# aicip/Cross-Scale-MAE

Measured on AMD Instinct MI355X. Metric: pretrain images/sec ViT-B/16 224^2 two-scale, higher is better.
Workload: dtype bf16; 1 GPU; MAE_ViT_MsLdCeCd ViT-B/16, 224^2 two-scale crops, mask 0.75, AdamW, full optimizer step; loss=mse, batch_per_gpu=128, global_batch=128, parallelism=dp1, headline_config=True

## Files before the change

### cross-scale-mae_amd/csmae_hip/__init__.py

```python
from __future__ import annotations

import ctypes
import os
from ctypes import c_float, c_int, c_longlong, c_void_p

import torch

F32, BF16 = 0, 1
ABI_VERSION = 7
EPI_NONE, EPI_GELU, EPI_RESID, EPI_DGELU, EPI_ATOMIC, EPI_SPLIT = 0, 1, 2, 3, 4, 5
EPI_GELU_Q8, EPI_DGELU_Q8 = 6, 7
ROUTE_F32, ROUTE_KSLAB = 7, 8
ATTN_ROUTE_RESIDENT, ATTN_ROUTE_STREAM, ATTN_ROUTE_ANY, ATTN_ROUTE_F32 = 0, 1, 2, 3
ATTN_STREAM_OWN, ATTN_STREAM_TILE = 128, 64
LOSS_KINDS = {"mse": 0, "l2": 1, "mae": 2, "l1": 3, "bce": 4, "none": 5}
SSIM_KINDS = {"ssim": ("none", 1, 1.0), "ms_ssim": ("none", 5, 1.0), "mse_ssim": ("mse", 1, 0.1), "mse_ms_ssim": ("mse", 5, 0.1)}

_ADDED_WITHIN_ABI = ("csmae_attn_route", "csmae_attn_stream_mode", "csmae_probe_pool_fwd", "csmae_bn1d_fwd", "csmae_head_linear_fwd",
                     "csmae_head_linear_bwd", "csmae_softmax_ce", "csmae_lars_step", "csmae_probe_pool_bwd", "csmae_head_linear_dx", "csmae_soft_ce",
                     "csmae_mixup_target", "csmae_mixup_cutmix", "csmae_pos_embed_grad", "csmae_eval_u8", "csmae_l2_normalize", "csmae_knn_select",
                     "csmae_knn_vote", "csmae_recon_eval", "csmae_recon_eval_workspace_floats", "csmae_recon_panel", "csmae_augment_u16",
                     "csmae_eval_u16")
_HERE = os.path.dirname(os.path.abspath(__file__))
LIB_PATH = os.environ.get("CSMAE_LIB_PATH") or os.path.join(_HERE, "libcsmae_hip.so")

I, L, P, F = c_int, c_longlong, c_void_p, c_float
_SIGNATURES = {
    "csmae_gemm": [I, I, I, L, L, L, P, L, P, L, P, L, I, P, I, P, L, P, L, I, P],
    "csmae_gemm_ks": [I, L, L, L, P, L, P, L, P, L, P, L, I, P, I, P, L, P, L, P],
    "csmae_weights_kslab": [I, P, I, P, P, P],
    "csmae_gemm_ln_supported": [L, L, L],
    "csmae_gemm_ln_fwd": [L, L, L, P, L, P, L, P, P, L, P, L, P, P, F, P, L, P, P, P],
    "csmae_gemm_ln_bwd": [L, L, L, P, L, P, L, P, L, P, P, P, P, L, P, L, P, L, P],
    "csmae_gemm_k2_mode": [I, I],
    "csmae_gemm_dw_mode": [I],
    "csmae_gemm_dw": [I, L, L, L, P, L, P, L, P, P, P, L, P],
    "csmae_gemm_dw_group": [I, I, L, P, P, P, P, P, P, P, P, I, P, L, P],
    "csmae_gemm_dw_group_fp8": [I, L, P, P, P, P, P, P, P, P, P, P, I, P, L, P],
    "csmae_fp8_amax": [I, L, I, P, L, P, P],
    "csmae_fp8_quantize": [I, I, I, L, I, P, L, P, L, P, P, P, P],
    "csmae_fp8_weights": [I, P, P, P, P, P, P, P],
    "csmae_gemm_fp8": [I, L, L, L, P, L, P, L, P, L, I, P, I, P, L, P, L, P, P, P, L, I, P, P, P, P],
    "csmae_gemm_force_tile": [I],
    "csmae_gemm_route": [I, I, I, L, L, L, L, L, L, I, I],
    "csmae_gemm_ks_route": [I, L, L, L, P, L, P, L, L, P, L, I],
    "csmae_attn_fwd": [I, L, I, I, I, P, P, P, P],
    "csmae_attn_bwd": [I, L, I, I, I, P, P, P, P, P, P],
    "csmae_attn_resident": [I, I, I],
    "csmae_attn_route": [I, I, I],
    "csmae_attn_stream_mode": [I],
    "csmae_attn_fwd_q": [I, L, I, I, I, P, P, P, P, I, P, P, P, P],
    "csmae_attn_bwd_q": [I, L, I, I, I, P, P, P, P, P, P, I, P, P, P, P],
    "csmae_layernorm_fwd": [I, I, L, I, P, P, P, F, P, P, P, P, P, I, P, P, P, P],
    "csmae_layernorm_bwd": [I, I, I, L, I, P, P, P, P, P, P, P, P, P, P, P, L, P, I, P, P, P, P],
    "csmae_ln_param_reduce": [I, L, I, P, L, L, P, P, P],
    "csmae_ln_param_reduce_rows": [I, I, I, P, L, P, P, P],
    "csmae_bnrelu_fwd": [I, I, I, I, P, P, P, F, F, P, P, P, P, P, P, I, P],
    "csmae_bnrelu_bwd": [I, I, I, I, P, P, P, P, P, P, P, P, P, P],
    "csmae_crop_resize": [L, I, P, P, P, P],
    "csmae_mask_sort": [L, I, I, P, P, P, P, P, P],
    "csmae_patch_gather": [I, L, I, I, I, I, I, P, P, P, P, L, P],
    "csmae_embed_assemble": [I, L, I, I, P, P, P, P, P, P],
    "csmae_embed_assemble_bwd": [I, I, L, I, I, P, P, P, P],
    "csmae_unshuffle_fwd": [I, L, I, I, I, P, P, P, P, P, P],
    "csmae_unshuffle_bwd": [I, I, L, I, I, I, P, P, P, P, P],
    "csmae_rows_gather": [I, L, I, P, L, L, L, P, P],
    "csmae_rows_scatter_add": [I, L, I, P, F, L, L, L, P, P],
    "csmae_rows_scatter_add2": [I, L, I, P, F, L, P, F, L, L, L, P, P],
    "csmae_spec_fixup": [P, P, L, P, L, P, L, P, P, P, P, I, P],
    "csmae_rows_gather_idx": [L, I, I, I, P, P, L, P, P],
    "csmae_target_minmax": [I, L, I, I, I, I, P, P, P, P, P],
    "csmae_recon_loss_fwd": [I, I, I, L, I, I, I, I, P, P, P, L, P, P, P, P],
    "csmae_recon_loss_bwd": [I, I, I, I, L, I, I, I, I, P, P, P, L, P, P, P, P, F, P, P, L, P],
    "csmae_ssim_workspace_floats": [L, I, I, I, I, P],
    "csmae_ssim_fwd": [I, I, I, L, I, I, I, I, P, P, P, L, P, P, P, P],
    "csmae_ssim_apply": [I, I, F, F, P, P, P],
    "csmae_ssim_bwd": [I, L, I, I, I, I, P, L, P, P, F, P, P, P],
    "csmae_pair_loss_fwd": [I, L, I, P, L, L, L, P, L, L, L, P, P],
    "csmae_pair_loss_bwd": [I, I, L, I, P, L, L, L, P, L, L, L, P, F, P, P, P, P],
    "csmae_ntxent_fwd": [I, I, I, I, P, F, F, P, P, P, P, P, P],
    "csmae_ntxent_bwd": [I, I, P, P, P, P, F, F, P, P, P],
    "csmae_latent_grad_finish": [I, L, I, I, P, P, F, P, P],
    "csmae_loss_finalize": [L, I, P, P, F, P, F, P, F, P, I, P, P],
    "csmae_augment_u8": [L, I, I, I, I, P, P, P, P, P, P],
    "csmae_eval_u8": [L, I, I, I, I, P, P, P, P, P, P],
    "csmae_augment_u16": [L, I, I, I, I, I, P, P, P, P, P, P, P],
    "csmae_eval_u16": [L, I, I, I, I, I, P, P, P, P, P, P, P],
    "csmae_next_launch_event": [P],
    "csmae_flush_launch_event": [P],
    "csmae_adamw": [L, P, P, P, P, P, P, P, F, F, F, F, F, F, P, P, P, P, P],
    "csmae_adamw_fp8": [L, P, F, P, P, P, P, F, F, F, F, F, F, P, P, P, P, P, P, P, P],
# ... 91 lines not shown
```

### cross-scale-mae_amd/csmae_hip/engine.py

```python
from __future__ import annotations

import contextlib
import math
import os
import weakref
from typing import Dict, Optional

import torch

from . import BF16, EPI_ATOMIC, EPI_DGELU, EPI_GELU, EPI_NONE, EPI_RESID, F32, SSIM_KINDS, debug_opt, ops
from . import trace

_FROZEN = ("encoder_pos_embed", "decoder_pos_embed")
_GEN_GONE = ("csmae_hip: backward of a forward whose activations are gone — the model ran another forward (training, eval "
             "or viz) in between; the engine keeps ONE activation workspace, so call loss.backward() before the next "
             "model(...) (accumulate gradients across backward calls, not across forwards)")
_GEN_TWICE = ("csmae_hip: backward called twice for the same forward (retain_graph is not supported: the reverse pass "
              "consumes the workspace)")


def _round_up(x, m):
    return (x + m - 1) // m * m


class FlatParams:

    def __init__(self, module: torch.nn.Module, device):
        self.names, self.slots = [], {}
        off = 0
        params = list(module.named_parameters())
        for name, p in params:
            n = p.numel()
            self.slots[name] = (off, n, tuple(p.shape))
            self.names.append(name)
            off += _round_up(n, 8)
        self.total = off
        self.p = torch.zeros(off, device=device, dtype=torch.float32)
        self.g = torch.zeros(off + 8, device=device, dtype=torch.float32)
        self.gate = self.g[off:off + 1]
        self.w_lp: Optional[torch.Tensor] = None
        self.lp_stamp = None
        self.raw_writes = 0
        self.params = dict(params)
        with torch.no_grad():
            for name, p in params:
                o, n, shape = self.slots[name]
                view = self.p[o:o + n].view(shape)
                view.copy_(p.data.to(device))
                p.data = view
        self.grad_views = {name: self.g[o:o + n].view(shape) for name, (o, n, shape) in self.slots.items()}
        self._by_id = {id(p): name for name, p in params}
        FlatParams._registry.append(weakref.ref(self))

    _registry = []

    @classmethod
    def owner_of(cls, p):
        alive = []
        found = None
        for ref in cls._registry:
            f = ref()
            if f is None:
                continue
            alive.append(ref)
            name = f._by_id.get(id(p))
            if name is not None and p.is_cuda and p.data_ptr() == f.p.data_ptr() + f.slots[name][0] * 4:
                found = f
        cls._registry[:] = alive
        return found

    def slot_of(self, p):
        return self.slots[self._by_id[id(p)]]

    def version_stamp(self) -> int:
        return sum(p._version for p in self.params.values())
# ... 121 lines not shown
                u8 = dict(device=dev, dtype=torch.uint8)
                self.t4_8 = [E(big8, **u8) for _ in range(2)]
                self.t3_8 = [E(max(Me * 3 * D, Md * 3 * Dd), **u8) for _ in range(2)]
                self.dres_e_8 = [E(Me, D, **u8) for _ in range(5)]
                self.dres_d_8 = [E(Md, Dd, **u8) for _ in range(5)]
            self.fp8_hist = False
            self.fp8_complete = False
        self.dw_ws = E(64 * 1024 * 1024, **f32)


class Engine:
    def __init__(self, module: torch.nn.Module, flat: FlatParams, cfg: dict, act_dtype=torch.bfloat16):
        self.module, self.cfg, self.device = module, cfg, flat.p.device
        self.fp8 = act_dtype == "fp8"
        self._fp8_site = 0
        self.fp8_dw = self.fp8 and not debug_opt("fp8_bf16_dw")
        self._fp8_blk = {}
        self._fp8_kept = {}
        self._fp8_cur = None
        self._fp8_fuse_lnb = not debug_opt("fp8_no_fuse_lnb")
        self._fp8_fuse_attn = not debug_opt("fp8_no_fuse_attn")
        self._fp8_fuse = not debug_opt("fp8_no_fuse")
        if self.fp8:
            act_dtype = torch.bfloat16
        if self.device.type != "cuda":
            raise RuntimeError("csmae_hip.Engine needs an MI355X (device 'cuda'): there is no CPU or eager fallback on the product path")
        self.act_dtype = act_dtype
        self.T = BF16 if act_dtype == torch.bfloat16 else F32
        self.res_dtype = torch.float32 if (self.T == F32 or os.environ.get("CSMAE_RESID_FP32")) else torch.bfloat16
        self.gp_q8 = self.T == BF16
        v = cfg["variant"]
        self.views = 1 if v == "Baseline" else 2
        self.has_pred = v in ("MsLdCd", "MsLdLeCd", "MsLdCeCd")
        self.has_ce = v == "MsLdCeCd"
        self.has_le = v in ("MsLdLe", "MsLdLeCd")
        self.Pp = _round_up(cfg["P"], 8) if self.T == BF16 else cfg["P"]
        self.flat = flat
        if self.T == BF16:
            if flat.w_lp is None:
                flat.w_lp = torch.zeros(flat.total, device=self.device, dtype=torch.bfloat16)
            if self.Pp != cfg["P"]:
                self.w_pe_pad = torch.zeros(cfg["D"], self.Pp, device=self.device, dtype=torch.bfloat16)
                self.w_pred_pad = torch.zeros(self.Pp, cfg["Dd"], device=self.device, dtype=torch.bfloat16)
        self.ws: Optional[Workspace] = None
        self._saved = None
        self.gen = 0
        self._gen_done = -1
        self.side, self.main, self.aux = None, None, None
        self._fwd_streams = []
        self._so = {}
        self._events, self._ev_i, self._side_reads, self._tog = [], 0, {}, 0
        self._side_seq, self._side_waited = 0, 0
        self._dw_cache = {}
        for key in ("bwd_main_cus", "main_cus"):
            v = debug_opt(key)
            if v is not None and not (len(v.split(":")) == 2 and all(q.isdigit() for q in v.split(":")) and int(v.split(":")[0]) < int(v.split(":")[1])):
                raise ValueError(f"CSMAE_DEBUG {key}={v!r}: expected lo:hi (mask bits of the compute units)")
        if not str(debug_opt("dw_cus", "0")).isdigit():
            raise ValueError(f"CSMAE_DEBUG dw_cus={debug_opt('dw_cus')!r}: expected the number of CUs per XCD")
        self.ln_fuse = self.T == BF16 and not self.fp8 and self.res_dtype == torch.bfloat16 and not debug_opt("no_lnfuse")
        self.ln_fuse_fwd = self.ln_fuse and not debug_opt("no_lnfuse_fwd")
        self.ln_fuse_bwd = self.ln_fuse and not debug_opt("no_lnfuse_bwd")
        self._ln_fuse_mask = int(debug_opt("lnfuse_mask", "15"))
        self.use_ks = not debug_opt("no_kslab")
        self._dw_slots = int(debug_opt("dw_slots", "160"))
        se = os.environ.get("CSMAE_DW_SLOTS_ED", "" if debug_opt("dw_slots") else "160,128")
        self._dw_slots_ed = tuple(int(v) for v in se.split(",")) if se else None
        self._dw_mode = debug_opt("dw_group", "half")
        self._dw_rot = self._dw_mode != "half0"
        if self._dw_mode == "half0":
            self._dw_mode = "half"
        if self._dw_mode not in ("block", "block_enc", "block_dec", "half", "none"):
            raise ValueError(f"CSMAE_DEBUG dw_group={self._dw_mode!r}: block, block_enc, block_dec, half or none")
        sl = flat.slots
        goff = lambda names: torch.tensor([[sl[n + ".weight"][0], sl[n + ".bias"][0]] for n in names], dtype=torch.long, device=self.device)
        self._goff_e = goff([f"encoder.{i}.norm{k}" for i in range(cfg["Ne"]) for k in (1, 2)])
        self._goff_d = goff([f"decoder.{i}.norm{k}" for i in range(cfg["Nd"]) for k in (1, 2)] + ["decoder_norm"])

    def W(self, name):
        if self.T == BF16:
            return self.flat.lp(name)
        t = self.flat.P(name)
        return t.view(t.shape[0], -1) if t.dim() > 1 else t

    def _refresh_lp(self, lazy_pads=False):
        if self.T != BF16:
            return
        if not self.fp8:
            self.flat.fp8_active = False
        stamp = self.flat.version_stamp()
        if stamp != self.flat.lp_stamp:
            self._opt_gate()
            ops.cast_bf16(self.flat.p, self.flat.w_lp)
            self.flat.lp_stamp = stamp
        if self.Pp != self.cfg["P"] and not lazy_pads:
            self._opt_gate()
            self._refresh_pads(True, True)
        self._refresh_ks()

    def _refresh_pads(self, pe, pred):
        P = self.cfg["P"]
        if pe:
            self.w_pe_pad[:, :P].copy_(self.flat.P("patch_embed.proj.weight").view(self.cfg["D"], P))
        if pred:
            self.w_pred_pad[:P].copy_(self.flat.P("decoder_pred.weight"))

# ... 122 lines not shown
                return ops.gemm_ks(a, f.w_ks[o:o + cnt], self.W(name), out, bias=bias, epilogue=epilogue, aux=aux, resid=resid, st=st)
            return ops.gemm(a, self.W(name), out, trans_b=trans_b, bias=bias, epilogue=epilogue, aux=aux, resid=resid, st=st)
        f, ws = self.flat, self.ws
        M, K = a.shape
        o, cnt, shape = f.slots[name]
        b8 = f.w8t[o:o + cnt].view(shape[1], shape[0]) if trans_b else f.w8[o:o + cnt].view(shape)
        fmt = ops.FP8_E5M2 if trans_b else ops.FP8_E4M3
        prev, cur = ws.fp8_amax[1], ws.fp8_amax[0]
        if a8 is not None:
            k = site
        else:
            k = site if site is not None else self._fp8_alloc()
            a8 = ws.a8[lane][: M * K].view(M, K)
            if ws.fp8_hist:
                ops.fp8_quantize(a, a8, prev[k], ws.fp8_dq[k:k + 1], fmt=fmt, amax_next=cur[k], st=st)
            else:
                ops.fp8_quantize(a, a8, cur[k], ws.fp8_dq[k:k + 1], fmt=fmt, st=st)
        emit = self._emit_to(emit_site, emit_dst, fmt) if emit_dst is not None else self._emit(emit_site, ws.q_b[lane], out.shape[0], out.shape[1], fmt)
        wi = f.w8_idx[name]
        return ops.gemm_fp8(a8, b8, out, ws.fp8_dq[k:k + 1], f.w8_dq[wi:wi + 1], a_fmt=fmt, bias=bias, epilogue=epilogue, aux=aux, resid=resid,
                            emit=emit, skip_out=skip_out and emit is not None, st=st)

    @staticmethod
    def _splitk(m_out, n_out, k_red, tile, ktile):
        tiles = math.ceil(m_out / tile) * math.ceil(n_out / tile)
        kt = math.ceil(k_red / ktile)
        want = max(1, 768 // tiles)
        return max(1, min(want, kt // 4 if kt >= 8 else 1))

    def _dw(self, dy, x, name):
        self._dw_group([(dy, x, name)])

    def _dw_group(self, items, slots=None, ready=None, items8=None):
        if items8 is not None:
            key = tuple((n, dy.data_ptr(), x.data_ptr(), qy.data_ptr(), qx.data_ptr()) for dy, qy, x, qx, n in items8)
            grp = self._dw_cache.get(key)
            if grp is None:
                prods = []
                for dy, qy, x, qx, name in items8:
                    gw = self.flat.G(name + ".weight")
                    gw2 = gw.view(gw.shape[0], -1)
                    prods.append((dy[:, : gw2.shape[0]], qy, x[:, : gw2.shape[1]], qx, gw2, self.flat.G(name + ".bias")))
                grp = self._dw_cache[key] = ops.DwGroup8(prods, self.ws.dw_ws)
        else:
            key = tuple((n, dy.data_ptr(), x.data_ptr()) for dy, x, n in items)
            grp = self._dw_cache.get(key)
        if grp is None:
            prods = []
            for dy, x, name in items:
                gw = self.flat.G(name + ".weight")
                gw2 = gw.view(gw.shape[0], -1)
                prods.append((dy[:, : gw2.shape[0]], x[:, : gw2.shape[1]], gw2, self.flat.G(name + ".bias")))
            grp = self._dw_cache[key] = ops.DwGroup(prods, self.ws.dw_ws)
        if ops._timer is not None or os.environ.get("CSMAE_DW_MAIN"):
            grp.launch(256, st=self.st)
            return
        side = self.side
        if ready is not None:
            ev = ready
        else:
            ev = self._event()
            ev.record(self.main)
        side.wait_event(ev)
        grp.launch(slots or self._dw_slots, st=side.cuda_stream)
        done = self._event()
        done.record(side)
        self._side_seq += 1
        for dy, _, _ in items:
            self._side_reads[dy.data_ptr()] = (self._side_seq, done)

    def _guard_write(self, *bufs):
        last = None
        for b in bufs:
            e = self._side_reads.pop(b.data_ptr(), None)
            if e is not None and (last is None or e[0] > last[0]):
                last = e
        if last is not None:
            if self._side_waited < last[0]:
                self.main.wait_event(last[1])
                self._side_waited = last[0]

    def _event(self):
        if self._ev_i == len(self._events):
            e = torch.cuda.Event()
            e.record()
            self._events.append(e)
        self._ev_i += 1
        return self._events[self._ev_i - 1]

    def _new_side(self):
        n = int(debug_opt("dw_cus", "0"))
        if n <= 0:
            return torch.cuda.Stream()
        self._side_masked = True
        return ops.cu_masked_stream(0, 8 * n)

    def _join_side(self):
        self.main.wait_stream(self.side)
        self._side_reads.clear()
        self._side_waited = self._side_seq

    def _block_fwd(self, S, i, pre, M, Dm, H, B2, T, b0=0, nb=None, st=None):
        P = self.flat.P
        st = self.st if st is None else st
        nb = B2 if nb is None else nb
        r = slice(b0 * T, (b0 + nb) * T)
        x_in, x_mid, x_out = S["x"][i][r], S["xm"][i][r], S["x"][i + 1][r]
        stt = [a[r] for a in S["st"][i]]
        lse = S["lse"][i][b0 * H * T: (b0 + nb) * H * T]
        qkv, o, h, pre_a = S["qkv"][i][r], S["o"][i][r], S["h"][i][r], S["pre"][i][r]
        y1, y2 = S["y1"][i][r], S["y2"][i][r]
        ws_q_a = self.ws.q_a if self.fp8 else None
        ln = int(b0 > 0)
        Mr = y1.shape[0]
        k1 = ko = k2 = kh = None
        if getattr(self.flat, "opt_pending", None) is not None:
            self._opt_gate((pre + "attn.qkv.weight", pre + "mlp.fc2.weight"), None if st is None else (self._so.get(st) or torch.cuda.ExternalStream(st)))
        if self.fp8:
            sites = self._fp8_blk.get((id(S), i))
            if sites is None:
                sites = self._fp8_blk[(id(S), i)] = tuple(self._fp8_alloc() for _ in range(4))
            k1, ko, k2, kh = sites
# ... 413 lines not shown
            self.ws = Workspace(self, N, keep)
        ws, P = self.ws, self.flat.P
        self.st = st = ops.stream()
        L, D = c["L"], c["D"]
        self.gen += 1
        if training:
            self._saved = dict(stream=True, N=N, keep=keep, gen=self.gen)
        self._opt_gate()
        self._refresh_lp()
        self._ks_wait()
        self._fp8_begin()
        ws.noise.copy_(noise)
        ops.mask_sort(ws.noise, keep, ws.ids_restore, ws.mask, ws.ids_keep, st=st)
        ops.patch_gather(imgs, None, ws.ids_keep, ws.a_pe, N, c["C"], c["S"], c["p"], keep, st=st)
        ops.gemm(ws.a_pe, self._w_pe(), ws.tok, bias=P("patch_embed.proj.bias"), st=st)
        ops.embed_assemble(ws.tok, P("encoder_pos_embed").view(L + 1, D), P("cls_token").view(D), ws.ids_keep, ws.enc["x"][0], N, keep, st=st)
        for i in range(c["Ne"]):
            self._block_fwd(ws.enc, i, f"encoder.{i}.", ws.Me, D, c["He"], N, ws.Te)
        return ws

    def stream_grad(self):
        return self.ws.dres_e if self.res_dtype == torch.float32 else self.ws.dres_e_lp[0]

    def stream_backward_ready(self, gen: Optional[int] = None):
        sv = self._saved
        if sv is None or not sv.get("stream"):
            if gen is not None and gen != self.gen:
                raise RuntimeError(_GEN_GONE)
            raise RuntimeError("backward_stream() called without a preceding encode_stream(training=True)")
        if (gen is not None and gen != sv["gen"]) or sv["gen"] != self.gen:
            raise RuntimeError(_GEN_GONE)
        if sv["gen"] == self._gen_done:
            raise RuntimeError(_GEN_TWICE)

    def backward_stream(self, dres: torch.Tensor, accumulate: bool, gen: Optional[int] = None, loss: Optional[torch.Tensor] = None):
        if self.fp8:
            raise NotImplementedError("backward_stream: the stand-alone encoder's backward is not implemented for fp8 engines")
        if getattr(self.module, "_dp", None) is not None:
            raise NotImplementedError("backward_stream: data-parallel gradient hooks are not implemented for the stand-alone encoder's backward")
        assert self.views == 1
        self.stream_backward_ready(gen)
        c, ws, sv = self.cfg, self.ws, self._saved
        N, keep, D = sv["N"], sv["keep"], c["D"]
        if keep != c["L"]:
            raise ValueError("backward_stream: the position-embedding gradient needs every patch in its place (mask_ratio 0)")
        self._gen_done = sv["gen"]
        self.st = st = ops.stream()
        self._opt_gate()
        self.main = torch.cuda.current_stream()
        if self.side is None:
            self.side = self._new_side()
        self._ev_i, self._tog = 0, 0
        self._side_reads.clear()
        with trace.range_("csmae.backward.encoder"):
            if not accumulate:
                self.flat.g[: self.flat.total].zero_()
            if loss is not None:
                ops.gate_accumulate(loss, self.flat.gate, accumulate, st=st)
            buf = self.stream_grad()
            if dres.dtype != buf.dtype or dres.numel() != buf.numel():
                raise ValueError(f"backward_stream: dres must be {tuple(buf.shape)} elements of {buf.dtype}, got {tuple(dres.shape)} of {dres.dtype}")
            if dres.data_ptr() != buf.data_ptr():
                buf.copy_(dres.reshape(buf.shape))
            if self.res_dtype == torch.float32:
                ops.latent_grad_finish(ws.dres_e, None, 1.0, ws.dres_e_lp[0], ws.B2, ws.Te, st=st)
            first = self._encoder_bwd()
            if self.flat.params["encoder_pos_embed"].requires_grad:
                ops.pos_embed_grad(first.view(N, ws.Te, D), self.flat.G("encoder_pos_embed").view(ws.Te, D), accumulate=True, st=st)
        for name, p in self.flat.params.items():
            if p.requires_grad:
                p.grad = self.flat.grad_views[name]
            elif not name.startswith("decoder"):
                self.flat.grad_views[name].zero_()

    def decode(self, latent: torch.Tensor, ids_restore: torch.Tensor):
        assert self.views == 1
        c = self.cfg
        N, Te, D = latent.shape
        keep, L, Dd = Te - 1, c["L"], c["Dd"]
        if self.ws is None or self.ws.N != N or self.ws.keep != keep:
            self.ws = None
            self.ws = Workspace(self, N, keep)
        ws, P = self.ws, self.flat.P
        self.st = st = ops.stream()
        self._opt_gate()
        self._refresh_lp()
        self._ks_wait()
        self._fp8_begin()
        lat = latent.reshape(N * Te, D).to(torch.float32).contiguous()
        if self.T == BF16:
            lat_op = ws.lat_lp if ws.lat_lp is not None else ws.enc["x"][c["Ne"]]
            ops.cast_bf16(lat, lat_op, st=st)
        else:
            lat_op = lat
        ws.ids_restore.copy_(ids_restore)
        ops.gemm(lat_op, self.W("decoder_embed.weight"), ws.z, bias=P("decoder_embed.bias"), st=st)
        ops.unshuffle_fwd(ws.z, P("mask_token").view(Dd), P("decoder_pos_embed").view(L + 1, Dd), ws.ids_restore, ws.dec["x"][0], N, L, keep, st=st)
        for i in range(c["Nd"]):
            self._block_fwd(ws.dec, i, f"decoder.{i}.", ws.Md, Dd, c["Hd"], N, ws.Td)
        ops.layernorm_fwd(ws.dec["x"][c["Nd"]], P("decoder_norm.weight"), P("decoder_norm.bias"), ws.emb_lp, ws.dn_st[0], ws.dn_st[1], y32=ws.emb32, st=st)
        ops.gemm(ws.emb_lp, self._w_pred()[: c["P"]], ws.pred, bias=P("decoder_pred.bias"), st=st)
        pred = ws.pred
        if pred.dtype != torch.float32:
            pred = torch.empty(ws.pred.shape, device=self.device, dtype=torch.float32)
            ops.cast_f32(ws.pred, pred, st=st)
        return pred.view(N, ws.Td, c["P"])[:, 1:, :].clone(), ws.emb32.view(N, ws.Td, Dd).clone()
# ... 7 lines not shown
        if not rng:
            with trace.range_("csmae.backward"):
                return self._backward(gout, accumulate, gen)
        lo, hi = (int(v) for v in rng.split(":"))
        outer, inner = torch.cuda.current_stream(), ops.cu_masked_stream(lo, hi)
        inner.wait_stream(outer)
        with torch.cuda.stream(inner):
            self._backward(gout, accumulate, gen)
        outer.wait_stream(inner)

    def _encoder_bwd(self, dp=None):
        c, ws, st, G = self.cfg, self.ws, self.st, self.flat.G
        B2, Te, D, keep = ws.B2, ws.Te, c["D"], self._saved["keep"]
        lp_stream = self.res_dtype != torch.float32
        self._fp8_cur = None
        pe, flushed = ws.ln_part_e, c["Ne"]
        fe = lp_stream and self._ln_fused_bwd(ws.Me, D)
        ke_ = 0
        for i in reversed(range(c["Ne"])):
            ke_ = self._block_bwd(ws.enc, i, f"encoder.{i}.", ws.Me, D, c["He"], B2, Te, None if lp_stream else ws.dres_e, ws.dres_e_lp, ke_, (pe[2 * i], pe[2 * i + 1]),
                                  lps8=ws.dres_e_8 if (self.fp8 and self.fp8_dw and lp_stream) else None)
            if dp is not None and dp.wants(("enc", i)):
                self._ln_flush(pe, self._goff_e, 2 * i, 2 * flushed, ws.Me, D, fused=fe)
                flushed = i
                dp.grads_ready(self.flat, ("enc", i), also=self.side if not (ops._timer is not None or os.environ.get("CSMAE_DW_MAIN")) else None)
        self._ln_flush(pe, self._goff_e, 0, 2 * flushed, ws.Me, D, fused=fe)
        first = ws.dres_e_lp[ke_] if lp_stream else ws.dres_e
        ops.embed_assemble_bwd(first, ws.dtok_lp, G("cls_token").view(D), B2, keep, st=st)
        self._join_side()
        ops.DwGroup([(ws.dtok_lp, ws.a_pe[:, : c["P"]], G("patch_embed.proj.weight").view(D, c["P"]), G("patch_embed.proj.bias"))], ws.dw_ws).launch(256, st=st)
        return first

    def _backward(self, gout: torch.Tensor, accumulate: bool, gen: Optional[int] = None):
        c, ws, sv = self.cfg, self.ws, self._saved
        if sv is None:
            raise RuntimeError("backward() called without a preceding forward()")
        if sv.get("stream"):
            raise RuntimeError("backward() after encode_stream(): the stand-alone encoder's reverse pass is backward_stream()")
        if gen is not None and gen != sv["gen"]:
            raise RuntimeError(_GEN_GONE)
        if sv["gen"] == self._gen_done:
            raise RuntimeError(_GEN_TWICE)
        self._gen_done = sv["gen"]
        P, G = self.flat.P, self.flat.G
        self.st = st = ops.stream()
        self._opt_gate()
        N, keep = sv["N"], sv["keep"]
        B2, Te, Td, L, D, Dd = ws.B2, ws.Te, ws.Td, c["L"], c["D"], c["Dd"]
        self.main = torch.cuda.current_stream()
        if self.side is None:
            self.side = self._new_side()
        self._ev_i, self._tog = 0, 0
        self._side_reads.clear()
        zeroed = None
        if not accumulate:
            if ops._timer is not None or os.environ.get("CSMAE_DW_MAIN") or debug_opt("zero_main"):
                self.flat.g[: self.flat.total].zero_()
            else:
                self.side.wait_stream(self.main)
                with torch.cuda.stream(self.side):
                    self.flat.g[: self.flat.total].zero_()
                zeroed = self._event()
                zeroed.record(self.side)
        ops.gate_accumulate(ws.losses, self.flat.gate, accumulate, st=st)
        ws.gout.copy_(gout.reshape(1).to(torch.float32))
        head_start = self._event()
        head_start.record(self.main)
        kind, npx = c["loss"], c["norm_pix"]
        trace.push("csmae.backward.junction")
        extra = None
        ssim = SSIM_KINDS.get(kind)
        if ssim is not None:
            kind, extra = ssim[0], ws.ssim_extra
            ops.ssim_bwd(ssim[1], ws.pred, ws.mask, ws.gout, sv["rscale"] * ssim[2], ws.ssim_ws, extra, B2, N, c["C"], c["S"], c["p"], st=st)
        ops.recon_loss_bwd(kind, npx, sv["img0"], sv["img1"], ws.pred, sv["mm"], ws.mask, ws.losses, ws.gout, sv["rscale"], ws.dpred_lp,
                           B2, N, c["C"], c["S"], c["p"], extra=extra, st=st)
        timed = ops._timer is not None or bool(os.environ.get("CSMAE_DW_MAIN"))
        heads_serial = timed or not self.has_pred
        if heads_serial:
            self._dw(ws.dpred_lp, ws.emb_lp, "decoder_pred")
        ops.gemm(ws.dpred_lp, self._w_pred(), ws.demb, trans_b=True, st=st)
        if zeroed is not None:
            self.main.wait_event(zeroed)
        if self.has_pred:
            kcd = c["loss_cd"]
            bn = "predictor.1."
            if heads_serial:
                ops.pair_loss_bwd(kcd, N * L, Dd, ws.v, (N * L, 0, 0), ws.emb32, (L, Td, 1), ws.gout, self._pair_scale(kcd, N * L, Dd),
                                  da_lp=ws.dv, dt_acc=ws.demb, st=st)
                self._dw(ws.dv, ws.r, "predictor.3")
                ops.gemm(ws.dv, self.W("predictor.3.weight"), ws.dr, trans_b=True, st=st)
                ops.bnrelu_bwd(ws.u, ws.dr, P(bn + "weight"), P(bn + "bias"), ws.bn_st[0], ws.bn_st[1], ws.dr, G(bn + "weight"), G(bn + "bias"), N, L, st=st)
                self._dw(ws.dr, ws.pin, "predictor.0")
                ops.gemm(ws.dr, self.W("predictor.0.weight"), ws.dpin, trans_b=True, st=st)
                ops.rows_scatter_add(ws.dpin, ws.demb, L, Td, N * Td + 1, st=st)
            else:
                aux, ast = self.aux, self.aux.cuda_stream
                aux.wait_event(head_start)
                if sv.get("spec"):
                    if zeroed is not None:
                        aux.wait_event(zeroed)
                    ops.spec_fixup(ws.gout, (ws.dv, ws.dr, ws.dpin), ws.bn_tmp, G(bn + "weight"), G(bn + "bias"), st=ast)
                else:
                    ops.pair_loss_bwd(kcd, N * L, Dd, ws.v, (N * L, 0, 0), ws.emb32, (L, Td, 1), ws.gout, self._pair_scale(kcd, N * L, Dd),
                                      da_lp=ws.dv, st=ast)
                    ops.gemm(ws.dv, self.W("predictor.3.weight"), ws.dr, trans_b=True, st=ast)
                    if zeroed is not None:
                        aux.wait_event(zeroed)
                    ops.bnrelu_bwd(ws.u, ws.dr, P(bn + "weight"), P(bn + "bias"), ws.bn_st[0], ws.bn_st[1], ws.dr, G(bn + "weight"), G(bn + "bias"), N, L, st=ast)
                    ops.gemm(ws.dr, self.W("predictor.0.weight"), ws.dpin, trans_b=True, st=ast)
                self.main.wait_stream(aux)
                ops.rows_scatter_add2(ws.dv, -1.0, 1, ws.dpin, 1.0, N * Td + 1, ws.demb, L, Td, st=st)
                ej = self._event()
                ej.record(self.main)
# ... 1 lines not shown
                self._dw_group([(ws.dv, ws.r, "predictor.3"), (ws.dr, ws.pin, "predictor.0")], ready=ej)
        trace.pop()
        trace.push("csmae.backward.decoder")
        lp_stream = self.res_dtype != torch.float32
        pd, Nd2 = ws.ln_part_d, 2 * c["Nd"]
        self._fp8_cur = None
        if lp_stream:
            k0 = self._fp8_alloc()
            e0 = None
            if self.fp8 and self._fp8_fuse_lnb:
                e0 = self._emit_to(k0, ws.dres_d_8[0], 1) if self.fp8_dw else self._emit(k0, ws.q_a[1], ws.Md, Dd, 1)
            ops.layernorm_bwd(ws.demb, ws.dec["x"][c["Nd"]], ws.dn_st[0], ws.dn_st[1], P("decoder_norm.weight"), ws.dres_d_lp[0], None, None,
                              partial_ws=pd[Nd2], emit=e0, st=st)
            if k0 is not None:
                self._fp8_cur = (k0, e0[0] if e0 else None)
        else:
            ops.layernorm_bwd(ws.demb, ws.dec["x"][c["Nd"]], ws.dn_st[0], ws.dn_st[1], P("decoder_norm.weight"), ws.dres_d, None, None,
                              dx_lp=ws.dres_d_lp[0], partial_ws=pd[Nd2], st=st)
        kd_ = 0
        for i in reversed(range(c["Nd"])):
            kd_ = self._block_bwd(ws.dec, i, f"decoder.{i}.", ws.Md, Dd, c["Hd"], B2, Td, ws.dres_d, ws.dres_d_lp, kd_, (pd[2 * i], pd[2 * i + 1]),
                                  lps8=ws.dres_d_8 if (self.fp8 and self.fp8_dw and lp_stream) else None)
        if lp_stream and self._ln_fused_bwd(ws.Md, Dd):
            self._ln_flush(pd, self._goff_d, 0, Nd2, ws.Md, Dd, fused=True)
            self._ln_flush(pd, self._goff_d, Nd2, Nd2 + 1, ws.Md, Dd)
        else:
            self._ln_flush(pd, self._goff_d, 0, Nd2 + 1, ws.Md, Dd)
        ops.unshuffle_bwd(ws.dres_d_lp[kd_] if lp_stream else ws.dres_d, ws.ids_restore, ws.dz_lp, G("mask_token").view(Dd), B2, L, keep, st=st)
        lat_op = ws.enc["x"][c["Ne"]] if (lp_stream or self.T != BF16) else ws.lat_lp
        self._dw(ws.dz_lp, lat_op, "decoder_embed")
        ops.gemm(ws.dz_lp, self.W("decoder_embed.weight"), ws.dres_e, trans_b=True, st=st)
        dp = getattr(self.module, "_dp", None)
        if dp is not None:
            dp.grads_ready(self.flat, "tail", also=self.side if not (ops._timer is not None or os.environ.get("CSMAE_DW_MAIN")) else None)
        trace.pop()
        trace.push("csmae.backward.encoder")
        latent = ws.lat32 if ws.lat32 is not None else ws.enc["x"][c["Ne"]]
        if self.has_le:
            ke = c["loss_e"]
            ops.pair_loss_bwd(ke, N * Te, D, latent, (N * Te, 0, N * Te), latent, (N * Te, 0, 0), ws.gout, self._pair_scale(ke, N * Te, D),
                              da_acc=ws.dres_e, dt_acc=ws.dres_e, lp_dtype=self.T, st=st)
        dpool = None
        if self.has_ce:
            ops.ntxent_bwd(ws.zc, ws.inv_norm, ws.E, ws.neg, ws.gout, ws.dpool, N, st=st)
            dpool = ws.dpool
        ops.latent_grad_finish(ws.dres_e, dpool, 1.0 / keep, ws.dres_e_lp[0], B2, Te, st=st)
        self._encoder_bwd(dp)
        if dp is not None:
            dp.grads_ready(self.flat, "stem")
            dp.backward_done(self.flat)
        trace.pop()
        if self.fp8:
            ws.fp8_complete = True
        for name, p in self.flat.params.items():
            if p.requires_grad and not name.startswith("encoder_norm."):
                p.grad = self.flat.grad_views[name]
            elif not (name in _FROZEN or name.startswith("encoder_norm.")):
                self.flat.grad_views[name].zero_()
```

### cross-scale-mae_amd/csmae_hip/ops.py

```python
from __future__ import annotations

import ctypes

import torch

from . import BF16, EPI_ATOMIC, EPI_DGELU, EPI_GELU, EPI_NONE, EPI_RESID, F32, LOSS_KINDS, check, load
from . import EPI_DGELU_Q8 as _EPI_DGELU_Q8, EPI_GELU_Q8 as _EPI_GELU_Q8

_DT = {torch.float32: F32, torch.bfloat16: BF16}
_timer = None
_Q8 = {EPI_GELU: _EPI_GELU_Q8, EPI_DGELU: _EPI_DGELU_Q8}


class KernelTimer:

    def __init__(self):
        self.records, self._e0 = [], None

    def __enter__(self):
        global _timer
        _timer = self
        return self

    def __exit__(self, *a):
# ... 132 lines not shown
    return rc


def gemm_ks(a, bk, b_plain, out, *, bias=None, epilogue=EPI_NONE, aux=None, resid=None, st=None):
    M, K = a.shape
    N = b_plain.shape[0]
    assert b_plain.shape[1] == K and out.shape == (M, N) and a.stride(1) == 1 and out.stride(1) == 1 and b_plain.stride(1) == 1
    assert resid is None or resid.dtype == out.dtype
    assert bk.dtype == torch.bfloat16 and bk.is_contiguous() and bk.numel() >= N * K, "gemm_ks: the K-slab mirror is a flat bf16 tensor of N * K elements"
    epilogue = _epi(epilogue, aux)
    t = _begin()
    check(load().csmae_gemm_ks(dt(a), M, N, K, _p(a), a.stride(0), _p(bk), N, _p(b_plain), b_plain.stride(0), _p(out), out.stride(0), dt(out), _p(bias), epilogue,
                               _p(aux), aux.stride(0) if aux is not None else 0, _p(resid), resid.stride(0) if resid is not None else 0, _s(st)), "csmae_gemm_ks")
    if t:
        t.end(("gemm_bf16" if a.dtype == torch.bfloat16 else "gemm_f32") + "_NT", 2.0 * M * N * K)
    return out


def gemm_ln_supported(M, N, K):
    return load().csmae_gemm_ln_supported(M, N, K) == 1


def gemm_ln_fwd(a, bk, bias, resid, x_out, gamma, beta, y, mean, rstd, eps=1e-6, st=None):
    M, K = a.shape
    N = x_out.shape[1]
    assert a.dtype == resid.dtype == x_out.dtype == y.dtype == bk.dtype == torch.bfloat16 and bk.is_contiguous() and bk.numel() >= N * K
    assert resid.shape == x_out.shape == y.shape == (M, N) and a.stride(1) == resid.stride(1) == x_out.stride(1) == y.stride(1) == 1
    assert mean.dtype == rstd.dtype == torch.float32 and mean.numel() >= M and rstd.numel() >= M and gamma.numel() == beta.numel() == N
    t = _begin()
    check(load().csmae_gemm_ln_fwd(M, N, K, _p(a), a.stride(0), _p(bk), N, _p(bias), _p(resid), resid.stride(0), _p(x_out), x_out.stride(0), _p(gamma), _p(beta),
                                   eps, _p(y), y.stride(0), _p(mean), _p(rstd), _s(st)), "csmae_gemm_ln_fwd")
    if t:
        t.end("gemm_bf16_NT", 2.0 * M * N * K)


def gemm_ln_bwd(dy, w, x, mean, rstd, gamma, dres_in, dx_out, partial_ws=None, st=None):
    M, K = dy.shape
    N = w.shape[1]
    assert w.shape[0] == K and x.shape == dx_out.shape == (M, N) and (dres_in is None or dres_in.shape == (M, N))
    assert dy.dtype == w.dtype == x.dtype == dx_out.dtype == torch.bfloat16 and (dres_in is None or dres_in.dtype == torch.bfloat16)
    assert dy.stride(1) == w.stride(1) == x.stride(1) == dx_out.stride(1) == 1 and mean.dtype == rstd.dtype == torch.float32
    t = _begin()
    check(load().csmae_gemm_ln_bwd(M, N, K, _p(dy), dy.stride(0), _p(w), w.stride(0), _p(x), x.stride(0), _p(mean), _p(rstd), _p(gamma), _p(dres_in),
                                   dres_in.stride(0) if dres_in is not None else 0, _p(dx_out), dx_out.stride(0), _p(partial_ws),
                                   partial_ws.numel() if partial_ws is not None else 0, _s(st)), "csmae_gemm_ln_bwd")
    if t:
        t.end("gemm_bf16_NN", 2.0 * M * N * K)


def weights_kslab(desc, src, dst, max_blocks=64, st=None):
    check(load().csmae_weights_kslab(desc.shape[0], _p(desc), max_blocks, _p(src), _p(dst), _s(st)), "csmae_weights_kslab")


def gemm_dw(dy, x, dw, workspace, db=None, st=None):
    K, M = dy.shape
    N = x.shape[1]
    assert x.shape[0] == K and dw.shape == (M, N) and dw.is_contiguous() and dy.dtype == x.dtype
    t = _begin()
    check(load().csmae_gemm_dw(dt(dy), M, N, K, _p(dy), dy.stride(0), _p(x), x.stride(0), _p(dw), _p(db), _p(workspace), workspace.numel(), _s(st)), "csmae_gemm_dw")
    if t:
        t.end(("gemm_bf16" if dy.dtype == torch.bfloat16 else "gemm_f32") + "_TN", 2.0 * M * N * K)


FP8_E4M3, FP8_E5M2 = 0, 1


def fp8_quantize(src, dst, amax, dq, fmt=FP8_E4M3, transpose=False, amax_next=None, st=None):
    rows, cols = src.shape
    assert dst.dtype == torch.uint8 and dst.shape == ((cols, rows) if transpose else (rows, cols)) and src.stride(1) == 1 and dst.stride(1) == 1
    s = _s(st)
    if amax_next is None:
        check(load().csmae_fp8_amax(dt(src), rows, cols, _p(src), src.stride(0), _p(amax), s), "csmae_fp8_amax")
    check(load().csmae_fp8_quantize(dt(src), fmt, int(transpose), rows, cols, _p(src), src.stride(0), _p(dst), dst.stride(0), _p(amax), _p(dq),
                                    _p(amax_next), s), "csmae_fp8_quantize")


FP8_SLOTS = 64


def fp8_weights(desc, p, w8, w8t, amax, dq, st=None):
    check(load().csmae_fp8_weights(desc.shape[0], _p(desc), _p(p), _p(w8), _p(w8t), _p(amax), _p(dq), _s(st)), "csmae_fp8_weights")


def gemm_fp8(a8, b8, out, dq_a, dq_b, *, a_fmt=FP8_E4M3, bias=None, epilogue=EPI_NONE, aux=None, resid=None, emit=None, skip_out=False, st=None):
    assert not skip_out or emit is not None
    M, K = a8.shape
    N = b8.shape[0]
    assert a8.dtype == torch.uint8 and b8.dtype == torch.uint8 and b8.shape[1] == K and out.shape == (M, N)
    assert resid is None or resid.dtype == out.dtype
    epilogue = _epi(epilogue, aux)
    q_out, *q_rest = _emit_args(emit)
    t = _begin()
    check(load().csmae_gemm_fp8(a_fmt, M, N, K, _p(a8), a8.stride(0), _p(b8), b8.stride(0), None if skip_out else _p(out), out.stride(0), dt(out), _p(bias), epilogue,
                                _p(aux), aux.stride(0) if aux is not None else 0, _p(resid), resid.stride(0) if resid is not None else 0,
                                _p(dq_a), _p(dq_b), q_out, emit[0].stride(0) if emit else 0, *q_rest, _s(st)), "csmae_gemm_fp8")
    if t:
        t.end("gemm_fp8_NT", 2.0 * M * N * K)
    return out


def _dw_group_args(self, products, workspace, dy, x, dw, db):
    VP, LL = ctypes.c_void_p * len(products), ctypes.c_longlong * len(products)
    self.n, self.keep = len(products), (products, workspace)
    self.dY, self.X, self.dW, self.dB = (VP(*[_p(q[i]) for q in products]) for i in (dy, x, dw, db))
    self.ldy, self.ldx = LL(*[q[dy].stride(0) for q in products]), LL(*[q[x].stride(0) for q in products])
    self.M, self.N = LL(*[q[dw].shape[0] for q in products]), LL(*[q[dw].shape[1] for q in products])
    self.flops = sum(2.0 * q[dw].shape[0] * q[dw].shape[1] * self.K for q in products)
    self.ws, self.ws_n = _p(workspace), workspace.numel()


class DwGroup:

    def __init__(self, products, workspace):
        self.K = products[0][0].shape[0]
        self.dtype = dt(products[0][0])
        for dy, x, dw, db in products:
            assert dy.shape[0] == self.K and x.shape[0] == self.K and dw.is_contiguous() and dy.dtype == x.dtype and dy.stride(1) == 1 and x.stride(1) == 1
        _dw_group_args(self, products, workspace, 0, 1, 2, 3)

    def launch(self, slots=0, st=None):
        t = _begin()
        check(load().csmae_gemm_dw_group(self.dtype, self.n, self.K, self.dY, self.ldy, self.X, self.ldx, self.dW, self.dB, self.M, self.N, slots,
                                         self.ws, self.ws_n, _s(st)), "csmae_gemm_dw_group")
        if t:
            t.end(("gemm_bf16" if self.dtype == BF16 else "gemm_f32") + "_TN", self.flops)


class DwGroup8:

    def __init__(self, products, workspace):
        self.K = products[0][0].shape[0]
        for dy, dqy, x, dqx, dw, db in products:
            assert dy.dtype == x.dtype == torch.uint8 and dy.shape[0] == x.shape[0] == self.K and dy.stride(1) == x.stride(1) == 1 and dw.is_contiguous()
            assert dqy.dtype == dqx.dtype == torch.float32 and dqy.numel() >= 1 and dqx.numel() >= 1
        _dw_group_args(self, products, workspace, 0, 2, 4, 5)
        self.dqy, self.dqx = ((ctypes.c_void_p * self.n)(*[_p(q[i]) for q in products]) for i in (1, 3))

    def launch(self, slots=0, st=None):
        t = _begin()
        check(load().csmae_gemm_dw_group_fp8(self.n, self.K, self.dY, self.ldy, self.dqy, self.X, self.ldx, self.dqx, self.dW, self.dB, self.M, self.N, slots,
                                             self.ws, self.ws_n, _s(st)), "csmae_gemm_dw_group_fp8")
        if t:
            t.end("gemm_fp8_TN", self.flops)


def attn_resident(dtype_code, T, hd):
    return load().csmae_attn_resident(dtype_code, T, hd) == 1


def attn_route(dtype_code, T, hd):
    rc = load().csmae_attn_route(dtype_code, T, hd)
    if rc < 0:
        raise RuntimeError(f"csmae_attn_route: dtype {dtype_code}, T {T}, head_dim {hd} unsupported ({rc})")
    return rc


def attn_stream_mode(mode=-1):
    return load().csmae_attn_stream_mode(mode)


def attn_fwd(qkv, out, lse, B, T, H, hd, emit=None, st=None):
    if emit is None:
        check(load().csmae_attn_fwd(dt(qkv), B, T, H, hd, _p(qkv), _p(out), _p(lse), _s(st)), "csmae_attn_fwd")
    else:
        check(load().csmae_attn_fwd_q(dt(qkv), B, T, H, hd, _p(qkv), _p(out), _p(lse), *_emit_args(emit), _s(st)), "csmae_attn_fwd_q")


def attn_bwd(qkv, out, dout, lse, dqkv, B, T, H, hd, emit=None, skip_out=False, st=None):
    assert not skip_out or emit is not None
    if emit is None:
        check(load().csmae_attn_bwd(dt(qkv), B, T, H, hd, _p(qkv), _p(out), _p(dout), _p(lse), _p(dqkv), _s(st)), "csmae_attn_bwd")
    else:
        check(load().csmae_attn_bwd_q(dt(qkv), B, T, H, hd, _p(qkv), _p(out), _p(dout), _p(lse), None if skip_out else _p(dqkv), *_emit_args(emit), _s(st)),
              "csmae_attn_bwd_q")


def _emit_args(emit):
    if emit is None:
        return None, 0, None, None, None
    return _p(emit[0]), emit[1], _p(emit[2]), _p(emit[3]), _p(emit[4])


def layernorm_fwd(x, gamma, beta, y, mean, rstd, y32=None, eps=1e-6, emit=None, skip_out=False, st=None):
    M, D = x.shape
    assert not skip_out or emit is not None
    check(load().csmae_layernorm_fwd(dt(x), dt(y), M, D, _p(x), _p(gamma), _p(beta), eps, None if skip_out else _p(y), _p(y32), _p(mean), _p(rstd), *_emit_args(emit),
                                     _s(st)), "csmae_layernorm_fwd")


def layernorm_bwd(dy, x, mean, rstd, gamma, dx_out, dgamma, dbeta, dres_in=None, dx_lp=None, partial_ws=None, emit=None, st=None):
    M, D = x.shape
    assert dx_out.dtype == x.dtype and (dres_in is None or dres_in.dtype == x.dtype)
    lp = dt(dx_lp) if dx_lp is not None else dt(dy)
    check(load().csmae_layernorm_bwd(dt(dy), dt(x), lp, M, D, _p(dy), _p(x), _p(mean), _p(rstd), _p(gamma), _p(dres_in), _p(dx_out), _p(dx_lp), _p(dgamma), _p(dbeta),
# ... 412 lines not shown
```

### cross-scale-mae_amd/csrc/gemm.hip

```cpp
#include "gemm_common.h"

template <bool TA, bool TB, int BM, int BN, int WM, int WN, int GEMM_STAGES, bool DB, int MINW = 1>
__global__ __launch_bounds__((BM / WM) * (BN / WN) * 64, MINW) void gemm_bf16_kernel(GemmArgs p) {
  constexpr int NWN = BN / WN, NW = (BM / WM) * NWN, FM = WM / 16, FN = WN / 16;
  constexpr int A_BYTES = BM * GEMM_BK * 2, B_BYTES = BN * GEMM_BK * 2, STAGE = A_BYTES + B_BYTES;
  constexpr int PA = A_BYTES / 1024, PB = B_BYTES / 1024, PPW = (PA + PB) / NW;
  static_assert((PA + PB) % NW == 0, "DMA pieces must divide evenly over the waves");
  __shared__ __attribute__((aligned(16))) char smem[GEMM_STAGES * STAGE];
  const int lane = threadIdx.x & 63, w = __builtin_amdgcn_readfirstlane(threadIdx.x >> 6);
  const int t = lane & 15, g = lane >> 4;
  const int tiles = p.tiles_m * p.tiles_n;
  const int wg = xcd_remap(blockIdx.x, tiles * p.splitk);
  const int split = wg / tiles, tile = wg - split * tiles;
  const int tm = tile / p.tiles_n, tn = tile - tm * p.tiles_n;
  const int m0 = tm * BM, n0 = tn * BN;
  const int kt_begin = split * p.ktiles_per_split;
  const int kt_end = min(kt_begin + p.ktiles_per_split, p.ktiles);
  if (kt_begin >= kt_end) return;
  if (p.epi == EPI_SPLIT) p.C = reinterpret_cast<float*>(p.C) + (long long)split * p.split_stride;

  const i4_t rsA = make_rsrc(p.A, p.a_bytes), rsB = make_rsrc(p.B, p.b_bytes);
  const unsigned kstepA = TA ? (unsigned)(GEMM_BK * p.lda * 2) : (unsigned)(GEMM_BK * 2);
  const unsigned kstepB = TB ? (unsigned)(GEMM_BK * p.ldb * 2) : (unsigned)(GEMM_BK * 2);

// ... 119 lines not shown
      if (!(grp == 1 && kt == last)) __builtin_amdgcn_s_barrier();
      __builtin_amdgcn_sched_barrier(0);
    }
  } else {
    int issued = min(kt_begin + GEMM_STAGES - 2, last);
    for (int kt = kt_begin; kt <= issued; ++kt) stage(kt);
    s8_t fa0[FM] = {}, fb0[FN] = {};
    for (int kt = kt_begin; kt < kt_end; ++kt) {
      arrive(kt, issued);
      if (issued < last) { ++issued; if (!(dbg & 32)) stage(issued); }
      if (!(dbg & 128)) read_frags(kt, fa0, fb0);
      if (!(dbg & 64)) mma(fa0, fb0);
    }
  }
  if (do_cs && g == 0) {
#pragma unroll
    for (int i = 0; i < FM; ++i) {
      const int m = m0 + wm + i * 16 + t;
      if (m < p.M) p.colsum[(long long)split * p.M + m] = accb[i][0];
    }
  }
  if ((p.force_cfg & 16) && acc[0][0][0] != 123456.0f) return;
  if (p.epi == EPI_ATOMIC) {
#pragma unroll
    for (int i = 0; i < FM; ++i)
#pragma unroll
      for (int j = 0; j < FN; ++j)
        epi_dispatch(p, m0 + wm + i * 16 + t, n0 + wn + j * 16 + 4 * g, acc[i][j]);
    return;
  }
  constexpr int ESTR = WN + 4, LPR = WN / 4, RPP = 64 / LPR;
  constexpr int EROWS = (NW * 32 * ESTR * 4 <= GEMM_STAGES * STAGE) ? 32 : 16;
  static_assert(NW * EROWS * ESTR * 4 <= GEMM_STAGES * STAGE, "epilogue strip must fit the staging ring");
  if (!DB) __syncthreads();
  void* Cptr = p.C;
  float* ew = reinterpret_cast<float*>(smem) + w * (EROWS * ESTR);
#define EPI_CALL(TC_, E_) epilogue_rows<TC_, E_, FM, FN, WM, EROWS, ESTR, LPR, RPP>(p, Cptr, acc, ew, m0 + wm, n0 + wn, lane, t, g)
  if (p.c_dtype == CSMAE_BF16) {
    if (p.epi == EPI_GELU) EPI_CALL(bf16_t, EPI_GELU); else if (p.epi == EPI_DGELU) EPI_CALL(bf16_t, EPI_DGELU);
    else if (p.epi == EPI_RESID) EPI_CALL(bf16_t, EPI_RESID); else EPI_CALL(bf16_t, EPI_NONE);
  } else {
    if (p.epi == EPI_GELU) EPI_CALL(float, EPI_GELU); else if (p.epi == EPI_DGELU) EPI_CALL(float, EPI_DGELU);
    else if (p.epi == EPI_RESID) EPI_CALL(float, EPI_RESID); else EPI_CALL(float, EPI_NONE);
  }
#undef EPI_CALL
}

#ifdef GEMM_TIMING
extern "C" int csmae_debug_gemm_ts(unsigned long long* out) { return (int)hipMemcpyFromSymbol(out, HIP_SYMBOL(g_gemm_ts), sizeof(g_gemm_ts)); }
#endif
#ifndef GEMM_ABL
#define GEMM_ABL 0
#endif
struct DwFold { float* slab; float* cs_slab; int nsplit; int slot; int nslots; };
#define K64_LDS_BYTES (5 * 256 * 64 * 2)

template <bool TA, bool TB, int BM, bool GROUP, int CSV = 0>
__device__ __forceinline__ void k64_tile(char* smem, const GemmArgs& p, const int tm, const int tn, const int split, const int kt_begin, const int kt_end, const DwFold fold) {
  static_assert(BM == 256 || (BM == 192 && !TA), "192-row tiles exist for K-contiguous A only");
  constexpr int BN = 256, WM = BM / 2, WN = 64, NWN = BN / WN, NW = 8, FM = WM / 16, FN = WN / 16;
  constexpr int UNIT = 256 * 64 * 2, NUNIT = 5, PPU = UNIT / 1024 / NW;
  constexpr int PPA = BM * 64 * 2 / 1024 / NW;
  static_assert(NUNIT * UNIT == K64_LDS_BYTES, "LDS of the pipelined kernels");
  const int lane = threadIdx.x & 63, w = __builtin_amdgcn_readfirstlane(threadIdx.x >> 6);
  const int t = lane & 15, g = lane >> 4;
  const int m0 = tm * BM, n0 = tn * BN;
  void* Cptr = (!GROUP && p.epi == EPI_SPLIT) ? static_cast<void*>(reinterpret_cast<float*>(p.C) + (long long)split * p.split_stride) : p.C;

  GTS(0);
  const i4_t rsA = make_rsrc(p.A, p.a_bytes), rsB = make_rsrc(p.B, p.b_bytes);
  const unsigned kstepA = TA ? (unsigned)(64 * p.lda * 2) : 128u;
  const unsigned kstepB = TB ? (unsigned)(64 * p.ldb * 2) : 128u;

  const int l3 = lane >> 3, l5 = lane >> 5, s16 = lane & 31;
  const int kc = ((lane & 7) ^ l3) * 8;
  auto tr_ch = [&](int qodd) { const int key = l5 | (qodd << 1) | ((w & 1) << 2); return (((s16 >> 1) ^ key) << 1) | (s16 & 1); };
  unsigned avo[2], bvo[2];
  if (!TA) avo[0] = avo[1] = (unsigned)(((long long)(m0 + w * (PPA * 8) + l3) * p.lda + kc) * 2);
  else {
    avo[0] = (unsigned)(((long long)(w * 8 + l5) * p.lda + m0 + tr_ch(0) * 8) * 2);
    avo[1] = (unsigned)(((long long)(w * 8 + l5) * p.lda + m0 + tr_ch(1) * 8) * 2);
  }
  if (!TB) bvo[0] = bvo[1] = (unsigned)(((long long)(n0 + w * 32 + l3) * p.ldb + kc) * 2);
  else {
    bvo[0] = (unsigned)(((long long)(w * 8 + l5) * p.ldb + n0 + tr_ch(0) * 8) * 2);
    bvo[1] = (unsigned)(((long long)(w * 8 + l5) * p.ldb + n0 + tr_ch(1) * 8) * 2);
  }
  const unsigned aqs = (unsigned)((TA ? 2 : 8) * p.lda * 2), bqs = (unsigned)((TB ? 2 : 8) * p.ldb * 2);
  const int dbg = p.force_cfg;
  const unsigned ldsA = (unsigned)(size_t)LDS_PTR(char, smem) + (unsigned)(w * PPA) * 1024u, ldsB = (unsigned)(size_t)LDS_PTR(char, smem) + (unsigned)(w * PPU) * 1024u;
  auto dma_a = [&](int slot, int j, int q) {
    if (GEMM_ABL & 2) return;
    lds_dma16u(rsA, avo[q & 1] + ((unsigned)j * kstepA + (unsigned)q * aqs), ldsA + (unsigned)(slot * UNIT + q * 1024));
  };
  auto dma_b = [&](int slot, int j, int q) {
    if (GEMM_ABL & 2) return;
    lds_dma16u(rsB, bvo[q & 1] + ((unsigned)j * kstepB + (unsigned)q * bqs), ldsB + (unsigned)(slot * UNIT + q * 1024));
  };

  f4_t acc[FM][FN];
#pragma unroll
  for (int i = 0; i < FM; ++i)
#pragma unroll
    for (int j = 0; j < FN; ++j) acc[i][j] = f4_t{0.f, 0.f, 0.f, 0.f};
  const int wm = (w / NWN) * WM, wn = (w % NWN) * WN;
  const int ra0 = !TA ? (wm + t) * 128 + ((g ^ (t & 7)) << 4)
                      : ((((wm >> 4) ^ ((t >> 2) | ((g & 1) << 2))) << 5) + (t & 3) * 8 + (8 * g + (t >> 2)) * (BM * 2));
// ... 113 lines not shown
    if (MODE <= 1) asm volatile("s_waitcnt vmcnt(%0)" ::"n"(PPA) : "memory");
    else if (MODE == 2) asm volatile("s_waitcnt vmcnt(0)" ::: "memory");
    asm volatile("s_waitcnt lgkmcnt(0)" ::: "memory");
    __builtin_amdgcn_s_barrier();
    __builtin_amdgcn_sched_barrier(0);
    if (more) { read_a(sl2, 0, std::integral_constant<int, 0>{}, fa[0]); read_a(sl2, 0, std::integral_constant<int, 1>{}, fa[1]); read_b(sl3, 0, fb0); }
    static_for<FM - 2>([&](auto ic) {
      constexpr int i = decltype(ic)::value + 2, r = i - 2, NR = FM - 2;
      mma_row(i, fa[i], fb1);
      if (more) read_a(sl2, 0, std::integral_constant<int, i>{}, fa[i]);
      if (MODE <= 1) {
#pragma unroll
        for (int pc = r * PPU / NR; pc < (r + 1) * PPU / NR; ++pc) dma_b(sl, jabs + 2, pc);
      }
      __builtin_amdgcn_sched_barrier(0);
    });
  };
  int j = 0, sl = 0;
  if (nsteps >= 3) { step(kt_begin, 0, std::integral_constant<int, 1>{}); j = 1; sl = 2; }
  for (; j < nsteps - 2; ++j, sl = nxt(sl, 2)) step(kt_begin + j, sl, std::integral_constant<int, 0>{});
  if (nsteps >= 2) { step(kt_begin + j, sl, std::integral_constant<int, 2>{}); ++j; sl = nxt(sl, 2); }
  step(kt_begin + j, sl, std::integral_constant<int, 3>{});
  GTS(2);
  if (TA && TB && do_cs) {
#pragma unroll
    for (int e = 0; e < 2; ++e) {
      float v = cs[e];
      v += __shfl_xor(v, 16); v += __shfl_xor(v, 32);
      cs[e] = v;
      const int m = m0 + wm + (2 * wq + e) * 16 + t;
      if (!GROUP && g == 0 && m < p.M) p.colsum[(long long)split * p.M + m] = v;
    }
  }
  if ((dbg & 16) && acc[0][0][0] != 123456.0f) return;
  if (GROUP) {
    constexpr int ESTR = WN + 4, LPR = WN / 4, RPP = 64 / LPR, EROWS = 32;
    float* ew = reinterpret_cast<float*>(smem) + w * (EROWS * ESTR);
    if (fold.nsplit > 1) {
      if (do_cs && g == 0) {
        float* csm = fold.cs_slab + ((long long)split * fold.nslots + fold.slot) * 256;
        csm[wm + (2 * wq) * 16 + t] = cs[0];
        csm[wm + (2 * wq + 1) * 16 + t] = cs[1];
      }
      GemmArgs q = p;
      q.M = 256; q.N = 256; q.ldc = 256; q.bias = nullptr;
      float* mine = fold.slab + ((long long)split * fold.nslots + fold.slot) * (256 * 256);
      epilogue_rows<float, EPI_NONE, FM, FN, WM, EROWS, ESTR, LPR, RPP>(q, mine, acc, ew, wm, wn, lane, t, g);
      return;
    }
    if (do_cs && g == 0) {
#pragma unroll
      for (int e = 0; e < 2; ++e) {
        const int m = m0 + wm + (2 * wq + e) * 16 + t;
        if (m < p.M) p.colsum[m] += cs[e];
      }
    }
    epilogue_rows<float, EPI_RESID, FM, FN, WM, EROWS, ESTR, LPR, RPP>(p, Cptr, acc, ew, m0 + wm, n0 + wn, lane, t, g);
    return;
  }
  if (p.epi == EPI_ATOMIC) {
#pragma unroll
    for (int i = 0; i < FM; ++i)
#pragma unroll
      for (int jj = 0; jj < FN; ++jj)
        epi_dispatch(p, m0 + wm + i * 16 + t, n0 + wn + jj * 16 + 4 * g, acc[i][jj]);
    return;
  }
  constexpr int ESTR = WN + 4, LPR = WN / 4, RPP = 64 / LPR, EROWS = 32;
  constexpr int STRIP = NW * EROWS * ESTR * 4;
  static_assert(STRIP <= NUNIT * UNIT, "epilogue strip must fit the staging ring");
  float* ew = reinterpret_cast<float*>(smem) + w * (EROWS * ESTR);
#define EPI_CALL(TC_, E_) epilogue_rows<TC_, E_, FM, FN, WM, EROWS, ESTR, LPR, RPP>(p, Cptr, acc, ew, m0 + wm, n0 + wn, lane, t, g)
#define EPI_CALL8(E_) epilogue_rows_bf16x8<E_, FM, FN, WM, EROWS, ESTR>(p, Cptr, acc, ew, m0 + wm, n0 + wn, lane, t, g)
  const bool wide = (p.ldc % 8 == 0) && (p.epi == EPI_NONE || (p.epi == EPI_RESID ? (p.ldr % 8 == 0 && (uintptr_t)p.resid % 16 == 0)
                                                                                   : (p.ldaux % 8 == 0 && (uintptr_t)p.aux % 16 == 0)));
  if (p.c_dtype == CSMAE_BF16) {
#define EPI_CALL8B(E_) epilogue_rows_bf16x8b<E_, FM, FN, WM, EROWS, ESTR>(p, acc, ew, m0 + wm, n0 + wn, lane, t, g)
    if (wide && p.epi == EPI_NONE && p.q_out == nullptr)
      epilogue_rows_bf16_plain<FM, FN, WM>(p, Cptr, acc, reinterpret_cast<char*>(ew), m0 + wm, n0 + wn, lane, t, g);
    else if (wide && (p.a_fmt & 256)) { if (p.epi == EPI_GELU) EPI_CALL8B(EPI_GELU); else if (p.epi == EPI_DGELU) EPI_CALL8B(EPI_DGELU); else EPI_CALL8B(EPI_RESID); }
    else if (wide) { if (p.epi == EPI_GELU) EPI_CALL8(EPI_GELU); else if (p.epi == EPI_DGELU) EPI_CALL8(EPI_DGELU); else if (p.epi == EPI_RESID) EPI_CALL8(EPI_RESID); else EPI_CALL8(EPI_NONE); }
    else if (p.epi == EPI_RESID) EPI_CALL(bf16_t, EPI_RESID);
    else if (p.epi == EPI_GELU) EPI_CALL(bf16_t, EPI_GELU); else if (p.epi == EPI_DGELU) EPI_CALL(bf16_t, EPI_DGELU);
    else EPI_CALL(bf16_t, EPI_NONE);
#undef EPI_CALL8B
  } else {
    if (p.epi == EPI_GELU) EPI_CALL(float, EPI_GELU); else if (p.epi == EPI_DGELU) EPI_CALL(float, EPI_DGELU);
    else if (p.epi == EPI_RESID) EPI_CALL(float, EPI_RESID); else EPI_CALL(float, EPI_NONE);
  }
#undef EPI_CALL
#undef EPI_CALL8
  GTS(3);
}

template <bool TA, bool TB, int BM = 256>
__global__ __launch_bounds__(512, 1) void gemm_bf16_k64_kernel(GemmArgs p) {
  const int tiles = p.tiles_m * p.tiles_n;
  const int wg = xcd_remap(blockIdx.x, tiles * p.splitk);
  const int split = wg / tiles, tile = wg - split * tiles;
  const int tm = tile / p.tiles_n, tn = tile - tm * p.tiles_n;
  const int kt_begin = split * p.ktiles_per_split;
  const int kt_end = min(kt_begin + p.ktiles_per_split, p.ktiles);
  if (kt_begin >= kt_end) return;
  __shared__ __attribute__((aligned(16))) char smem[K64_LDS_BYTES];
  k64_tile<TA, TB, BM, false>(smem, p, tm, tn, split, kt_begin, kt_end, DwFold{});
}
__global__ __launch_bounds__(512, 1) void gemm_dw_group_kernel(DwGroupArgs ga) {
  const int wg = xcd_remap(blockIdx.x, ga.total_tiles * ga.nsplit);
  const int split = wg / ga.total_tiles, tile_id = wg - split * ga.total_tiles;
  DwDesc d = ga.d[0];
#pragma unroll
  for (int i = 1; i < DW_GROUP_MAX; ++i) if (i < ga.n && tile_id >= ga.d[i].tile0) d = ga.d[i];
  const int tile = tile_id - d.tile0;
  const int tm = tile / d.tiles_n, tn = tile - tm * d.tiles_n;
  const int kt_begin = split * ga.ktiles_per_split;
  const int kt_end = min(kt_begin + ga.ktiles_per_split, ga.ktiles);
  GemmArgs p;
  p.A = d.dY; p.B = d.X; p.C = d.dW; p.bias = nullptr; p.aux = nullptr; p.resid = d.dW;
  p.lda = d.ldy; p.ldb = d.ldx; p.ldc = d.N; p.ldaux = 0; p.ldr = d.N;
  p.M = d.M; p.N = d.N; p.K = ga.K;
  p.c_dtype = CSMAE_F32; p.epi = EPI_RESID; p.splitk = ga.nsplit; p.tiles_m = 0; p.tiles_n = d.tiles_n; p.ktiles = ga.ktiles; p.ktiles_per_split = ga.ktiles_per_split;
  p.a_bytes = (unsigned)((long long)ga.K * d.ldy * 2); p.b_bytes = (unsigned)((long long)ga.K * d.ldx * 2);
  p.force_cfg = ga.force_cfg; p.split_stride = 0; p.colsum = d.db; p.dq_a = p.dq_b = nullptr; p.a_fmt = 0; p.aux_q8 = 0; p.q_out = nullptr;
  __shared__ __attribute__((aligned(16))) char smem[K64_LDS_BYTES];
  const DwFold fold{ga.slab, ga.cs_slab, ga.nsplit, tile_id, ga.total_tiles};
  if (d.db != nullptr && tn == 0) k64_tile<true, true, 256, true, 2>(smem, p, tm, tn, split, kt_begin, kt_end, fold);
  else k64_tile<true, true, 256, true, 1>(smem, p, tm, tn, split, kt_begin, kt_end, fold);
}
__global__ __launch_bounds__(256) void dw_group_reduce_kernel(DwGroupArgs ga) {
  const int tile_id = blockIdx.x / DWR_PARTS, quarter = blockIdx.x % DWR_PARTS;
  DwDesc d = ga.d[0];
#pragma unroll
  for (int i = 1; i < DW_GROUP_MAX; ++i) if (i < ga.n && tile_id >= ga.d[i].tile0) d = ga.d[i];
  const int tile = tile_id - d.tile0;
  const int tm = tile / d.tiles_n, tn = tile - tm * d.tiles_n;
  const int m0 = tm * 256, n0 = tn * 256;
  const int c4 = threadIdx.x & 63, r0 = threadIdx.x >> 6;
  const long long sstride = (long long)ga.total_tiles * 256 * 256;
  const float* base = ga.slab + (long long)tile_id * 256 * 256;
  const int n = n0 + c4 * 4;
  constexpr int RPB = 256 / DWR_PARTS;
#pragma unroll
  for (int r = quarter * RPB + r0; r < quarter * RPB + RPB; r += 4) {
    const int m = m0 + r;
    if (m >= d.M || n >= d.N) continue;
    float* dst = d.dW + (long long)m * d.N + n;
    f4_t a = *reinterpret_cast<f4_t*>(dst);
    for (int sl = 0; sl < ga.nsplit; ++sl) a += *reinterpret_cast<const f4_t*>(base + sl * sstride + r * 256 + c4 * 4);
    *reinterpret_cast<f4_t*>(dst) = a;
  }
  if (quarter == 0 && tn == 0 && d.db != nullptr) {
    const int m = m0 + threadIdx.x;
    if (m < d.M) {
      float a = d.db[m];
      for (int sl = 0; sl < ga.nsplit; ++sl) a += ga.cs_slab[((long long)sl * ga.total_tiles + tile_id) * 256 + threadIdx.x];
      d.db[m] = a;
    }
  }
}

typedef int i8v_t __attribute__((ext_vector_type(8)));
template <int AFMT>
__global__ __launch_bounds__(512, 1) void gemm_fp8_kernel(GemmArgs p) {
  constexpr int BM = 256, BN = 256, WM = 128, WN = 64, NWN = 4, NW = 8, FM = 8, FN = 4, IMG = 256 * 128, STAGE = 2 * IMG;
  __shared__ __attribute__((aligned(16))) char smem[2 * STAGE];
  const int lane = threadIdx.x & 63, w = __builtin_amdgcn_readfirstlane(threadIdx.x >> 6);
  const int t = lane & 15, g = lane >> 4;
  const int tiles = p.tiles_m * p.tiles_n;
  const int tile = xcd_remap(blockIdx.x, tiles);
  const int tm = tile / p.tiles_n, tn = tile - tm * p.tiles_n;
  const int m0 = tm * BM, n0 = tn * BN;
  const i4_t rsA = make_rsrc(p.A, p.a_bytes), rsB = make_rsrc(p.B, p.b_bytes);
  const int l3 = lane >> 3, kc = ((lane & 7) ^ l3) * 16;
  const int arow = m0 + w * 32 + l3, brow = n0 + w * 32 + l3;
  const unsigned avo = (unsigned)((long long)arow * p.lda + kc), bvo = (unsigned)((long long)brow * p.ldb + kc);
  auto stage = [&](int kt, int buf) {
    char* base = smem + buf * STAGE;
    const bool kok = kt * 128 + kc < p.K;
#pragma unroll
    for (int q = 0; q < 4; ++q) {
      const unsigned oa = (kok && arow + q * 8 < p.M) ? avo + (unsigned)(kt * 128) + (unsigned)(q * 8 * p.lda) : OOB_OFF;
      lds_dma16(rsA, oa, base + (w * 4 + q) * 1024);
    }
#pragma unroll
    for (int q = 0; q < 4; ++q) {
      const unsigned ob = (kok && brow + q * 8 < p.N) ? bvo + (unsigned)(kt * 128) + (unsigned)(q * 8 * p.ldb) : OOB_OFF;
      lds_dma16(rsB, ob, base + IMG + (w * 4 + q) * 1024);
    }
  };
  f4_t acc[FM][FN];
#pragma unroll
  for (int i = 0; i < FM; ++i)
#pragma unroll
    for (int j = 0; j < FN; ++j) acc[i][j] = f4_t{0.f, 0.f, 0.f, 0.f};
  const int wm = (w / NWN) * WM, wn = (w % NWN) * WN;
  const int ra0 = (wm + t) * 128, rb0 = (wn + t) * 128, sw = t & 7;
  const int c0 = ((2 * g) ^ sw) << 4, c1 = ((2 * g + 1) ^ sw) << 4;
  auto frag = [&](const char* img, int roff) {
    const u4_t lo = *reinterpret_cast<const u4_t*>(img + roff + c0), hi = *reinterpret_cast<const u4_t*>(img + roff + c1);
    return i8v_t{(int)lo[0], (int)lo[1], (int)lo[2], (int)lo[3], (int)hi[0], (int)hi[1], (int)hi[2], (int)hi[3]};
  };
  const int nk = p.ktiles;
  stage(0, 0);
  for (int kt = 0; kt < nk; ++kt) {
    const int buf = kt & 1;
    asm volatile("s_waitcnt vmcnt(0)" ::: "memory");
    __syncthreads();
// ... 360 lines not shown
    p.splitk = cdiv(p.ktiles, p.ktiles_per_split);
    dim3 grid(p.tiles_m * p.tiles_n * p.splitk);
#define LAUNCH_CFG(TA_, TB_)                                                                                              \
    if (cfg == 1) hipLaunchKernelGGL((gemm_bf16_kernel<TA_, TB_, 256, 128, 64, 64, 3, false, 4>), grid, dim3(512), 0, st, p);     \
    else if (cfg == 2) hipLaunchKernelGGL((gemm_bf16_kernel<TA_, TB_, 256, 256, 128, 64, 4, false>), grid, dim3(512), 0, st, p);  \
    else if (cfg == 3) hipLaunchKernelGGL((gemm_bf16_kernel<TA_, TB_, 256, 256, 128, 64, 4, true>), grid, dim3(512), 0, st, p);   \
    else hipLaunchKernelGGL((gemm_bf16_kernel<TA_, TB_, 128, 128, 64, 64, 4, false>), grid, dim3(256), 0, st, p);
    if (cfg == 6) gemm_k2_launch_nn(p, st);
    else if (cfg == 5 && !transB) CSMAE_LAUNCH((gemm_bf16_k64_kernel<false, false, 192>), grid, dim3(512), 0, st, p);
    else if (cfg == 5) CSMAE_LAUNCH((gemm_bf16_k64_kernel<false, true, 192>), grid, dim3(512), 0, st, p);
    else if (cfg == 4 && transA) CSMAE_LAUNCH((gemm_bf16_k64_kernel<true, true>), grid, dim3(512), 0, st, p);
    else if (cfg == 4 && !transB) CSMAE_LAUNCH((gemm_bf16_k64_kernel<false, false>), grid, dim3(512), 0, st, p);
    else if (cfg == 4) CSMAE_LAUNCH((gemm_bf16_k64_kernel<false, true>), grid, dim3(512), 0, st, p);
    else if (!transA && !transB) { LAUNCH_CFG(false, false) }
    else if (!transA && transB) { LAUNCH_CFG(false, true) }
    else if (transA && transB) { LAUNCH_CFG(true, true) }
    else { LAUNCH_CFG(true, false) }
#undef LAUNCH_CFG
  } else if (dtype == CSMAE_F32) {
    p.a_bytes = p.b_bytes = 0;
    p.tiles_m = cdiv(M, 64); p.tiles_n = cdiv(N, 64); p.ktiles = cdiv(K, 16);
    p.ktiles_per_split = cdiv(p.ktiles, splitk);
    p.splitk = cdiv(p.ktiles, p.ktiles_per_split);
    dim3 grid(p.tiles_m * p.tiles_n * p.splitk), block(256);
    if (!transA && !transB) hipLaunchKernelGGL((gemm_f32_kernel<false, false>), grid, block, 0, st, p);
    else if (!transA && transB) hipLaunchKernelGGL((gemm_f32_kernel<false, true>), grid, block, 0, st, p);
    else if (transA && transB) hipLaunchKernelGGL((gemm_f32_kernel<true, true>), grid, block, 0, st, p);
    else hipLaunchKernelGGL((gemm_f32_kernel<true, false>), grid, block, 0, st, p);
  } else {
    csmae_set_error("csmae_gemm: unsupported dtype %d", dtype);
    return CSMAE_ERR_UNSUPPORTED;
  }
  return csmae_check_launch("csmae_gemm");
}
extern "C" int csmae_gemm(int dtype, int transA, int transB, long long M, long long N, long long K,
                          const void* A, long long lda, const void* B, long long ldb,
                          void* C, long long ldc, int c_dtype, const float* bias, int epilogue,
                          void* aux, long long ldaux, const void* resid, long long ldr,
                          int splitk, void* stream) {
  return gemm_core(dtype, transA, transB, M, N, K, A, lda, B, ldb, C, ldc, c_dtype, bias, epilogue, aux, ldaux, resid, ldr, splitk, stream);
}

int gemm_core_route(int dtype, int transA, int transB, long long M, long long N, long long K, long long lda, long long ldb, int epilogue, int splitk) {
  if (dtype != CSMAE_F32 && dtype != CSMAE_BF16) return CSMAE_ERR_UNSUPPORTED;
  return gemm_route(dtype, transA, transB, M, N, K, lda, ldb, epilogue == EPI_GELU_Q8 ? EPI_GELU : (epilogue == EPI_DGELU_Q8 ? EPI_DGELU : epilogue), splitk);
}
extern "C" int csmae_gemm_route(int dtype, int transA, int transB, long long M, long long N, long long K, long long lda, long long ldb, long long ldc,
                                int epilogue, int splitk) {
  (void)ldc;
  return gemm_core_route(dtype, transA, transB, M, N, K, lda, ldb, epilogue, splitk);
}

__global__ __launch_bounds__(256) void dw_reduce_kernel(long long n4, int S, long long slab4, const f4_t* __restrict__ ws, f4_t* __restrict__ dw,
                                                        const float* __restrict__ wsb, float* __restrict__ db, int M) {
  for (long long i = (long long)blockIdx.x * blockDim.x + threadIdx.x; i < n4; i += (long long)gridDim.x * blockDim.x) {
    f4_t a = dw[i];
    for (int s = 0; s < S; ++s) a += ws[s * slab4 + i];
    dw[i] = a;
  }
  if (db && blockIdx.x == 0)
    for (int m = threadIdx.x; m < M; m += blockDim.x) {
      float a = db[m];
      for (int s = 0; s < S; ++s) a += wsb[(long long)s * M + m];
      db[m] = a;
    }
}
extern "C" int csmae_gemm_dw(int dtype, long long M, long long N, long long K, const void* dY, long long ldy, const void* X, long long ldx,
                             float* dW, float* db, float* workspace, long long ws_elems, void* stream);
extern "C" int csmae_gemm_dw_group(int dtype, int count, long long K, const void* const* dY, const long long* ldy, const void* const* X,
                                   const long long* ldx, float* const* dW, float* const* db, const long long* M, const long long* N, int slots,
                                   float* workspace, long long ws_elems, void* stream) {
  CSMAE_REQUIRE(count > 0 && count <= DW_GROUP_MAX && K > 0 && dY && X && dW && M && N && ldy && ldx && workspace, "csmae_gemm_dw_group: bad arguments (1..%d products)", DW_GROUP_MAX);
  bool fused = dtype == CSMAE_BF16 && g_force_cfg < 0;
  for (int i = 0; i < count && fused; ++i) fused = M[i] >= 256 && N[i] >= 256 && N[i] % 4 == 0 && ldy[i] % 8 == 0 && ldx[i] % 8 == 0 && ldy[i] >= (M[i] + 7) / 8 * 8 && ldx[i] >= (N[i] + 7) / 8 * 8 &&
                                                   K * ldy[i] * 2 < 0xFFFFFFF0ll && K * ldx[i] * 2 < 0xFFFFFFF0ll && ((((uintptr_t)dY[i] | (uintptr_t)X[i] | (uintptr_t)dW[i]) & 15) == 0);
  if (!fused) {
    for (int i = 0; i < count; ++i) {
      int rc = csmae_gemm_dw(dtype, M[i], N[i], K, dY[i], ldy[i], X[i], ldx[i], dW[i], db ? db[i] : nullptr, workspace, ws_elems, stream);
      if (rc) return rc;
    }
    return CSMAE_OK;
  }
  DwGroupArgs ga;
  if (g_k2_dw) {
    for (int i = 0; i < count; ++i) {
      DwDesc& d = ga.d[i];
      d.dY = dY[i]; d.X = X[i]; d.dW = dW[i]; d.db = db ? db[i] : nullptr; d.M = (int)M[i]; d.N = (int)N[i]; d.ldy = ldy[i]; d.ldx = ldx[i];
    }
    ga.n = count; ga.K = (int)K; ga.force_cfg = 0; ga.ktiles = cdiv(K, 64);
    return gemm_k2_launch_dw(ga, count, slots <= 0 ? 128 : slots, workspace, ws_elems, (hipStream_t)stream);
  }
  int tiles = 0;
  for (int i = 0; i < count; ++i) {
    DwDesc& d = ga.d[i];
    d.dY = dY[i]; d.X = X[i]; d.dW = dW[i]; d.db = db ? db[i] : nullptr; d.M = (int)M[i]; d.N = (int)N[i]; d.ldy = ldy[i]; d.ldx = ldx[i];
    d.tiles_n = cdiv(N[i], 256); d.tile0 = tiles;
    tiles += cdiv(M[i], 256) * d.tiles_n;
  }
  for (int i = count; i < DW_GROUP_MAX; ++i) ga.d[i] = ga.d[0];
  ga.n = count; ga.K = (int)K; ga.total_tiles = tiles; ga.force_cfg = 0;
  ga.ktiles = cdiv(K, 64);
  if (slots <= 0) slots = 128;
  long long S = slots / tiles;
  if (S > ga.ktiles / 8) S = ga.ktiles / 8;
  const long long per_slice = (long long)tiles * (256 * 256 + 256);
  if (S > ws_elems / per_slice) S = ws_elems / per_slice;
  if (S < 1) S = 1;
  ga.ktiles_per_split = cdiv(ga.ktiles, S);
  ga.nsplit = cdiv(ga.ktiles, ga.ktiles_per_split);
  ga.slab = workspace; ga.cs_slab = workspace + (long long)ga.nsplit * tiles * 256 * 256;
  CSMAE_REQUIRE(ga.nsplit == 1 || ws_elems >= ga.nsplit * per_slice, "csmae_gemm_dw_group: workspace too small");
  hipLaunchKernelGGL(gemm_dw_group_kernel, dim3(tiles * ga.nsplit), dim3(512), 0, (hipStream_t)stream, ga);
  if (ga.nsplit > 1) hipLaunchKernelGGL(dw_group_reduce_kernel, dim3(tiles * DWR_PARTS), dim3(256), 0, (hipStream_t)stream, ga);
  return csmae_check_launch("csmae_gemm_dw_group");
}
extern "C" int csmae_gemm_dw(int dtype, long long M, long long N, long long K, const void* dY, long long ldy, const void* X, long long ldx,
                             float* dW, float* db, float* workspace, long long ws_elems, void* stream) {
  CSMAE_REQUIRE(M > 0 && N > 0 && K > 0 && N % 4 == 0 && workspace && ws_elems >= M * N + M, "csmae_gemm_dw: bad arguments / workspace too small");
  const int tile = dtype == CSMAE_BF16 ? ((M >= 256 && N >= 256) ? 256 : 128) : 64;
  const bool k64 = dtype == CSMAE_BF16 && tile == 256 && (g_force_cfg < 0 || (g_force_cfg & 7) == 4);
  const int kt = dtype == CSMAE_BF16 ? (k64 ? 64 : GEMM_BK) : 16;
  const long long tiles = (long long)cdiv(M, tile) * cdiv(N, tile), ktiles = cdiv(K, kt);
  static const int slots256 = csmae_debug_opt("dw_slots") ? atoi(csmae_debug_opt("dw_slots")) : 160;
  const long long slots = dtype == CSMAE_BF16 ? (tile == 256 ? slots256 : 512) : 2048;
  long long S = slots / tiles;
  if (S > ktiles / (k64 ? 4 : 6)) S = ktiles / (k64 ? 4 : 6);
  if (S > ws_elems / (M * N + M)) S = ws_elems / (M * N + M);
  if (S < 1) S = 1;
  const int kps = cdiv(ktiles, S);
  S = cdiv(ktiles, kps);
  float* wsb = workspace + S * M * N;
  const bool fused_bias = db && dtype == CSMAE_BF16;
  int rc = csmae_gemm(dtype, 1, 1, M, N, K, dY, ldy, X, ldx, workspace, N, CSMAE_F32, nullptr, EPI_SPLIT, fused_bias ? wsb : nullptr, 0, nullptr, 0, (int)S, stream);
  if (rc) return rc;
  const long long n4 = M * N / 4;
  hipLaunchKernelGGL(dw_reduce_kernel, dim3((unsigned)fmin((double)cdiv(n4, 256), 2048.0)), dim3(256), 0, (hipStream_t)stream, n4, (int)S, n4,
                     reinterpret_cast<const f4_t*>(workspace), reinterpret_cast<f4_t*>(dW), wsb, fused_bias ? db : nullptr, (int)M);
  if (db && !fused_bias) return csmae_colsum_launch(dtype, K, (int)M, dY, ldy, db, stream);
  return csmae_check_launch("csmae_gemm_dw");
}
```

### cross-scale-mae_amd/csrc/gemm_common.h

```cpp
#pragma once
#include "common.h"
#include <type_traits>
#include <cstdlib>
#include <utility>

template <typename F, int... I>
__device__ __forceinline__ void static_for_impl(F&& f, std::integer_sequence<int, I...>) { (f(std::integral_constant<int, I>{}), ...); }
template <int N, typename F>
__device__ __forceinline__ void static_for(F&& f) { static_for_impl(f, std::make_integer_sequence<int, N>{}); }

constexpr int EPI_NONE = CSMAE_EPI_NONE;
constexpr int EPI_GELU = CSMAE_EPI_GELU;
constexpr int EPI_RESID = CSMAE_EPI_RESID;
constexpr int EPI_DGELU = CSMAE_EPI_DGELU;
constexpr int EPI_ATOMIC = CSMAE_EPI_ATOMIC;
constexpr int EPI_SPLIT = CSMAE_EPI_SPLIT;
constexpr int EPI_GELU_Q8 = CSMAE_EPI_GELU_Q8, EPI_DGELU_Q8 = CSMAE_EPI_DGELU_Q8;

struct GemmArgs {
  const void* A; const void* B; void* C; const float* bias; void* aux; const void* resid;
  long long lda, ldb, ldc, ldaux, ldr;
  int M, N, K;
  int c_dtype, epi, splitk, tiles_m, tiles_n, ktiles, ktiles_per_split;
  unsigned a_bytes, b_bytes;
// ... 370 lines not shown
  }
}

template <int FM, int FN, int WM>
__device__ __forceinline__ void epilogue_rows_bf16_plain(const GemmArgs& p, void* Cptr, f4_t (&acc)[FM][FN], char* ew, int mbase, int nbase, int lane, int t, int g) {
  constexpr int WN = FN * 16, ROWB = WN * 2 + 8, EROWS = (WM % 64 == 0) ? 64 : 32, NPART = WM / EROWS, LPR = WN / 8, RPP = 64 / LPR, NPASS = EROWS / RPP;
  static_assert(WM % EROWS == 0 && EROWS * ROWB <= 32 * (WN + 4) * 4, "the bf16 strip reuses the fp32 strip's bytes");
  f4_t bj[FN];
#pragma unroll
  for (int j = 0; j < FN; ++j) {
    const int n = nbase + j * 16 + 4 * g;
    bj[j] = (p.bias && n < p.N) ? *reinterpret_cast<const f4_t*>(p.bias + n) : f4_t{0.f, 0.f, 0.f, 0.f};
  }
  const int col = (lane % LPR) * 8, rsub = lane / LPR;
  const int gn = nbase + col;
  const bool ok0 = gn < p.N, ok1 = gn + 4 < p.N;
  bf16_t* C = reinterpret_cast<bf16_t*>(Cptr);
#pragma unroll
  for (int part = 0; part < NPART; ++part) {
#pragma unroll
    for (int ii = 0; ii < EROWS / 16; ++ii)
#pragma unroll
      for (int j = 0; j < FN; ++j) {
        f4_t v = acc[part * (EROWS / 16) + ii][j];
        v += bj[j];
        *reinterpret_cast<uint2*>(ew + (ii * 16 + t) * ROWB + (j * 16 + 4 * g) * 2) = make_uint2(pack2bf(v[0], v[1]), pack2bf(v[2], v[3]));
      }
#pragma unroll
    for (int ps = 0; ps < NPASS; ++ps) {
      const int r = ps * RPP + rsub, gm = mbase + part * EROWS + r;
      const uint4 v = *reinterpret_cast<const uint4*>(ew + r * ROWB + col * 2);
      if (gm < p.M) {
        if (ok1) *reinterpret_cast<uint4*>(C + (long long)gm * p.ldc + gn) = v;
        else if (ok0) *reinterpret_cast<uint2*>(C + (long long)gm * p.ldc + gn) = make_uint2(v.x, v.y);
      }
    }
  }
}

#ifdef GEMM_TIMING
static __device__ unsigned long long g_gemm_ts[8];
#ifndef GTS_BLOCK
#define GTS_BLOCK 300
#endif
#define GTS(i) do { if (blockIdx.x == GTS_BLOCK && threadIdx.x == 0) g_gemm_ts[i] = __builtin_readcyclecounter(); } while (0)
#else
#define GTS(i)
#endif
#define DW_GROUP_MAX 8
struct DwDesc { const void* dY; const void* X; float* dW; float* db; int M, N; long long ldy, ldx; int tiles_n, tile0; };
struct DwGroupArgs {
  DwDesc d[DW_GROUP_MAX];
  int n, K, ktiles, ktiles_per_split, nsplit, total_tiles, force_cfg;
  float* slab; float* cs_slab;
};
#define DWR_PARTS 16
int gemm_k2_launch_dw(DwGroupArgs& ga, int count, int slots, float* workspace, long long ws_elems, hipStream_t st);
int gemm_force_cfg();
bool gemm_k2_nn_wanted(int epilogue, long long K, long long N, long long M);
bool gemm_k2_nt_wanted(int epilogue, long long K, long long N, long long M);
int gemm_k2_launch_nn(const GemmArgs& p, hipStream_t st);
int gemm_core_route(int dtype, int transA, int transB, long long M, long long N, long long K, long long lda, long long ldb, int epilogue, int splitk);
int gemm_core(int dtype, int transA, int transB, long long M, long long N, long long K, const void* A, long long lda, const void* B, long long ldb,
              void* C, long long ldc, int c_dtype, const float* bias, int epilogue, void* aux, long long ldaux, const void* resid, long long ldr,
              int splitk, void* stream);
```

### cross-scale-mae_amd/csrc/gemm_fp8_dw.hip

```cpp
#include "gemm_common.h"

typedef int i8v_t __attribute__((ext_vector_type(8)));
struct Dw8Desc { const void* dY; const void* X; float* dW; float* db; const float* dq_y; const float* dq_x; int M, N; long long ldy, ldx; int tiles_n, tile0; };
struct Dw8GroupArgs {
  Dw8Desc d[DW_GROUP_MAX];
  int n, K, ktiles, ktiles_per_split, nsplit, total_tiles;
  float* slab; float* cs_slab;
};

__device__ __forceinline__ void fp8_dw_tile(char* smem, const Dw8Desc& d, const int K, const int tm, const int tn, const int split, const int kt_begin, const int kt_end,
                                            float* slab, const int nsplit, const int slot, const int nslots) {
  constexpr int WM = 128, WN = 64, NWN = 4, NW = 8, FM = 8, FN = 4, UNIT = 128 * 256, NUNIT = 5, PP = UNIT / 1024 / NW;
  const int lane = threadIdx.x & 63, w = __builtin_amdgcn_readfirstlane(threadIdx.x >> 6);
  const int t = lane & 15, g = lane >> 4;
  const int m0 = tm * 256, n0 = tn * 256;
  const i4_t rsA = make_rsrc(d.dY, (unsigned)((long long)K * d.ldy)), rsB = make_rsrc(d.X, (unsigned)((long long)K * d.ldx));
  unsigned avo[2], bvo[2];
  {
    const int kr = lane >> 4, p = lane & 15;
#pragma unroll
    for (int qo = 0; qo < 2; ++qo) {
      const int key = ((4 * qo + kr) & 7) | (((w >> 1) & 1) << 3);
      avo[qo] = (unsigned)((long long)(16 * w + kr) * d.ldy + m0 + ((p ^ key) << 4));
      bvo[qo] = (unsigned)((long long)(16 * w + kr) * d.ldx + n0 + ((p ^ key) << 4));
    }
  }
  const unsigned aqs = (unsigned)(4 * d.ldy), bqs = (unsigned)(4 * d.ldx), ajs = (unsigned)(128 * d.ldy), bjs = (unsigned)(128 * d.ldx);
  const unsigned lds0 = (unsigned)(size_t)LDS_PTR(char, smem);
  const unsigned ldsW = lds0 + (unsigned)(w * PP) * 1024u;
  auto dma_a = [&](int slot_, int j, int q) { lds_dma16u(rsA, avo[q & 1] + ((unsigned)j * ajs + (unsigned)q * aqs), ldsW + (unsigned)(slot_ * UNIT + q * 1024)); };
  auto dma_b = [&](int slot_, int j, int q) { lds_dma16u(rsB, bvo[q & 1] + ((unsigned)j * bjs + (unsigned)q * bqs), ldsW + (unsigned)(slot_ * UNIT + q * 1024)); };
  f4_t acc[FM][FN];
#pragma unroll
  for (int i = 0; i < FM; ++i)
#pragma unroll
    for (int j = 0; j < FN; ++j) acc[i][j] = f4_t{0.f, 0.f, 0.f, 0.f};
  const int wm = (w / NWN) * WM, wn = (w % NWN) * WN;
  const int kx = (t >> 1) | ((g & 1) << 3);
  const int ra0 = (32 * g + (t >> 1)) * 256 + ((((wm >> 4)) ^ kx) << 4) + (t & 1) * 8;
  const int rb0 = (32 * g + (t >> 1)) * 256 + ((((wn >> 4)) ^ kx) << 4) + (t & 1) * 8;
  uint2 fa[FM][4], fb[FN][4];
#pragma unroll
  for (int i = 0; i < FM; ++i)
#pragma unroll
    for (int r = 0; r < 4; ++r) fa[i][r] = make_uint2(0u, 0u);
#pragma unroll
  for (int j = 0; j < FN; ++j)
#pragma unroll
    for (int r = 0; r < 4; ++r) fb[j][r] = make_uint2(0u, 0u);
  auto read_frag = [&](int slot_, int base, int i, uint2 (&f)[4]) {
    const unsigned a = lds0 + (unsigned)(slot_ * UNIT) + (unsigned)(base ^ (i << 4));
    asm volatile("ds_read_b64_tr_b8 %0, %1" : "+v"(f[0]) : "v"(a));
    asm volatile("ds_read_b64_tr_b8 %0, %1 offset:2048" : "+v"(f[1]) : "v"(a));
    asm volatile("ds_read_b64_tr_b8 %0, %1 offset:4096" : "+v"(f[2]) : "v"(a));
    asm volatile("ds_read_b64_tr_b8 %0, %1 offset:6144" : "+v"(f[3]) : "v"(a));
  };
  auto read_a = [&](int slot_, auto ic) { constexpr int i = decltype(ic)::value; read_frag(slot_, ra0, i, fa[i]); };
  auto read_b = [&](int slot_, auto jc) { constexpr int j = decltype(jc)::value; read_frag(slot_, rb0, j, fb[j]); };
  auto join8 = [](const uint2 (&f)[4]) { return i8v_t{(int)f[0].x, (int)f[0].y, (int)f[1].x, (int)f[1].y, (int)f[2].x, (int)f[2].y, (int)f[3].x, (int)f[3].y}; };
  const int nsteps = kt_end - kt_begin, U = 2 * nsteps;
  const int issued0 = min(NUNIT - 1, U - 1);
#pragma unroll
  for (int u = 0; u < NUNIT; ++u)
    if (u <= issued0) {
// ... 10 lines not shown
#define FP8_MMA(i, j) acc[i][j] = __builtin_amdgcn_mfma_scale_f32_16x16x128_f8f6f4(join8(fb[j]), join8(fa[i]), acc[i][j], 0, 1, 0, 0x7f7f7f7f, 0, 0x7f7f7f7f)
  auto step = [&](int j, int sl, auto mode_tag) {
    constexpr int MODE = decltype(mode_tag)::value;
    constexpr bool more = MODE < 3;
    if (MODE <= 1) asm volatile("s_waitcnt vmcnt(%0)" ::"n"(PP) : "memory"); else asm volatile("s_waitcnt vmcnt(0)" ::: "memory");
    asm volatile("s_waitcnt lgkmcnt(0)" ::: "memory");
    __builtin_amdgcn_s_barrier();
    __builtin_amdgcn_sched_barrier(0);
    const int sb_cur = nxt(sl, 1), sa = nxt(sl, 2), sb = nxt(sl, 3);
    static_for<FM - 2>([&](auto ic) {
      constexpr int i = decltype(ic)::value;
#pragma unroll
      for (int jj = 0; jj < FN; ++jj) FP8_MMA(i, jj);
      if (more) read_a(sa, ic);
      if (i < PP) { if (MODE <= 1) dma_b(sl, kt_begin + j + 2, i); }
      else if (MODE == 0) dma_a(sb_cur, kt_begin + j + 3, i - PP);
      __builtin_amdgcn_sched_barrier(0);
    });
    static_for<FN>([&](auto jc) {
      constexpr int jj = decltype(jc)::value;
      FP8_MMA(FM - 2, jj); FP8_MMA(FM - 1, jj);
      if (more) read_b(sb, jc);
      if (MODE == 0 && jj + (FM - 2 - PP) < PP) dma_a(sb_cur, kt_begin + j + 3, jj + (FM - 2 - PP));
      __builtin_amdgcn_sched_barrier(0);
    });
    if (more) { read_a(sa, std::integral_constant<int, FM - 2>{}); read_a(sa, std::integral_constant<int, FM - 1>{}); }
    __builtin_amdgcn_sched_barrier(0);
  };
  int j = 0, sl = 0;
  for (; j < nsteps - 3; ++j, sl = nxt(sl, 2)) step(j, sl, std::integral_constant<int, 0>{});
  if (nsteps >= 3) { step(j, sl, std::integral_constant<int, 1>{}); ++j; sl = nxt(sl, 2); }
  if (nsteps >= 2) { step(j, sl, std::integral_constant<int, 2>{}); ++j; sl = nxt(sl, 2); }
  step(j, sl, std::integral_constant<int, 3>{});
#undef FP8_MMA
  const float alpha = (d.dq_y ? d.dq_y[0] : 1.f) * (d.dq_x ? d.dq_x[0] : 1.f);
#pragma unroll
  for (int i = 0; i < FM; ++i)
#pragma unroll
    for (int jj = 0; jj < FN; ++jj) acc[i][jj] *= alpha;
  constexpr int ESTR = WN + 4, LPR = WN / 4, RPP = 64 / LPR, EROWS = 32;
  float* ew = reinterpret_cast<float*>(smem) + w * (EROWS * ESTR);
  GemmArgs p;
  p.A = nullptr; p.B = nullptr; p.C = d.dW; p.bias = nullptr; p.aux = nullptr; p.resid = d.dW; p.lda = p.ldb = 0; p.ldc = d.N; p.ldaux = 0; p.ldr = d.N;
  p.M = d.M; p.N = d.N; p.K = K; p.c_dtype = CSMAE_F32; p.epi = EPI_RESID; p.splitk = nsplit; p.tiles_m = 0; p.tiles_n = d.tiles_n; p.ktiles = 0; p.ktiles_per_split = 0;
  p.a_bytes = p.b_bytes = 0; p.force_cfg = 0; p.split_stride = 0; p.colsum = d.db; p.dq_a = p.dq_b = nullptr; p.a_fmt = 0; p.aux_q8 = 0; p.q_out = nullptr;
  __syncthreads();
  if (nsplit > 1) {
    GemmArgs q = p;
    q.M = 256; q.N = 256; q.ldc = 256;
    float* mine = slab + ((long long)split * nslots + slot) * (256 * 256);
    epilogue_rows<float, EPI_NONE, FM, FN, WM, EROWS, ESTR, LPR, RPP>(q, mine, acc, ew, wm, wn, lane, t, g);
    return;
  }
  epilogue_rows<float, EPI_RESID, FM, FN, WM, EROWS, ESTR, LPR, RPP>(p, d.dW, acc, ew, m0 + wm, n0 + wn, lane, t, g);
}

__global__ __launch_bounds__(512, 1) void gemm_fp8_dw_group_kernel(Dw8GroupArgs ga) {
  const int wg = xcd_remap(blockIdx.x, ga.total_tiles * ga.nsplit);
  const int split = wg / ga.total_tiles, tile_id = wg - split * ga.total_tiles;
  Dw8Desc d = ga.d[0];
#pragma unroll
  for (int i = 1; i < DW_GROUP_MAX; ++i) if (i < ga.n && tile_id >= ga.d[i].tile0) d = ga.d[i];
  const int tile = tile_id - d.tile0;
  const int tm = tile / d.tiles_n, tn = tile - tm * d.tiles_n;
  const int kt_begin = split * ga.ktiles_per_split;
  const int kt_end = min(kt_begin + ga.ktiles_per_split, ga.ktiles);
  __shared__ __attribute__((aligned(16))) char smem[5 * 128 * 256];
fp8_dw_tile(smem, d, ga.K, tm, tn, split, kt_begin, kt_end, ga.slab, ga.nsplit, tile_id, ga.total_tiles);
}
__global__ __launch_bounds__(256) void fp8_dw_group_reduce_kernel(Dw8GroupArgs ga) {
  const int tile_id = blockIdx.x / DWR_PARTS, quarter = blockIdx.x % DWR_PARTS;
  Dw8Desc d = ga.d[0];
#pragma unroll
  for (int i = 1; i < DW_GROUP_MAX; ++i) if (i < ga.n && tile_id >= ga.d[i].tile0) d = ga.d[i];
  const int tile = tile_id - d.tile0;
  const int tm = tile / d.tiles_n, tn = tile - tm * d.tiles_n;
  const int m0 = tm * 256, n0 = tn * 256;
  const int c4 = threadIdx.x & 63, r0 = threadIdx.x >> 6;
  const long long sstride = (long long)ga.total_tiles * 256 * 256;
  const float* base = ga.slab + (long long)tile_id * 256 * 256;
  const int n = n0 + c4 * 4;
  constexpr int RPB = 256 / DWR_PARTS;
#pragma unroll 1
  for (int r = quarter * RPB + r0; r < quarter * RPB + RPB; r += 4) {
    const int m = m0 + r;
    if (m >= d.M || n >= d.N) continue;
    float* dst = d.dW + (long long)m * d.N + n;
    f4_t a = *reinterpret_cast<f4_t*>(dst);
    for (int sl = 0; sl < ga.nsplit; ++sl) a += *reinterpret_cast<const f4_t*>(base + sl * sstride + r * 256 + c4 * 4);
    *reinterpret_cast<f4_t*>(dst) = a;
  }
}

#define CS_RB 64
__global__ __launch_bounds__(256) void fp8_colsum_partial_kernel(Dw8GroupArgs ga, float* __restrict__ part , int pitch) {
  const Dw8Desc d = ga.d[blockIdx.z];
  if (d.db == nullptr || (int)blockIdx.x * 256 >= d.M) return;
  __shared__ float red[16][256 + 4];
  const int cg = threadIdx.x & 15, rl = threadIdx.x >> 4;
  const int col = blockIdx.x * 256 + cg * 16;
  const long long rows_per = ((long long)ga.K + CS_RB - 1) / CS_RB, r0 = (long long)blockIdx.y * rows_per, r1 = r0 + rows_per < ga.K ? r0 + rows_per : ga.K;
  float s[16];
#pragma unroll
  for (int e = 0; e < 16; ++e) s[e] = 0.f;
  if (col < d.ldy) {
    const unsigned char* src = reinterpret_cast<const unsigned char*>(d.dY) + col;
    auto add16 = [&](const uint4& v) {
      const unsigned wv[4] = {v.x, v.y, v.z, v.w};
#pragma unroll
      for (int q = 0; q < 4; ++q) {
        const auto lo = __builtin_amdgcn_cvt_pk_f32_bf8((int)wv[q], false), hi = __builtin_amdgcn_cvt_pk_f32_bf8((int)wv[q], true);
        s[4 * q] += lo[0]; s[4 * q + 1] += lo[1]; s[4 * q + 2] += hi[0]; s[4 * q + 3] += hi[1];
      }
    };
    long long r = r0 + rl;
    for (; r + 48 < r1; r += 64) {
      const uint4 v0 = *reinterpret_cast<const uint4*>(src + r * d.ldy), v1 = *reinterpret_cast<const uint4*>(src + (r + 16) * d.ldy);
      const uint4 v2 = *reinterpret_cast<const uint4*>(src + (r + 32) * d.ldy), v3 = *reinterpret_cast<const uint4*>(src + (r + 48) * d.ldy);
      add16(v0); add16(v1); add16(v2); add16(v3);
    }
    for (; r < r1; r += 16) add16(*reinterpret_cast<const uint4*>(src + r * d.ldy));
  }
#pragma unroll
  for (int e = 0; e < 16; ++e) red[rl][cg * 16 + e] = s[e];
  __syncthreads();
  float a = 0.f;
#pragma unroll
  for (int k = 0; k < 16; ++k) a += red[k][threadIdx.x];
  part[((long long)blockIdx.z * CS_RB + blockIdx.y) * pitch + blockIdx.x * 256 + threadIdx.x] = a;
}
__global__ __launch_bounds__(256) void fp8_colsum_fold_kernel(Dw8GroupArgs ga, const float* __restrict__ part, int pitch) {
  const Dw8Desc d = ga.d[blockIdx.z];
  const int m = blockIdx.x * 256 + threadIdx.x;
  if (d.db == nullptr || m >= d.M) return;
  const float* src = part + (long long)blockIdx.z * CS_RB * pitch + m;
  float a0 = 0.f, a1 = 0.f, a2 = 0.f, a3 = 0.f;
#pragma unroll 4
  for (int rb = 0; rb < CS_RB; rb += 4) {
    a0 += src[(long long)rb * pitch]; a1 += src[(long long)(rb + 1) * pitch]; a2 += src[(long long)(rb + 2) * pitch]; a3 += src[(long long)(rb + 3) * pitch];
  }
  d.db[m] += ((a0 + a1) + (a2 + a3)) * (d.dq_y ? d.dq_y[0] : 1.f);
}

extern "C" int csmae_gemm_dw_group_fp8(int count, long long K, const void* const* dY, const long long* ldy, const float* const* dq_y, const void* const* X,
                                       const long long* ldx, const float* const* dq_x, float* const* dW, float* const* db, const long long* M, const long long* N,
                                       int slots, float* workspace, long long ws_elems, void* stream) {
  CSMAE_REQUIRE(count > 0 && count <= DW_GROUP_MAX && K > 0 && dY && X && dW && M && N && ldy && ldx && dq_y && dq_x && workspace, "csmae_gemm_dw_group_fp8: bad arguments (1..%d products)", DW_GROUP_MAX);
  Dw8GroupArgs ga;
  int tiles = 0;
  for (int i = 0; i < count; ++i) {
    CSMAE_REQUIRE(M[i] >= 256 && N[i] >= 256 && N[i] % 4 == 0 && ldy[i] % 16 == 0 && ldx[i] % 16 == 0 && ldy[i] >= (M[i] + 15) / 16 * 16 && ldx[i] >= (N[i] + 15) / 16 * 16 &&
                  (K + 128) * ldy[i] < 0xFFFFFFF0ll && (K + 128) * ldx[i] < 0xFFFFFFF0ll && ((((uintptr_t)dY[i] | (uintptr_t)X[i] | (uintptr_t)dW[i]) & 15) == 0),
                  "csmae_gemm_dw_group_fp8: product %d: need M, N >= 256, N %% 4 == 0, rows of 16-byte multiples covering the rounded-up widths, 16-byte aligned operands", i);
    Dw8Desc& d = ga.d[i];
    d.dY = dY[i]; d.X = X[i]; d.dW = dW[i]; d.db = db ? db[i] : nullptr; d.dq_y = dq_y[i]; d.dq_x = dq_x[i]; d.M = (int)M[i]; d.N = (int)N[i]; d.ldy = ldy[i]; d.ldx = ldx[i];
    d.tiles_n = cdiv(N[i], 256); d.tile0 = tiles;
    tiles += cdiv(M[i], 256) * d.tiles_n;
  }
  for (int i = count; i < DW_GROUP_MAX; ++i) ga.d[i] = ga.d[0];
  ga.n = count; ga.K = (int)K; ga.total_tiles = tiles;
  ga.ktiles = cdiv(K, 128);
  if (slots <= 0) slots = 128;
  long long S = slots / tiles;
  if (S > ga.ktiles / 4) S = ga.ktiles / 4;
  const long long per_slice = (long long)tiles * (256 * 256);
  if (S > ws_elems / per_slice) S = ws_elems / per_slice;
  if (S < 1) S = 1;
  ga.ktiles_per_split = cdiv(ga.ktiles, S);
  ga.nsplit = cdiv(ga.ktiles, ga.ktiles_per_split);
  ga.slab = workspace; ga.cs_slab = nullptr;
  CSMAE_REQUIRE(ga.nsplit == 1 || ws_elems >= ga.nsplit * per_slice, "csmae_gemm_dw_group_fp8: workspace too small");
  hipLaunchKernelGGL(gemm_fp8_dw_group_kernel, dim3(tiles * ga.nsplit), dim3(512), 0, (hipStream_t)stream, ga);
  if (ga.nsplit > 1) hipLaunchKernelGGL(fp8_dw_group_reduce_kernel, dim3(tiles * DWR_PARTS), dim3(256), 0, (hipStream_t)stream, ga);
  if (db) {
    int maxM = 0; bool any = false;
    for (int i = 0; i < count; ++i) if (db[i]) { any = true; if (M[i] > maxM) maxM = (int)M[i]; }
    if (any) {
      const int pitch = cdiv(maxM, 256) * 256;
      float* part = workspace + (long long)ga.nsplit * per_slice;
      CSMAE_REQUIRE(ws_elems >= (long long)ga.nsplit * per_slice + (long long)count * CS_RB * pitch, "csmae_gemm_dw_group_fp8: workspace too small for the bias-gradient partial sums");
      hipLaunchKernelGGL(fp8_colsum_partial_kernel, dim3(pitch / 256, CS_RB, count), dim3(256), 0, (hipStream_t)stream, ga, part, pitch);
      hipLaunchKernelGGL(fp8_colsum_fold_kernel, dim3(pitch / 256, 1, count), dim3(256), 0, (hipStream_t)stream, ga, part, pitch);
    }
  }
  return csmae_check_launch("csmae_gemm_dw_group_fp8");
}
```

### cross-scale-mae_amd/csrc/gemm_k2.hip

```cpp
#include "gemm_common.h"
#ifdef GEMM_TIMING
extern "C" int csmae_debug_k2_ts(unsigned long long* out) { return (int)hipMemcpyFromSymbol(out, HIP_SYMBOL(g_gemm_ts), sizeof(g_gemm_ts)); }
#endif

#ifndef K2_ABL
#define K2_ABL 0
#endif
template <bool TB>
__device__ __forceinline__ void k2_tile(const GemmArgs& p, const int tm, const int tn) {
  constexpr int WM = 128, WN = 64, NW = 4, FM = 8, FN = 4;
  constexpr int ASLOT = 128 * 64 * 2, BSLOT = 64 * 32 * 2, BWAVE = 3 * BSLOT, BBASE = 2 * ASLOT;
  __shared__ __attribute__((aligned(16))) char smem[BBASE + NW * BWAVE];
  const int lane = threadIdx.x & 63, w = __builtin_amdgcn_readfirstlane(threadIdx.x >> 6);
  const int t = lane & 15, g = lane >> 4;
  const int m0 = tm * 128, n0 = tn * 256, wn = w * WN;
  GTS(0);
  const i4_t rsA = make_rsrc(p.A, p.a_bytes), rsB = make_rsrc(p.B, p.b_bytes);
  const int l3 = lane >> 3;
  const unsigned avo = (unsigned)(((long long)(m0 + w * 32 + l3) * p.lda + ((lane & 7) ^ l3) * 8) * 2);
  const unsigned aqs = (unsigned)(8 * p.lda * 2);
  unsigned bvo[2], bqs, bhs;
  if (!TB) {
    const int r = lane >> 2, c = (lane & 3) ^ ((r >> 1) & 3);
    bvo[0] = bvo[1] = (unsigned)(((long long)(n0 + wn + r) * 32 + c * 8) * 2);
// ... 202 lines not shown
}
extern "C" int csmae_gemm_ks(int dtype, long long M, long long N, long long K, const void* A, long long lda, const void* Bk, long long slab_rows,
                             const void* B_plain, long long ldb_plain, void* C, long long ldc, int c_dtype, const float* bias, int epilogue,
                             void* aux, long long ldaux, const void* resid, long long ldr, void* stream) {
  if (!ks_taken(dtype, M, N, K, A, lda, Bk, slab_rows, C, ldc, epilogue)) {
    CSMAE_REQUIRE(B_plain != nullptr, "csmae_gemm_ks: shape not taken by the K-slab kernel and no plain weight given (M=%lld N=%lld K=%lld)", M, N, K);
    return gemm_core(dtype, 0, 0, M, N, K, A, lda, B_plain, ldb_plain, C, ldc, c_dtype, bias, epilogue, aux, ldaux, resid, ldr, 1, stream);
  }
  const int q8 = (epilogue == EPI_GELU_Q8 || epilogue == EPI_DGELU_Q8);
  if (q8) epilogue = epilogue == EPI_GELU_Q8 ? EPI_GELU : EPI_DGELU;
  CSMAE_REQUIRE(!q8 || c_dtype == CSMAE_BF16, "csmae_gemm_ks: the 8-bit gelu' epilogues write bf16");
  CSMAE_REQUIRE(epilogue >= EPI_NONE && epilogue <= EPI_DGELU, "csmae_gemm_ks: bad epilogue %d", epilogue);
  CSMAE_REQUIRE(!(epilogue == EPI_GELU || epilogue == EPI_DGELU) || (aux && ldaux % 4 == 0), "csmae_gemm_ks: gelu epilogues need aux");
  CSMAE_REQUIRE(epilogue != EPI_RESID || (resid && ldr % 4 == 0), "csmae_gemm_ks: residual epilogue needs resid");
  GemmArgs p;
  p.force_cfg = 0; p.split_stride = 0; p.colsum = nullptr; p.dq_a = p.dq_b = nullptr; p.a_fmt = 0; p.aux_q8 = q8; p.q_out = nullptr;
  p.A = A; p.B = Bk; p.C = C; p.bias = (epilogue >= EPI_DGELU) ? nullptr : bias; p.aux = aux; p.resid = resid;
  p.lda = lda; p.ldb = slab_rows; p.ldc = ldc; p.ldaux = ldaux; p.ldr = ldr;
  p.M = (int)M; p.N = (int)N; p.K = (int)K; p.c_dtype = c_dtype; p.epi = epilogue; p.splitk = 1;
  p.a_bytes = (unsigned)(M * lda * 2); p.b_bytes = (unsigned)((K / 32) * slab_rows * 64);
  p.ktiles = (int)(K / 64); p.ktiles_per_split = p.ktiles;
  p.tiles_m = cdiv(M, 128); p.tiles_n = cdiv(N, 256);
  if (c_dtype == CSMAE_BF16 && N % 8 == 0 && ldc % 8 == 0 && (M + 256) * ldc * 2 < 0xFFFFFFF0ll && (epilogue != EPI_RESID || (M + 256) * ldr * 2 < 0xFFFFFFF0ll) &&
      ((epilogue != EPI_GELU && epilogue != EPI_DGELU) || (M + 256) * ldaux * 2 < 0xFFFFFFF0ll) && !csmae_debug_opt("epi_pointers"))
    p.a_fmt |= 256;
  p.split_stride = k2_stagger_sleeps(p.ktiles, p.epi);
  CSMAE_LAUNCH((gemm_bf16_k2_kernel<false>), dim3(p.tiles_m * p.tiles_n), dim3(256), 0, (hipStream_t)stream, p);
  return csmae_check_launch("csmae_gemm_ks");
}
__global__ __launch_bounds__(256) void weights_kslab_kernel(const long long* __restrict__ desc, const bf16_t* __restrict__ src, bf16_t* __restrict__ dst) {
  const long long off = desc[blockIdx.y * 3 + 0];
  const int N = (int)desc[blockIdx.y * 3 + 1], K = (int)desc[blockIdx.y * 3 + 2];
  const int kb2 = K / 64, nblk = (N + 31) / 32;
  __shared__ uint4 tile[32][9];
  for (int b = blockIdx.x; b < nblk * kb2; b += gridDim.x) {
    const int nb = b / kb2, k2 = b - nb * kb2;
    const int r = threadIdx.x >> 3, c = threadIdx.x & 7, n = nb * 32 + r;
    __syncthreads();
    if (n < N) tile[r][c] = *reinterpret_cast<const uint4*>(src + off + (long long)n * K + k2 * 64 + c * 8);
    __syncthreads();
    const int h = threadIdx.x >> 7, ro = (threadIdx.x >> 2) & 31, co = threadIdx.x & 3, no = nb * 32 + ro;
    if (no < N) *reinterpret_cast<uint4*>(dst + off + ((long long)(2 * k2 + h) * N + no) * 32 + co * 8) = tile[ro][h * 4 + co];
  }
}
extern "C" int csmae_weights_kslab(int count, const long long* desc, int max_blocks, const void* src_bf16, void* dst_bf16, void* stream) {
  CSMAE_REQUIRE(count > 0 && desc && src_bf16 && dst_bf16 && max_blocks > 0, "csmae_weights_kslab: bad arguments");
  hipLaunchKernelGGL(weights_kslab_kernel, dim3((unsigned)max_blocks, (unsigned)count), dim3(256), 0, (hipStream_t)stream, desc,
                     reinterpret_cast<const bf16_t*>(src_bf16), reinterpret_cast<bf16_t*>(dst_bf16));
  return csmae_check_launch("csmae_weights_kslab");
}


#ifdef CSMAE_K2_DW
struct DwFold2 { float* slab; float* cs_slab; int nsplit; int slot; int nslots; };
#define K2_LDS_BYTES (2 * 64 * 128 * 2 + 4 * 3 * 32 * 64 * 2)
template <bool CS>
__device__ __forceinline__ void k2_tile_tn(char* smem, const GemmArgs& p, const int tm, const int tn, const int split, const int kt_begin, const int kt_end, const DwFold2 fold) {
  constexpr int WM = 128, WN = 64, NW = 4, FM = 8, FN = 4;
  constexpr int ASLOT = 64 * 128 * 2, BSLOT = 32 * 64 * 2, BWAVE = 3 * BSLOT, BBASE = 2 * ASLOT;
  static_assert(BBASE + NW * BWAVE == K2_LDS_BYTES, "LDS layout");
  const int lane = threadIdx.x & 63, w = __builtin_amdgcn_readfirstlane(threadIdx.x >> 6);
  const int t = lane & 15, g = lane >> 4;
  const int m0 = tm * 128, n0 = tn * 256, wn = w * WN;
  GTS(0);
  const i4_t rsA = make_rsrc(p.A, p.a_bytes), rsB = make_rsrc(p.B, p.b_bytes);
  unsigned avo[2], bvo[2];
  {
    const int kr = lane >> 4, ch = lane & 15;
#pragma unroll
    for (int qq = 0; qq < 2; ++qq) {
      const int key = kr | (qq << 2);
      avo[qq] = (unsigned)(((long long)(w * 16 + kr) * p.lda + m0 + ((((ch >> 1) ^ key) << 1) | (ch & 1)) * 8) * 2);
    }
  }
  {
    const int kr = lane >> 3, ch = lane & 7;
#pragma unroll
    for (int qo = 0; qo < 2; ++qo) {
      const int key = ((kr >> 1) & 1) | (qo << 1);
      bvo[qo] = (unsigned)(((long long)kr * p.ldb + n0 + wn + ((((ch >> 1) ^ key) << 1) | (ch & 1)) * 8) * 2);
    }
  }
  const unsigned aqs = (unsigned)(4 * p.lda * 2), ajs = (unsigned)(64 * p.lda * 2), bqs = (unsigned)(8 * p.ldb * 2), bhs = (unsigned)(32 * p.ldb * 2);
  const unsigned lds0 = (unsigned)(size_t)LDS_PTR(char, smem);
  const unsigned ldsA = lds0 + (unsigned)(w * 4) * 1024u, ldsB = lds0 + (unsigned)(BBASE + w * BWAVE);
  auto dma_a = [&](int slot, int j, int q) {
    lds_dma16u(rsA, avo[q >> 1] + ((unsigned)j * ajs + (unsigned)q * aqs), ldsA + (unsigned)(slot * ASLOT + q * 1024));
  };
  auto dma_b = [&](int slot, int u, int q) {
    lds_dma16u(rsB, bvo[q & 1] + ((unsigned)u * bhs + (unsigned)q * bqs), ldsB + (unsigned)(slot * BSLOT + q * 1024));
  };
  f4_t acc[FM][FN];
#pragma unroll
  for (int i = 0; i < FM; ++i)
#pragma unroll
    for (int jj = 0; jj < FN; ++jj) acc[i][jj] = f4_t{0.f, 0.f, 0.f, 0.f};
  const int ra0 = (8 * g + (t >> 2)) * 256 + (((t >> 2) | ((g & 1) << 2)) << 5) + (t & 3) * 8;
  const int rb0 = (8 * g + (t >> 2)) * 128 + ((((t >> 3) & 1) | ((g & 1) << 1)) << 5) + (t & 3) * 8;
  s4_t alo[FM], ahi[FM], b0lo[FN], b0hi[FN], b1lo[FN], b1hi[FN];
#pragma unroll
  for (int i = 0; i < FM; ++i) { alo[i] = s4_t{0, 0, 0, 0}; ahi[i] = s4_t{0, 0, 0, 0}; }
  auto read_a2 = [&](int slot, int h, int i, s4_t& lo, s4_t& hi) {
    const unsigned addr = lds0 + (unsigned)(slot * ASLOT) + (unsigned)((ra0 ^ (i << 5)) + h * 8192);
    asm volatile("ds_read_b64_tr_b16 %0, %1" : "+v"(lo) : "v"(addr));
    asm volatile("ds_read_b64_tr_b16 %0, %1 offset:1024" : "+v"(hi) : "v"(addr));
  };
  auto read_a = [&](int slot, int h, auto ic) { constexpr int i = decltype(ic)::value; read_a2(slot, h, i, alo[i], ahi[i]); };
// ... 64 lines not shown
      else if (r < 8) read_a(sa, 1, std::integral_constant<int, r - 4>{});
      else if (r < 12) read_a(sa, 1, std::integral_constant<int, r - 4>{});
      if (r == 0) read_b(sb1, b1lo, b1hi);
      if (r == 8 && more) {
        asm volatile("s_waitcnt vmcnt(8)" ::: "memory");
        read_b(sb2, b0lo, b0hi);
      }
      if (r == 13) {
        if (MODE == 0) asm volatile("s_waitcnt vmcnt(8)" ::: "memory"); else if (MODE == 2) asm volatile("s_waitcnt vmcnt(4)" ::: "memory");
        asm volatile("s_waitcnt lgkmcnt(0)" ::: "memory");
        if (more) {
          __builtin_amdgcn_s_barrier();
          __builtin_amdgcn_sched_barrier(0);
          read_a(sa ^ 1, 0, std::integral_constant<int, 0>{}); read_a(sa ^ 1, 0, std::integral_constant<int, 1>{});
        }
      }
      if (r == 14 && more) read_a(sa ^ 1, 0, std::integral_constant<int, 2>{});
      if (r == 15 && more) read_a(sa ^ 1, 0, std::integral_constant<int, 3>{});
      if (more && r < 8 && (r & 1)) dma_b(sb, 2 * ja + 3, r >> 1);
      if (MODE == 0 && r >= 9 && r <= 12) dma_b(sb1, 2 * ja + 4, r - 9);
      if (MODE == 0 && r >= 14) { dma_a(sa, ja + 2, 2 * (r - 14)); dma_a(sa, ja + 2, 2 * (r - 14) + 1); }
      __builtin_amdgcn_sched_barrier(0);
    });
  };
  int j = 0, sa = 0, sb = 0;
  for (; j < nsteps - 2; ++j, sa ^= 1, sb = nx3(sb, 2)) step(j, sa, sb, std::integral_constant<int, 0>{});
  if (nsteps >= 2) { step(j, sa, sb, std::integral_constant<int, 2>{}); ++j; sa ^= 1; sb = nx3(sb, 2); }
  step(j, sa, sb, std::integral_constant<int, 3>{});
  GTS(2);
  asm volatile("s_waitcnt lgkmcnt(0)" ::: "memory");
  if (do_cs) {
#pragma unroll
    for (int e = 0; e < 2; ++e) { float v = cs[e]; v += __shfl_xor(v, 16); v += __shfl_xor(v, 32); cs[e] = v; }
  }
  constexpr int ESTR = WN + 4, LPR = WN / 4, RPP = 64 / LPR, EROWS = 32;
  float* ew = reinterpret_cast<float*>(smem + BBASE + w * BWAVE);
  if (fold.nsplit > 1) {
    if (do_cs && g == 0) {
      float* csm = fold.cs_slab + ((long long)split * fold.nslots + fold.slot) * 128;
      csm[(2 * w) * 16 + t] = cs[0];
      csm[(2 * w + 1) * 16 + t] = cs[1];
    }
    GemmArgs q = p;
    q.M = 128; q.N = 256; q.ldc = 256; q.bias = nullptr;
    float* mine = fold.slab + ((long long)split * fold.nslots + fold.slot) * (128 * 256);
    epilogue_rows<float, EPI_NONE, FM, FN, WM, EROWS, ESTR, LPR, RPP>(q, mine, acc, ew, 0, wn, lane, t, g);
    GTS(3);
    return;
  }
  if (do_cs && g == 0) {
#pragma unroll
    for (int e = 0; e < 2; ++e) {
      const int m = m0 + (2 * w + e) * 16 + t;
      if (m < p.M) p.colsum[m] += cs[e];
    }
  }
  epilogue_rows<float, EPI_RESID, FM, FN, WM, EROWS, ESTR, LPR, RPP>(p, p.C, acc, ew, m0, n0 + wn, lane, t, g);
  GTS(3);
}
__global__ __launch_bounds__(256, 2) void gemm_dw_group_k2_kernel(DwGroupArgs ga) {
  const int wg = xcd_remap(blockIdx.x, ga.total_tiles * ga.nsplit);
  const int split = wg / ga.total_tiles, tile_id = wg - split * ga.total_tiles;
  DwDesc d = ga.d[0];
#pragma unroll
  for (int i = 1; i < DW_GROUP_MAX; ++i) if (i < ga.n && tile_id >= ga.d[i].tile0) d = ga.d[i];
  const int tile = tile_id - d.tile0;
  const int tm = tile / d.tiles_n, tn = tile - tm * d.tiles_n;
  const int kt_begin = split * ga.ktiles_per_split;
  const int kt_end = min(kt_begin + ga.ktiles_per_split, ga.ktiles);
  GemmArgs p;
  p.A = d.dY; p.B = d.X; p.C = d.dW; p.bias = nullptr; p.aux = nullptr; p.resid = d.dW;
  p.lda = d.ldy; p.ldb = d.ldx; p.ldc = d.N; p.ldaux = 0; p.ldr = d.N;
  p.M = d.M; p.N = d.N; p.K = ga.K;
  p.c_dtype = CSMAE_F32; p.epi = EPI_RESID; p.splitk = ga.nsplit; p.tiles_m = 0; p.tiles_n = d.tiles_n; p.ktiles = ga.ktiles; p.ktiles_per_split = ga.ktiles_per_split;
  p.a_bytes = (unsigned)((long long)ga.K * d.ldy * 2); p.b_bytes = (unsigned)((long long)ga.K * d.ldx * 2);
  p.force_cfg = 0; p.split_stride = 0; p.colsum = d.db; p.dq_a = p.dq_b = nullptr; p.a_fmt = 0; p.aux_q8 = 0; p.q_out = nullptr;
  __shared__ __attribute__((aligned(16))) char smem[K2_LDS_BYTES];
  const DwFold2 fold{ga.slab, ga.cs_slab, ga.nsplit, tile_id, ga.total_tiles};
  if (d.db != nullptr && tn == 0) k2_tile_tn<true>(smem, p, tm, tn, split, kt_begin, kt_end, fold);
  else k2_tile_tn<false>(smem, p, tm, tn, split, kt_begin, kt_end, fold);
}
__global__ __launch_bounds__(256) void dw_group_reduce_k2_kernel(DwGroupArgs ga) {
  const int tile_id = blockIdx.x / DWR_PARTS, part = blockIdx.x % DWR_PARTS;
  DwDesc d = ga.d[0];
#pragma unroll
  for (int i = 1; i < DW_GROUP_MAX; ++i) if (i < ga.n && tile_id >= ga.d[i].tile0) d = ga.d[i];
  const int tile = tile_id - d.tile0;
  const int tm = tile / d.tiles_n, tn = tile - tm * d.tiles_n;
  const int m0 = tm * 128, n0 = tn * 256;
  const int c4 = threadIdx.x & 63, r0 = threadIdx.x >> 6;
  const long long sstride = (long long)ga.total_tiles * 128 * 256;
  const float* base = ga.slab + (long long)tile_id * 128 * 256;
  const int n = n0 + c4 * 4;
  constexpr int RPB = 128 / DWR_PARTS;
#pragma unroll
  for (int r = part * RPB + r0; r < part * RPB + RPB; r += 4) {
    const int m = m0 + r;
    if (m >= d.M || n >= d.N) continue;
    float* dst = d.dW + (long long)m * d.N + n;
    f4_t a = *reinterpret_cast<f4_t*>(dst);
    for (int sl = 0; sl < ga.nsplit; ++sl) a += *reinterpret_cast<const f4_t*>(base + sl * sstride + r * 256 + c4 * 4);
    *reinterpret_cast<f4_t*>(dst) = a;
  }
  if (part == 0 && tn == 0 && d.db != nullptr && threadIdx.x < 128) {
    const int m = m0 + threadIdx.x;
    if (m < d.M) {
      float a = d.db[m];
      for (int sl = 0; sl < ga.nsplit; ++sl) a += ga.cs_slab[((long long)sl * ga.total_tiles + tile_id) * 128 + threadIdx.x];
      d.db[m] = a;
    }
  }
}
int gemm_k2_launch_dw(DwGroupArgs& ga, int count, int slots, float* workspace, long long ws_elems, hipStream_t st) {
  int tiles = 0;
  for (int i = 0; i < count; ++i) {
    DwDesc& d = ga.d[i];
    d.tiles_n = cdiv(d.N, 256); d.tile0 = tiles;
    tiles += cdiv(d.M, 128) * d.tiles_n;
  }
  for (int i = count; i < DW_GROUP_MAX; ++i) ga.d[i] = ga.d[0];
  ga.total_tiles = tiles;
  long long S = (2LL * slots) / tiles;
  if (S > ga.ktiles / 8) S = ga.ktiles / 8;
  const long long per_slice = (long long)tiles * (128 * 256 + 128);
  if (S > ws_elems / per_slice) S = ws_elems / per_slice;
  if (S < 1) S = 1;
  ga.ktiles_per_split = cdiv(ga.ktiles, S);
  ga.nsplit = cdiv(ga.ktiles, ga.ktiles_per_split);
  ga.slab = workspace; ga.cs_slab = workspace + (long long)ga.nsplit * tiles * 128 * 256;
  if (ga.nsplit > 1 && ws_elems < ga.nsplit * per_slice) { csmae_set_error("csmae_gemm_dw_group: workspace too small"); return CSMAE_ERR_ARG; }
  hipLaunchKernelGGL(gemm_dw_group_k2_kernel, dim3(tiles * ga.nsplit), dim3(256), 0, st, ga);
  if (ga.nsplit > 1) hipLaunchKernelGGL(dw_group_reduce_k2_kernel, dim3(tiles * DWR_PARTS), dim3(256), 0, st, ga);
  return csmae_check_launch("csmae_gemm_dw_group");
}
#else
int gemm_k2_launch_dw(DwGroupArgs&, int, int, float*, long long, hipStream_t) {
  csmae_set_error("csmae_gemm_dw_group: the two-workgroups-per-CU weight-gradient kernel is not in this build (-DCSMAE_K2_DW)");
  return CSMAE_ERR_UNSUPPORTED;
}
#endif
bool gemm_k2_dw_built() {
#ifdef CSMAE_K2_DW
  return true;
#else
  return false;
#endif
}
```

### cross-scale-mae_amd/csrc/optim.hip

```cpp
#include "common.h"

__global__ __launch_bounds__(256) void adamw_kernel(const long long* __restrict__ tile_off, const int* __restrict__ tile_cnt,
                                                    const float* __restrict__ tile_wd, float* __restrict__ p, const float* __restrict__ g,
                                                    float* __restrict__ m, float* __restrict__ v, float lr, float b1, float b2, float eps,
                                                    float bc1, float bc2, bf16_t* __restrict__ p_lp, const float* __restrict__ gate,
                                                    const long long* __restrict__ tile_ks, bf16_t* __restrict__ p_ks) {
  if (gate != nullptr && !isfinite(gate[0])) return;
  const long long off = tile_off[blockIdx.x];
  const int cnt = tile_cnt[blockIdx.x];
  const float wd = tile_wd[blockIdx.x];
  const float step_size = lr / bc1, rbc2 = 1.f / sqrtf(bc2), decay = 1.f - lr * wd;
  long long wbase = 0; int ksN = 0, ksK = 0;
  if (tile_ks != nullptr && p_ks != nullptr) { wbase = tile_ks[blockIdx.x * 3]; ksN = (int)tile_ks[blockIdx.x * 3 + 1]; ksK = (int)tile_ks[blockIdx.x * 3 + 2]; }
  for (int i = threadIdx.x * 4; i < cnt; i += blockDim.x * 4) {
    if (i + 4 <= cnt && ((off + i) & 3) == 0) {
      f4_t pp = *reinterpret_cast<f4_t*>(p + off + i), gg = *reinterpret_cast<const f4_t*>(g + off + i);
      f4_t mm = *reinterpret_cast<f4_t*>(m + off + i), vv = *reinterpret_cast<f4_t*>(v + off + i);
#pragma unroll
      for (int k = 0; k < 4; ++k) {
        pp[k] *= decay;
        mm[k] = mm[k] + (1.f - b1) * (gg[k] - mm[k]);
        vv[k] = b2 * vv[k] + (1.f - b2) * gg[k] * gg[k];
        pp[k] -= step_size * (mm[k] / (sqrtf(vv[k]) * rbc2 + eps));
      }
      *reinterpret_cast<f4_t*>(p + off + i) = pp; *reinterpret_cast<f4_t*>(m + off + i) = mm; *reinterpret_cast<f4_t*>(v + off + i) = vv;
      if (p_lp) st4<bf16_t>(p_lp + off + i, pp);
      if (ksK) {
        const long long e = off + i - wbase;
        const int n = (int)(e / ksK), k = (int)(e - (long long)n * ksK);
        if ((k & 3) == 0 && k + 4 <= ksK) st4<bf16_t>(p_ks + wbase + ((long long)(k >> 5) * ksN + n) * 32 + (k & 31), pp);
        else {
#pragma unroll
          for (int q = 0; q < 4; ++q) {
            const long long eq = e + q;
            const int nq = (int)(eq / ksK), kq = (int)(eq - (long long)nq * ksK);
            p_ks[wbase + ((long long)(kq >> 5) * ksN + nq) * 32 + (kq & 31)] = f2bf(pp[q]);
          }
        }
      }
    } else {
      for (int k = i; k < cnt && k < i + 4; ++k) {
        float pp = p[off + k] * decay, gg = g[off + k];
        float mm = m[off + k] + (1.f - b1) * (gg - m[off + k]);
        float vv = b2 * v[off + k] + (1.f - b2) * gg * gg;
        pp -= step_size * (mm / (sqrtf(vv) * rbc2 + eps));
        p[off + k] = pp; m[off + k] = mm; v[off + k] = vv;
        if (p_lp) p_lp[off + k] = f2bf(pp);
        if (ksK) {
          const long long e = off + k - wbase;
          const int n = (int)(e / ksK), kk = (int)(e - (long long)n * ksK);
          p_ks[wbase + ((long long)(kk >> 5) * ksN + n) * 32 + (kk & 31)] = f2bf(pp);
        }
      }
    }
  }
}
extern "C" int csmae_adamw(long long ntiles, const long long* tile_off, const int* tile_cnt, const float* tile_wd, float* p, const float* g,
                           float* m, float* v, float lr, float beta1, float beta2, float eps, float bias_correction1, float bias_correction2,
                           void* p_lp, const float* gate, const long long* tile_ks, void* p_ks, void* stream) {
  CSMAE_REQUIRE(ntiles > 0 && tile_off && tile_cnt && tile_wd && p && g && m && v, "csmae_adamw: null argument");
  CSMAE_REQUIRE(bias_correction1 > 0.f && bias_correction2 > 0.f, "csmae_adamw: bias corrections must be positive (step >= 1)");
  hipLaunchKernelGGL(adamw_kernel, dim3((unsigned)ntiles), dim3(256), 0, (hipStream_t)stream, tile_off, tile_cnt, tile_wd, p, g, m, v, lr, beta1, beta2, eps,
                     bias_correction1, bias_correction2, (bf16_t*)p_lp, gate, tile_ks, (bf16_t*)p_ks);
  return csmae_check_launch("csmae_adamw");
}

__global__ __launch_bounds__(256) void adamw_f8_kernel(const long long* __restrict__ tile8, float wd, float* __restrict__ p, const float* __restrict__ g, float* __restrict__ m,
                                                       float* __restrict__ v, float lr, float b1, float b2, float eps, float bc1, float bc2, bf16_t* __restrict__ p_lp,
                                                       const float* __restrict__ gate, unsigned char* __restrict__ w8, unsigned char* __restrict__ w8t,
                                                       const float* __restrict__ amax_prev, float* __restrict__ amax_next, float* __restrict__ dq) {
  const long long* t = tile8 + (long long)blockIdx.x * 6;
  const long long wbase = t[0];
  const int N = (int)t[1], K = (int)t[2], n0 = (int)t[3], k0 = (int)t[4], wi = (int)t[5];
  const int lane = threadIdx.x & 63;
  const float am = wave_max(amax_prev[(long long)wi * 64 + lane]);
  if (gate != nullptr && !isfinite(gate[0])) {
    if (n0 == 0 && k0 == 0 && threadIdx.x == 0 && am > 0.f) atomicMax(reinterpret_cast<unsigned*>(amax_next) + (long long)wi * 64, __float_as_uint(am));
    return;
  }
  __shared__ unsigned q8[64][17];
  __shared__ float red[4];
  const float scale = am > 0.f ? 448.0f / am : 1.f;
  if (n0 == 0 && k0 == 0 && threadIdx.x == 0) dq[wi] = am > 0.f ? am / 448.0f : 1.f;
  const float step_size = lr / bc1, rbc2 = 1.f / sqrtf(bc2), decay = 1.f - lr * wd;
  const int c4 = (threadIdx.x & 15) * 4, r0 = threadIdx.x >> 4;
  float seen = 0.f;
#pragma unroll
  for (int pass = 0; pass < 4; ++pass) {
    const int r = pass * 16 + r0;
    const long long e = wbase + (long long)(n0 + r) * K + k0 + c4;
    f4_t pp = *reinterpret_cast<f4_t*>(p + e), gg = *reinterpret_cast<const f4_t*>(g + e);
    f4_t mm = *reinterpret_cast<f4_t*>(m + e), vv = *reinterpret_cast<f4_t*>(v + e);
#pragma unroll
    for (int k = 0; k < 4; ++k) {
      pp[k] *= decay;
      mm[k] = mm[k] + (1.f - b1) * (gg[k] - mm[k]);
      vv[k] = b2 * vv[k] + (1.f - b2) * gg[k] * gg[k];
      pp[k] -= step_size * (mm[k] / (sqrtf(vv[k]) * rbc2 + eps));
      const float a = fabsf(pp[k]);
      seen = fmaxf(seen, a == a ? a : INFINITY);
    }
    *reinterpret_cast<f4_t*>(p + e) = pp; *reinterpret_cast<f4_t*>(m + e) = mm; *reinterpret_cast<f4_t*>(v + e) = vv;
    if (p_lp) st4<bf16_t>(p_lp + e, pp);
    f4_t q = pp * scale;
#pragma unroll
    for (int k = 0; k < 4; ++k) q[k] = q[k] != q[k] ? q[k] : fminf(fmaxf(q[k], -448.0f), 448.0f);
    int w = 0;
    w = __builtin_amdgcn_cvt_pk_fp8_f32(q[0], q[1], w, false); w = __builtin_amdgcn_cvt_pk_fp8_f32(q[2], q[3], w, true);
    *reinterpret_cast<unsigned*>(w8 + e) = (unsigned)w;
    q8[r][c4 >> 2] = (unsigned)w;
  }
  __syncthreads();
  const unsigned char* qb = reinterpret_cast<const unsigned char*>(&q8[0][0]);
#pragma unroll
  for (int pass = 0; pass < 4; ++pass) {
    const int c = pass * 16 + r0, r4 = (threadIdx.x & 15) * 4;
    const unsigned b0 = qb[(r4 + 0) * 68 + c], b1_ = qb[(r4 + 1) * 68 + c], b2_ = qb[(r4 + 2) * 68 + c], b3 = qb[(r4 + 3) * 68 + c];
    *reinterpret_cast<unsigned*>(w8t + wbase + (long long)(k0 + c) * N + n0 + r4) = b0 | (b1_ << 8) | (b2_ << 16) | (b3 << 24);
  }
// ... 125 lines not shown
```

### include/csmae.h

```cpp
#ifndef CSMAE_H
#define CSMAE_H
#ifdef __cplusplus
extern "C" {
#endif

#define CSMAE_F32 0
#define CSMAE_BF16 1

enum csmae_status { CSMAE_OK = 0, CSMAE_ERR_ARG = -1, CSMAE_ERR_LAUNCH = -2, CSMAE_ERR_UNSUPPORTED = -3 };
enum csmae_epilogue { CSMAE_EPI_NONE = 0, CSMAE_EPI_GELU = 1, CSMAE_EPI_RESID = 2, CSMAE_EPI_DGELU = 3, CSMAE_EPI_ATOMIC = 4, CSMAE_EPI_SPLIT = 5,
                      CSMAE_EPI_GELU_Q8 = 6, CSMAE_EPI_DGELU_Q8 = 7  };
enum csmae_loss { CSMAE_LOSS_MSE = 0, CSMAE_LOSS_L2 = 1, CSMAE_LOSS_MAE = 2, CSMAE_LOSS_L1 = 3, CSMAE_LOSS_BCE = 4 };

const char* csmae_last_error(void);
int csmae_abi_version(void);
const char* csmae_source_hash(void);

int csmae_next_launch_event(void* hip_event);
int csmae_flush_launch_event(void* stream);

int csmae_gemm(int dtype, int transA, int transB, long long M, long long N, long long K,
               const void* A, long long lda, const void* B, long long ldb, void* C, long long ldc, int c_dtype,
               const float* bias, int epilogue, void* aux, long long ldaux, const void* resid , long long ldr,
               int splitk, void* stream);

int csmae_gemm_ks(int dtype, long long M, long long N, long long K, const void* A, long long lda, const void* Bk, long long slab_rows,
                  const void* B_plain, long long ldb_plain, void* C, long long ldc, int c_dtype, const float* bias, int epilogue,
                  void* aux, long long ldaux, const void* resid, long long ldr, void* stream);
int csmae_weights_kslab(int count, const long long* desc, int max_blocks, const void* src_bf16, void* dst_bf16, void* stream);
int csmae_gemm_ln_supported(long long M, long long N, long long K);
int csmae_gemm_ln_fwd(long long M, long long N, long long K, const void* A, long long lda, const void* Bk, long long slab_rows,
                      const float* bias, const void* resid, long long ldr, void* X, long long ldx, const float* gamma, const float* beta,
                      float eps, void* Y, long long ldy, float* mean, float* rstd, void* stream);
int csmae_gemm_ln_bwd(long long M, long long N, long long K, const void* dY, long long lda, const void* W, long long ldb,
                      const void* x, long long ldx, const float* mean, const float* rstd, const float* gamma, const void* dres_in, long long ldd,
                      void* dx_out, long long ldo, float* partial_ws, long long partial_elems, void* stream);
int csmae_gemm_k2_mode(int nn, int nt);
int csmae_gemm_dw_mode(int k2);

int csmae_gemm_dw(int dtype, long long M, long long N, long long K, const void* dY, long long ldy, const void* X, long long ldx,
                  float* dW, float* db, float* workspace, long long ws_elems, void* stream);
int csmae_gemm_dw_group(int dtype, int count, long long K, const void* const* dY, const long long* ldy, const void* const* X,
                        const long long* ldx, float* const* dW, float* const* db, const long long* M, const long long* N, int slots,
                        float* workspace, long long ws_elems, void* stream);
int csmae_gemm_dw_group_fp8(int count, long long K, const void* const* dY, const long long* ldy, const float* const* dq_y, const void* const* X,
                            const long long* ldx, const float* const* dq_x, float* const* dW, float* const* db, const long long* M, const long long* N,
                            int slots, float* workspace, long long ws_elems, void* stream);
int csmae_fp8_amax(int in_dtype, long long rows, int cols, const void* src, long long ld, float* amax, void* stream);
int csmae_fp8_quantize(int in_dtype, int fmt, int transpose, long long rows, int cols, const void* src, long long ld, void* dst,
                       long long ldd, const float* amax, float* dq, float* amax_next , void* stream);
int csmae_fp8_weights(int count, const long long* desc, const float* p, void* w8, void* w8t, float* amax, float* dq, void* stream);
int csmae_gemm_fp8(int a_fmt, long long M, long long N, long long K, const void* A, long long lda, const void* B, long long ldb,
                   void* C, long long ldc, int c_dtype, const float* bias, int epilogue, void* aux, long long ldaux,
                   const void* resid, long long ldr, const float* dq_a, const float* dq_b,
                   void* q_out ,
                   long long ldq, int q_fmt, const float* q_amax_prev , float* q_amax_next , float* q_dq, void* stream);
int csmae_gemm_force_tile(int cfg);
#define CSMAE_GEMM_ROUTE_F32 7
#define CSMAE_GEMM_ROUTE_KSLAB 8
int csmae_gemm_route(int dtype, int transA, int transB, long long M, long long N, long long K, long long lda, long long ldb, long long ldc,
                     int epilogue, int splitk);
int csmae_gemm_ks_route(int dtype, long long M, long long N, long long K, const void* A, long long lda, const void* Bk, long long slab_rows,
                        long long ldb_plain, const void* C, long long ldc, int epilogue);

int csmae_attn_fwd(int dtype, long long B, int T, int H, int hd, const void* qkv, void* out, float* lse, void* stream);
int csmae_attn_bwd(int dtype, long long B, int T, int H, int hd, const void* qkv, const void* out, const void* dout,
                   const float* lse, void* dqkv, void* stream);
#define CSMAE_ATTN_ROUTE_RESIDENT 0
#define CSMAE_ATTN_ROUTE_STREAM 1
#define CSMAE_ATTN_ROUTE_ANY 2
#define CSMAE_ATTN_ROUTE_F32 3
int csmae_attn_route(int dtype, int T, int hd);
int csmae_attn_stream_mode(int mode);
int csmae_attn_resident(int dtype, int T, int hd);
int csmae_attn_fwd_q(int dtype, long long B, int T, int H, int hd, const void* qkv, void* out, float* lse, void* q_out, int q_fmt,
                     const float* q_amax_prev, float* q_amax_next, float* q_dq, void* stream);
int csmae_attn_bwd_q(int dtype, long long B, int T, int H, int hd, const void* qkv, const void* out, const void* dout, const float* lse,
                     void* dqkv, void* q_out, int q_fmt, const float* q_amax_prev, float* q_amax_next, float* q_dq, void* stream);

int csmae_layernorm_fwd(int x_dtype, int out_dtype, long long M, int D, const void* x, const float* gamma, const float* beta, float eps,
                        void* y, float* y32, float* mean, float* rstd, void* q_out, int q_fmt, const float* q_amax_prev,
                        float* q_amax_next, float* q_dq, void* stream);
int csmae_layernorm_bwd(int dy_dtype, int x_dtype, int lp_dtype, long long M, int D, const void* dy, const void* x, const float* mean,
                        const float* rstd, const float* gamma, const void* dres_in, void* dx_out, void* dx_lp,
                        float* dgamma, float* dbeta, float* partial_ws, long long partial_elems, void* q_out, int q_fmt,
                        const float* q_amax_prev, float* q_amax_next, float* q_dq, void* stream);
int csmae_ln_param_reduce(int count, long long M, int D, const float* partials, long long stride, long long slice_elems,
                          float* gbase, const long long* goff, void* stream);
int csmae_ln_param_reduce_rows(int count, int rows, int D, const float* partials, long long stride, float* gbase, const long long* goff, void* stream);

int csmae_bnrelu_fwd(int dtype, int N, int L, int Hp, const void* u, const float* gamma, const float* beta, float eps,
                     float momentum, void* r, float* mean, float* rstd, float* running_mean, float* running_var,
                     long long* num_batches_tracked, int training, void* stream);
int csmae_bnrelu_bwd(int dtype, int N, int L, int Hp, const void* u, const void* dr, const float* gamma, const float* beta,
                     const float* mean, const float* rstd, void* du, float* dgamma, float* dbeta, void* stream);

int csmae_crop_resize(long long planes, int S, const float* src, float* dst, const int* box, void* stream);
int csmae_mask_sort(long long rows, int L, int keep, const float* noise, long long* ids_restore, float* mask, int* ids_keep,
                    int* ids_shuffle, void* stream);
int csmae_patch_gather(int dtype, long long rows, int keep, int N, int C, int S, int p, const float* img0, const float* img1,
// ... 7 lines not shown
                        float* dmask_token, void* stream);
int csmae_rows_gather(int dtype, long long rows, int D, const float* src, long long group, long long gstride, long long off,
                      void* dst, void* stream);
int csmae_rows_scatter_add(int dtype, long long rows, int D, const void* src, float scale, long long group, long long gstride,
                           long long off, float* dst, void* stream);
int csmae_rows_scatter_add2(int dtype, long long rows, int D, const void* a, float scale_a, long long off_a, const void* b, float scale_b, long long off_b,
                            long long group, long long gstride, float* dst, void* stream);
int csmae_spec_fixup(const float* g, void* b0, long long n0, void* b1, long long n1, void* b2, long long n2, const float* tmp_dgamma, const float* tmp_dbeta,
                     float* dgamma, float* dbeta, int L, void* stream);
int csmae_rows_gather_idx(long long N, int L, int keep, int D, const float* x, const int* ids, long long ids_ld, float* out, void* stream);

int csmae_target_minmax(int norm_pix, long long B2, int N, int C, int S, int p, const float* img0, const float* img1,
                        float* scratch, float* out, void* stream);
int csmae_recon_loss_fwd(int kind, int norm_pix, int pred_dtype, long long B2, int N, int C, int S, int p, const float* img0, const float* img1,
                         const void* pred, long long ldp, const float* minmax, const float* mask, float* rowloss, void* stream);
int csmae_recon_loss_bwd(int kind, int norm_pix, int out_dtype, int pred_dtype, long long B2, int N, int C, int S, int p, const float* img0,
                         const float* img1, const void* pred, long long ldp, const float* minmax, const float* mask,
                         const float* losses, const float* gout, float vscale, const float* extra, void* dpred, long long ldd,
                         void* stream);
int csmae_ssim_workspace_floats(long long B2, int C, int S, int p, int levels, long long* floats );
int csmae_ssim_fwd(int levels, int flags , int norm_pix,
                   long long B2, int N, int C, int S, int p, const float* img0, const float* img1, const float* pred, long long ldp,
                   const float* mask, float* ws, float* terms, void* stream);
int csmae_ssim_apply(int pure, int views, float weight, float recon_scale, const float* terms, float* losses, void* stream);
int csmae_ssim_bwd(int levels, long long B2, int N, int C, int S, int p, const float* pred, long long ldp, const float* mask,
                   const float* gout, float scale, float* ws, float* extra, void* stream);
int csmae_pair_loss_fwd(int kind, long long rows, int D, const float* a, long long a_group, long long a_gstride, long long a_off,
                        const float* t, long long t_group, long long t_gstride, long long t_off, float* partial, void* stream);
int csmae_pair_loss_bwd(int kind, int lp_dtype, long long rows, int D, const float* a, long long a_group, long long a_gstride,
                        long long a_off, const float* t, long long t_group, long long t_gstride, long long t_off,
                        const float* gout, float coef, void* da_lp, float* da_acc, float* dt_acc, void* stream);
int csmae_ntxent_fwd(int N, int Te, int keep, int D, const float* latent, float tau, float eps, float* z, float* inv_norm,
                     float* E, float* neg, float* rowloss, void* stream);
int csmae_ntxent_bwd(int N, int D, const float* z, const float* inv_norm, const float* E, const float* neg, float tau, float eps,
                     const float* gout, float* dpool, void* stream);
int csmae_latent_grad_finish(int lp_dtype, long long B2, int Te, int D, float* dlat, const float* dpool, float inv_keep,
                             void* dlat_lp, void* stream);
int csmae_loss_finalize(long long per_view, int views, const float* rowloss, const float* mask, float recon_scale,
                        const float* cd_partial, float cd_scale, const float* e_partial, float e_scale,
                        const float* ce_rowloss, int ce_rows, float* losses, void* stream);

int csmae_augment_u8(long long N, int C, int Hmax, int Wmax, int S, const unsigned char* src, const int* meta, const float* mean,
                     const float* inv_std, float* dst, void* stream);
int csmae_eval_u8(long long N, int C, int Hmax, int Wmax, int S, const unsigned char* src, const int* meta, const float* mean,
                  const float* inv_std, float* dst, void* stream);
int csmae_augment_u16(long long N, int Cin, int Cout, int Hmax, int Wmax, int S, const unsigned short* src, const int* meta,
                      const int* band, const float* mean, const float* inv_std, float* dst, void* stream);
int csmae_eval_u16(long long N, int Cin, int Cout, int Hmax, int Wmax, int S, const unsigned short* src, const int* meta,
                   const int* band, const float* mean, const float* inv_std, float* dst, void* stream);

int csmae_adamw(long long ntiles, const long long* tile_off, const int* tile_cnt, const float* tile_wd, float* p, const float* g,
                float* m, float* v, float lr, float beta1, float beta2, float eps, float bias_correction1, float bias_correction2,
                void* p_lp, const float* gate, const long long* tile_ks, void* p_ks, void* stream);
int csmae_adamw_fp8(long long ntiles, const long long* tile8, float weight_decay, float* p, const float* g, float* m, float* v, float lr, float beta1,
                    float beta2, float eps, float bias_correction1, float bias_correction2, void* p_lp, const float* gate, void* w8, void* w8t,
                    const float* amax_prev, float* amax_next, float* dq, void* stream);
int csmae_gate_accumulate(const float* loss, float* slot, int accumulate, void* stream);
int csmae_clip_grad_norm(long long n, float* g, float max_norm, float* scratch, float* out, void* stream);
int csmae_cast_f32_to_bf16(long long n, const float* src, void* dst, void* stream);
int csmae_cast_bf16_to_f32(long long n, const void* src, float* dst, void* stream);
int csmae_colsum(int dtype, long long M, int N, const void* x, long long ld, float* out, void* stream);

int csmae_probe_pool_fwd(int dtype, int global_pool, long long N, int T, int D, const void* x, const float* gamma, const float* beta, float eps,
                         float* feat, void* stream);
int csmae_bn1d_fwd(long long N, int D, const float* feat, float eps, float momentum, float* fbn, float* running_mean, float* running_var,
                   long long* num_batches_tracked, int training, void* stream);
int csmae_head_linear_fwd(long long N, int D, int K, const float* x, const float* w, const float* b, float* logits, void* stream);
int csmae_head_linear_bwd(long long N, int D, int K, const float* dlogits, const float* x, const float* gscale, float* dw, float* db, int accumulate,
                          void* stream);
int csmae_softmax_ce(long long N, int K, const float* logits, const long long* labels, const float* gout, float* scratch, float* loss, float* dlogits,
                     float* counts, int accumulate_counts, void* stream);
int csmae_lars_step(int ntensors, const long long* table, float lr, float weight_decay, float momentum, float trust, float* norms, const float* gate,
                    void* stream);

int csmae_probe_pool_bwd(int dtype, int global_pool, long long N, int T, int D, const void* x, const float* dfeat, const float* gamma, float eps,
                         void* dres, float* partial, float* dgamma, float* dbeta, int accumulate, void* stream);
int csmae_head_linear_dx(long long N, int D, int K, const float* dlogits, const float* w, const float* gscale, float* dx, void* stream);
int csmae_soft_ce(long long N, int K, const float* logits, const float* target, const float* gout, float* scratch, float* loss, float* dlogits,
                  void* stream);
int csmae_mixup_target(long long N, int K, const long long* labels, float lam, float smoothing, float* target, void* stream);
int csmae_mixup_cutmix(int cutmix, long long N, int C, int H, int W, const float* x, float* out, float lam, int yl, int yh, int xl, int xh,
                       void* stream);
int csmae_pos_embed_grad(int dtype, long long N, int T, int D, const void* dres, float* dpos, int accumulate, void* stream);

int csmae_l2_normalize(int in_dtype, int out_dtype, long long rows, int D, const void* src, long long ld, float eps, void* dst, void* stream);
int csmae_knn_select(long long Q, int Bc, int k, const float* sim, long long ld, long long base, float* val, int* idx, void* stream);
int csmae_knn_vote(long long Q, int k, int K, const float* val, const int* idx, const long long* bank_labels, float inv_T, float* votes, int* top5,
                   float* counts, const long long* query_labels, int accumulate_counts, void* stream);

int csmae_recon_eval_workspace_floats(long long N, int C, int S, long long* floats );
int csmae_recon_eval(int pred_dtype, long long N, int C, int S, int p, const float* img, const void* pred, long long ldp, long long img_stride,
                     const float* mean, const float* std, float* part, float* out, void* stream);

int csmae_recon_panel(int pred_dtype, long long N, int C, int S, int p, const float* img, const void* pred, long long ldp, long long img_stride,
                      const float* mask, const float* mean, const float* std, int band_r, int band_g, int band_b, int panel0, int panel1, int panel2,
                      int panel3, int panel4, int n_panels, int gap, unsigned char* out, void* stream);


int csmae_stream_create_cu_mask(int words, const unsigned* mask, void** out);
int csmae_stream_destroy(void* stream);

#ifdef __cplusplus
}
#endif
#endif
```

Baseline: 6041 images/s.

## Overwrite linear weight gradients in dW kernels instead of zero-then-accumulate

The full gradient buffer is no longer zeroed before backward. Only ranges outside the main linear layers (qkv, proj, fc1, fc2, decoder embed/pred, predictor) are cleared, using a new multi-range zero kernel. The first dW group write to those slots stores directly instead of doing a read-modify-write, which saves a memset and a read pass over most of the gradient memory. Bookkeeping tracks which slots are still fresh, raises an error on mixed groups, and zeroes any fresh slots left unwritten at the end.

```diff
diff --git a/cross-scale-mae_amd/csmae_hip/__init__.py b/cross-scale-mae_amd/csmae_hip/__init__.py
--- a/cross-scale-mae_amd/csmae_hip/__init__.py
+++ b/cross-scale-mae_amd/csmae_hip/__init__.py
@@ -20,7 +20,7 @@
                      "csmae_head_linear_bwd", "csmae_softmax_ce", "csmae_lars_step", "csmae_probe_pool_bwd", "csmae_head_linear_dx", "csmae_soft_ce",
                      "csmae_mixup_target", "csmae_mixup_cutmix", "csmae_pos_embed_grad", "csmae_eval_u8", "csmae_l2_normalize", "csmae_knn_select",
                      "csmae_knn_vote", "csmae_recon_eval", "csmae_recon_eval_workspace_floats", "csmae_recon_panel", "csmae_augment_u16",
-                     "csmae_eval_u16")
+                     "csmae_eval_u16", "csmae_gemm_dw_group_ow", "csmae_gemm_dw_group_fp8_ow", "csmae_zero_ranges")
 _HERE = os.path.dirname(os.path.abspath(__file__))
 LIB_PATH = os.environ.get("CSMAE_LIB_PATH") or os.path.join(_HERE, "libcsmae_hip.so")
 
@@ -37,6 +37,9 @@
     "csmae_gemm_dw": [I, L, L, L, P, L, P, L, P, P, P, L, P],
     "csmae_gemm_dw_group": [I, I, L, P, P, P, P, P, P, P, P, I, P, L, P],
     "csmae_gemm_dw_group_fp8": [I, L, P, P, P, P, P, P, P, P, P, P, I, P, L, P],
+    "csmae_gemm_dw_group_ow": [I, I, L, P, P, P, P, P, P, P, P, I, P, L, I, P],
+    "csmae_gemm_dw_group_fp8_ow": [I, L, P, P, P, P, P, P, P, P, P, P, I, P, L, I, P],
+    "csmae_zero_ranges": [I, P, L, P, P],
     "csmae_fp8_amax": [I, L, I, P, L, P, P],
     "csmae_fp8_quantize": [I, I, I, L, I, P, L, P, L, P, P, P, P],
     "csmae_fp8_weights": [I, P, P, P, P, P, P, P],
diff --git a/cross-scale-mae_amd/csmae_hip/engine.py b/cross-scale-mae_amd/csmae_hip/engine.py
--- a/cross-scale-mae_amd/csmae_hip/engine.py
+++ b/cross-scale-mae_amd/csmae_hip/engine.py
@@ -3,6 +3,7 @@
 import contextlib
 import math
 import os
+import re
 import weakref
 from typing import Dict, Optional
 
@@ -21,6 +22,21 @@
 
 def _round_up(x, m):
     return (x + m - 1) // m * m
+
+
+_OW_LINEAR = re.compile(r"^(?:(?:encoder|decoder)\.\d+\.(?:attn\.qkv|attn\.proj|mlp\.fc1|mlp\.fc2)|decoder_embed|decoder_pred|predictor\.[03])$")
+
+
+def clear_ranges(slots, total, skip):
+    holes = sorted((slots[n + sfx][0], slots[n + sfx][1]) for n in skip for sfx in (".weight", ".bias"))
+    out, at = [], 0
+    for off, cnt in holes:
+        if off > at:
+            out.append((at, off - at))
+        at = max(at, off + cnt)
+    if total > at:
+        out.append((at, total - at))
+    return out
 
 
 class FlatParams:
@@ -248,6 +264,10 @@
         self._events, self._ev_i, self._side_reads, self._tog = [], 0, {}, 0
         self._side_seq, self._side_waited = 0, 0
         self._dw_cache = {}
+        self._ow_names = frozenset() if debug_opt("dw_accum") else frozenset(
+            n[:-7] for n in flat.slots if n.endswith(".weight") and _OW_LINEAR.match(n[:-7]) and n[:-7] + ".bias" in flat.slots)
+        self._ow_live = None
+        self._clear_table = None
         for key in ("bwd_main_cus", "main_cus"):
             v = debug_opt(key)
             if v is not None and not (len(v.split(":")) == 2 and all(q.isdigit() for q in v.split(":")) and int(v.split(":")[0]) < int(v.split(":")[1])):
@@ -476,8 +496,16 @@
                 gw2 = gw.view(gw.shape[0], -1)
                 prods.append((dy[:, : gw2.shape[0]], x[:, : gw2.shape[1]], gw2, self.flat.G(name + ".bias")))
             grp = self._dw_cache[key] = ops.DwGroup(prods, self.ws.dw_ws)
+        ow = False
+        if self._ow_live is not None:
+            names = [it[-1] for it in (items8 if items8 is not None else items)]
+            fresh = [n for n in names if n in self._ow_live]
+            if fresh and len(fresh) != len(set(names)):
+                raise RuntimeError(f"_dw_group: {names} mixes gradient slots that were cleared or already written with slots that were not ({fresh})")
+            ow = bool(fresh)
+            self._ow_live.difference_update(fresh)
         if ops._timer is not None or os.environ.get("CSMAE_DW_MAIN"):
-            grp.launch(256, st=self.st)
+            grp.launch(256, st=self.st, overwrite=ow)
             return
         side = self.side
         if ready is not None:
@@ -486,12 +514,22 @@
             ev = self._event()
             ev.record(self.main)
         side.wait_event(ev)
-        grp.launch(slots or self._dw_slots, st=side.cuda_stream)
+        grp.launch(slots or self._dw_slots, st=side.cuda_stream, overwrite=ow)
         done = self._event()
         done.record(side)
         self._side_seq += 1
         for dy, _, _ in items:
             self._side_reads[dy.data_ptr()] = (self._side_seq, done)
+
+    def _clear_grads(self, st=None):
+        if not self._ow_names:
+            self.flat.g[: self.flat.total].zero_()
+            return
+        if self._clear_table is None:
+            rows = clear_ranges(self.flat.slots, self.flat.total, self._ow_names)
+            self._clear_table = (torch.tensor(rows, dtype=torch.int64, device=self.device).reshape(-1, 2), max((c for _, c in rows), default=0))
+        ops.zero_ranges(self._clear_table[0], self._clear_table[1], self.flat.g, st=torch.cuda.current_stream().cuda_stream if st is None else st)
+        self._ow_live = set(self._ow_names)
 
     def _guard_write(self, *bufs):
         last = None
@@ -1011,6 +1049,7 @@
             self.side = self._new_side()
         self._ev_i, self._tog = 0, 0
         self._side_reads.clear()
+        self._ow_live = None
         with trace.range_("csmae.backward.encoder"):
             if not accumulate:
                 self.flat.g[: self.flat.total].zero_()
@@ -1124,14 +1163,15 @@
             self.side = self._new_side()
         self._ev_i, self._tog = 0, 0
         self._side_reads.clear()
+        self._ow_live = None
         zeroed = None
         if not accumulate:
             if ops._timer is not None or os.environ.get("CSMAE_DW_MAIN") or debug_opt("zero_main"):
-                self.flat.g[: self.flat.total].zero_()
+                self._clear_grads()
             else:
                 self.side.wait_stream(self.main)
                 with torch.cuda.stream(self.side):
-                    self.flat.g[: self.flat.total].zero_()
+                    self._clear_grads()
                 zeroed = self._event()
                 zeroed.record(self.side)
         ops.gate_accumulate(ws.losses, self.flat.gate, accumulate, st=st)
@@ -1239,6 +1279,10 @@
         trace.pop()
         if self.fp8:
             ws.fp8_complete = True
+        for name in sorted(self._ow_live or ()):
+            G(name + ".weight").zero_()
+            G(name + ".bias").zero_()
+        self._ow_live = None
         for name, p in self.flat.params.items():
             if p.requires_grad and not name.startswith("encoder_norm."):
                 p.grad = self.flat.grad_views[name]
diff --git a/cross-scale-mae_amd/csmae_hip/ops.py b/cross-scale-mae_amd/csmae_hip/ops.py
--- a/cross-scale-mae_amd/csmae_hip/ops.py
+++ b/cross-scale-mae_amd/csmae_hip/ops.py
@@ -208,6 +208,11 @@
     check(load().csmae_weights_kslab(desc.shape[0], _p(desc), max_blocks, _p(src), _p(dst), _s(st)), "csmae_weights_kslab")
 
 
+def zero_ranges(table, max_count, buf, st=None):
+    assert table.dtype == torch.int64 and table.is_contiguous() and table.dim() == 2 and table.shape[1] == 2 and buf.dtype == torch.float32 and buf.is_contiguous()
+    check(load().csmae_zero_ranges(table.shape[0], _p(table), int(max_count), _p(buf), _s(st)), "csmae_zero_ranges")
+
+
 def gemm_dw(dy, x, dw, workspace, db=None, st=None):
     K, M = dy.shape
     N = x.shape[1]
@@ -274,10 +279,10 @@
             assert dy.shape[0] == self.K and x.shape[0] == self.K and dw.is_contiguous() and dy.dtype == x.dtype and dy.stride(1) == 1 and x.stride(1) == 1
         _dw_group_args(self, products, workspace, 0, 1, 2, 3)
 
-    def launch(self, slots=0, st=None):
+    def launch(self, slots=0, st=None, overwrite=False):
         t = _begin()
-        check(load().csmae_gemm_dw_group(self.dtype, self.n, self.K, self.dY, self.ldy, self.X, self.ldx, self.dW, self.dB, self.M, self.N, slots,
-                                         self.ws, self.ws_n, _s(st)), "csmae_gemm_dw_group")
+        check(load().csmae_gemm_dw_group_ow(self.dtype, self.n, self.K, self.dY, self.ldy, self.X, self.ldx, self.dW, self.dB, self.M, self.N, slots,
+                                            self.ws, self.ws_n, int(overwrite), _s(st)), "csmae_gemm_dw_group_ow")
         if t:
             t.end(("gemm_bf16" if self.dtype == BF16 else "gemm_f32") + "_TN", self.flops)
 
@@ -292,10 +297,10 @@
         _dw_group_args(self, products, workspace, 0, 2, 4, 5)
         self.dqy, self.dqx = ((ctypes.c_void_p * self.n)(*[_p(q[i]) for q in products]) for i in (1, 3))
 
-    def launch(self, slots=0, st=None):
+    def launch(self, slots=0, st=None, overwrite=False):
         t = _begin()
-        check(load().csmae_gemm_dw_group_fp8(self.n, self.K, self.dY, self.ldy, self.dqy, self.X, self.ldx, self.dqx, self.dW, self.dB, self.M, self.N, slots,
-                                             self.ws, self.ws_n, _s(st)), "csmae_gemm_dw_group_fp8")
+        check(load().csmae_gemm_dw_group_fp8_ow(self.n, self.K, self.dY, self.ldy, self.dqy, self.X, self.ldx, self.dqx, self.dW, self.dB, self.M, self.N, slots,
+                                                self.ws, self.ws_n, int(overwrite), _s(st)), "csmae_gemm_dw_group_fp8_ow")
         if t:
             t.end("gemm_fp8_TN", self.flops)
 
diff --git a/cross-scale-mae_amd/csrc/gemm.hip b/cross-scale-mae_amd/csrc/gemm.hip
--- a/cross-scale-mae_amd/csrc/gemm.hip
+++ b/cross-scale-mae_amd/csrc/gemm.hip
@@ -195,7 +195,7 @@
 #ifndef GEMM_ABL
 #define GEMM_ABL 0
 #endif
-struct DwFold { float* slab; float* cs_slab; int nsplit; int slot; int nslots; };
+struct DwFold { float* slab; float* cs_slab; int nsplit; int slot; int nslots; int overwrite; };
 #define K64_LDS_BYTES (5 * 256 * 64 * 2)
 
 template <bool TA, bool TB, int BM, bool GROUP, int CSV = 0>
@@ -415,8 +415,16 @@
 #pragma unroll
       for (int e = 0; e < 2; ++e) {
         const int m = m0 + wm + (2 * wq + e) * 16 + t;
-        if (m < p.M) p.colsum[m] += cs[e];
+        if (m < p.M) p.colsum[m] = (fold.overwrite ? 0.0f : p.colsum[m]) + cs[e];
       }
+    }
+    if (fold.overwrite) {
+#pragma unroll
+      for (int i = 0; i < FM; ++i)
+#pragma unroll
+        for (int jj = 0; jj < FN; ++jj) acc[i][jj] = f4_t{0.f, 0.f, 0.f, 0.f} + acc[i][jj];
+      epilogue_rows<float, EPI_NONE, FM, FN, WM, EROWS, ESTR, LPR, RPP>(p, Cptr, acc, ew, m0 + wm, n0 + wn, lane, t, g);
+      return;
     }
     epilogue_rows<float, EPI_RESID, FM, FN, WM, EROWS, ESTR, LPR, RPP>(p, Cptr, acc, ew, m0 + wm, n0 + wn, lane, t, g);
     return;
@@ -486,7 +494,7 @@
   p.a_bytes = (unsigned)((long long)ga.K * d.ldy * 2); p.b_bytes = (unsigned)((long long)ga.K * d.ldx * 2);
   p.force_cfg = ga.force_cfg; p.split_stride = 0; p.colsum = d.db; p.dq_a = p.dq_b = nullptr; p.a_fmt = 0; p.aux_q8 = 0; p.q_out = nullptr;
   __shared__ __attribute__((aligned(16))) char smem[K64_LDS_BYTES];
-  const DwFold fold{ga.slab, ga.cs_slab, ga.nsplit, tile_id, ga.total_tiles};
+  const DwFold fold{ga.slab, ga.cs_slab, ga.nsplit, tile_id, ga.total_tiles, ga.overwrite};
   if (d.db != nullptr && tn == 0) k64_tile<true, true, 256, true, 2>(smem, p, tm, tn, split, kt_begin, kt_end, fold);
   else k64_tile<true, true, 256, true, 1>(smem, p, tm, tn, split, kt_begin, kt_end, fold);
 }
@@ -502,20 +510,20 @@
   const long long sstride = (long long)ga.total_tiles * 256 * 256;
   const float* base = ga.slab + (long long)tile_id * 256 * 256;
   const int n = n0 + c4 * 4;
-  constexpr int RPB = 256 / DWR_PARTS;
-#pragma unroll
-  for (int r = quarter * RPB + r0; r < quarter * RPB + RPB; r += 4) {
-    const int m = m0 + r;
-    if (m >= d.M || n >= d.N) continue;
-    float* dst = d.dW + (long long)m * d.N + n;
-    f4_t a = *reinterpret_cast<f4_t*>(dst);
-    for (int sl = 0; sl < ga.nsplit; ++sl) a += *reinterpret_cast<const f4_t*>(base + sl * sstride + r * 256 + c4 * 4);
-    *reinterpret_cast<f4_t*>(dst) = a;
-  }
+  constexpr int RPB = 256 / DWR_PARTS, NR = RPB / 4;
+  const int r = quarter * RPB + r0;
+  float* dst[NR]; bool ok[NR];
+#pragma unroll
+  for (int i = 0; i < NR; ++i) {
+    const int m = m0 + r + 4 * i;
+    ok[i] = m < d.M && n < d.N;
+    dst[i] = d.dW + (long long)(ok[i] ? m : 0) * d.N + (ok[i] ? n : 0);
+  }
+  dw_fold_rows<NR>(base + r * 256 + c4 * 4, sstride, 4 * 256, ga.nsplit, dst, ok, ga.overwrite != 0);
   if (quarter == 0 && tn == 0 && d.db != nullptr) {
     const int m = m0 + threadIdx.x;
     if (m < d.M) {
-      float a = d.db[m];
+      float a = ga.overwrite ? 0.0f : d.db[m];
       for (int sl = 0; sl < ga.nsplit; ++sl) a += ga.cs_slab[((long long)sl * ga.total_tiles + tile_id) * 256 + threadIdx.x];
       d.db[m] = a;
     }
@@ -982,36 +990,43 @@
 }
 
 __global__ __launch_bounds__(256) void dw_reduce_kernel(long long n4, int S, long long slab4, const f4_t* __restrict__ ws, f4_t* __restrict__ dw,
-                                                        const float* __restrict__ wsb, float* __restrict__ db, int M) {
+                                                        const float* __restrict__ wsb, float* __restrict__ db, int M, int overwrite) {
   for (long long i = (long long)blockIdx.x * blockDim.x + threadIdx.x; i < n4; i += (long long)gridDim.x * blockDim.x) {
-    f4_t a = dw[i];
+    f4_t a = {0.f, 0.f, 0.f, 0.f};
+    if (!overwrite) a = dw[i];
     for (int s = 0; s < S; ++s) a += ws[s * slab4 + i];
     dw[i] = a;
   }
   if (db && blockIdx.x == 0)
     for (int m = threadIdx.x; m < M; m += blockDim.x) {
-      float a = db[m];
+      float a = overwrite ? 0.0f : db[m];
       for (int s = 0; s < S; ++s) a += wsb[(long long)s * M + m];
       db[m] = a;
     }
 }
-extern "C" int csmae_gemm_dw(int dtype, long long M, long long N, long long K, const void* dY, long long ldy, const void* X, long long ldx,
-                             float* dW, float* db, float* workspace, long long ws_elems, void* stream);
-extern "C" int csmae_gemm_dw_group(int dtype, int count, long long K, const void* const* dY, const long long* ldy, const void* const* X,
-                                   const long long* ldx, float* const* dW, float* const* db, const long long* M, const long long* N, int slots,
-                                   float* workspace, long long ws_elems, void* stream) {
+static int gemm_dw_one(int dtype, long long M, long long N, long long K, const void* dY, long long ldy, const void* X, long long ldx,
+                       float* dW, float* db, float* workspace, long long ws_elems, int overwrite, void* stream);
+static bool gemm_dw_one_ok(int dtype, long long M, long long N, long long K, long long ldy, const float* db, const float* workspace, long long ws_elems) {
+  return M > 0 && N > 0 && K > 0 && N % 4 == 0 && workspace && ws_elems >= M * N + M && (!db || dtype == CSMAE_BF16 || (M % 4 == 0 && ldy % 4 == 0));
+}
+static int gemm_dw_group_core(int dtype, int count, long long K, const void* const* dY, const long long* ldy, const void* const* X,
+                              const long long* ldx, float* const* dW, float* const* db, const long long* M, const long long* N, int slots,
+                              float* workspace, long long ws_elems, int overwrite, void* stream) {
   CSMAE_REQUIRE(count > 0 && count <= DW_GROUP_MAX && K > 0 && dY && X && dW && M && N && ldy && ldx && workspace, "csmae_gemm_dw_group: bad arguments (1..%d products)", DW_GROUP_MAX);
   bool fused = dtype == CSMAE_BF16 && g_force_cfg < 0;
   for (int i = 0; i < count && fused; ++i) fused = M[i] >= 256 && N[i] >= 256 && N[i] % 4 == 0 && ldy[i] % 8 == 0 && ldx[i] % 8 == 0 && ldy[i] >= (M[i] + 7) / 8 * 8 && ldx[i] >= (N[i] + 7) / 8 * 8 &&
                                                    K * ldy[i] * 2 < 0xFFFFFFF0ll && K * ldx[i] * 2 < 0xFFFFFFF0ll && ((((uintptr_t)dY[i] | (uintptr_t)X[i] | (uintptr_t)dW[i]) & 15) == 0);
   if (!fused) {
+    for (int i = 0; i < count; ++i)
+      CSMAE_REQUIRE(gemm_dw_one_ok(dtype, M[i], N[i], K, ldy[i], db ? db[i] : nullptr, workspace, ws_elems), "csmae_gemm_dw_group: product %d: bad arguments / workspace too small", i);
     for (int i = 0; i < count; ++i) {
-      int rc = csmae_gemm_dw(dtype, M[i], N[i], K, dY[i], ldy[i], X[i], ldx[i], dW[i], db ? db[i] : nullptr, workspace, ws_elems, stream);
+      int rc = gemm_dw_one(dtype, M[i], N[i], K, dY[i], ldy[i], X[i], ldx[i], dW[i], db ? db[i] : nullptr, workspace, ws_elems, overwrite, stream);
       if (rc) return rc;
     }
     return CSMAE_OK;
   }
   DwGroupArgs ga;
+  ga.overwrite = overwrite ? 1 : 0;
   if (g_k2_dw) {
     for (int i = 0; i < count; ++i) {
       DwDesc& d = ga.d[i];
@@ -1044,9 +1059,23 @@
   if (ga.nsplit > 1) hipLaunchKernelGGL(dw_group_reduce_kernel, dim3(tiles * DWR_PARTS), dim3(256), 0, (hipStream_t)stream, ga);
   return csmae_check_launch("csmae_gemm_dw_group");
 }
+extern "C" int csmae_gemm_dw_group(int dtype, int count, long long K, const void* const* dY, const long long* ldy, const void* const* X,
+                                   const long long* ldx, float* const* dW, float* const* db, const long long* M, const long long* N, int slots,
+                                   float* workspace, long long ws_elems, void* stream) {
+  return gemm_dw_group_core(dtype, count, K, dY, ldy, X, ldx, dW, db, M, N, slots, workspace, ws_elems, 0, stream);
+}
+extern "C" int csmae_gemm_dw_group_ow(int dtype, int count, long long K, const void* const* dY, const long long* ldy, const void* const* X,
+                                      const long long* ldx, float* const* dW, float* const* db, const long long* M, const long long* N, int slots,
+                                      float* workspace, long long ws_elems, int overwrite, void* stream) {
+  return gemm_dw_group_core(dtype, count, K, dY, ldy, X, ldx, dW, db, M, N, slots, workspace, ws_elems, overwrite, stream);
+}
 extern "C" int csmae_gemm_dw(int dtype, long long M, long long N, long long K, const void* dY, long long ldy, const void* X, long long ldx,
                              float* dW, float* db, float* workspace, long long ws_elems, void* stream) {
-  CSMAE_REQUIRE(M > 0 && N > 0 && K > 0 && N % 4 == 0 && workspace && ws_elems >= M * N + M, "csmae_gemm_dw: bad arguments / workspace too small");
+  return gemm_dw_one(dtype, M, N, K, dY, ldy, X, ldx, dW, db, workspace, ws_elems, 0, stream);
+}
+static int gemm_dw_one(int dtype, long long M, long long N, long long K, const void* dY, long long ldy, const void* X, long long ldx,
+                       float* dW, float* db, float* workspace, long long ws_elems, int overwrite, void* stream) {
+  CSMAE_REQUIRE(gemm_dw_one_ok(dtype, M, N, K, ldy, db, workspace, ws_elems), "csmae_gemm_dw: bad arguments / workspace too small");
   const int tile = dtype == CSMAE_BF16 ? ((M >= 256 && N >= 256) ? 256 : 128) : 64;
   const bool k64 = dtype == CSMAE_BF16 && tile == 256 && (g_force_cfg < 0 || (g_force_cfg & 7) == 4);
   const int kt = dtype == CSMAE_BF16 ? (k64 ? 64 : GEMM_BK) : 16;
@@ -1065,7 +1094,10 @@
   if (rc) return rc;
   const long long n4 = M * N / 4;
   hipLaunchKernelGGL(dw_reduce_kernel, dim3((unsigned)fmin((double)cdiv(n4, 256), 2048.0)), dim3(256), 0, (hipStream_t)stream, n4, (int)S, n4,
-                     reinterpret_cast<const f4_t*>(workspace), reinterpret_cast<f4_t*>(dW), wsb, fused_bias ? db : nullptr, (int)M);
-  if (db && !fused_bias) return csmae_colsum_launch(dtype, K, (int)M, dY, ldy, db, stream);
+                     reinterpret_cast<const f4_t*>(workspace), reinterpret_cast<f4_t*>(dW), wsb, fused_bias ? db : nullptr, (int)M, overwrite ? 1 : 0);
+  if (db && !fused_bias) {
+    if (overwrite && hipMemsetAsync(db, 0, (size_t)M * sizeof(float), (hipStream_t)stream) != hipSuccess) { csmae_set_error("csmae_gemm_dw: clearing db failed"); return CSMAE_ERR_LAUNCH; }
+    return csmae_colsum_launch(dtype, K, (int)M, dY, ldy, db, stream);
+  }
   return csmae_check_launch("csmae_gemm_dw");
 }
diff --git a/cross-scale-mae_amd/csrc/gemm_common.h b/cross-scale-mae_amd/csrc/gemm_common.h
--- a/cross-scale-mae_amd/csrc/gemm_common.h
+++ b/cross-scale-mae_amd/csrc/gemm_common.h
@@ -446,9 +446,40 @@
 struct DwGroupArgs {
   DwDesc d[DW_GROUP_MAX];
   int n, K, ktiles, ktiles_per_split, nsplit, total_tiles, force_cfg;
+  int overwrite;
   float* slab; float* cs_slab;
 };
 #define DWR_PARTS 16
+template <int NR, int NS>
+__device__ __forceinline__ void dw_fold_batch(const float* __restrict__ src, const long long sstride, const int rstep_elems, f4_t (&a)[NR]) {
+  f4_t v[NS][NR];
+#pragma unroll
+  for (int s = 0; s < NS; ++s)
+#pragma unroll
+    for (int i = 0; i < NR; ++i) v[s][i] = *reinterpret_cast<const f4_t*>(src + (long long)s * sstride + (long long)i * rstep_elems);
+#pragma unroll
+  for (int s = 0; s < NS; ++s)
+#pragma unroll
+    for (int i = 0; i < NR; ++i) a[i] += v[s][i];
+}
+template <int NR>
+__device__ __forceinline__ void dw_fold_rows(const float* __restrict__ src, const long long sstride, const int rstep_elems, const int nsplit,
+                                             float* const (&dst)[NR], const bool (&ok)[NR], const bool overwrite) {
+  f4_t a[NR];
+#pragma unroll
+  for (int i = 0; i < NR; ++i) {
+    a[i] = f4_t{0.f, 0.f, 0.f, 0.f};
+    if (!overwrite && ok[i]) a[i] = *reinterpret_cast<const f4_t*>(dst[i]);
+  }
+  int s = 0;
+  for (; s + 8 <= nsplit; s += 8) dw_fold_batch<NR, 8>(src + s * sstride, sstride, rstep_elems, a);
+  if (s + 4 <= nsplit) { dw_fold_batch<NR, 4>(src + s * sstride, sstride, rstep_elems, a); s += 4; }
+  if (s + 2 <= nsplit) { dw_fold_batch<NR, 2>(src + s * sstride, sstride, rstep_elems, a); s += 2; }
+  if (s < nsplit) dw_fold_batch<NR, 1>(src + s * sstride, sstride, rstep_elems, a);
+#pragma unroll
+  for (int i = 0; i < NR; ++i)
+    if (ok[i]) *reinterpret_cast<f4_t*>(dst[i]) = a[i];
+}
 int gemm_k2_launch_dw(DwGroupArgs& ga, int count, int slots, float* workspace, long long ws_elems, hipStream_t st);
 int gemm_force_cfg();
 bool gemm_k2_nn_wanted(int epilogue, long long K, long long N, long long M);
diff --git a/cross-scale-mae_amd/csrc/gemm_fp8_dw.hip b/cross-scale-mae_amd/csrc/gemm_fp8_dw.hip
--- a/cross-scale-mae_amd/csrc/gemm_fp8_dw.hip
+++ b/cross-scale-mae_amd/csrc/gemm_fp8_dw.hip
@@ -5,11 +5,12 @@
 struct Dw8GroupArgs {
   Dw8Desc d[DW_GROUP_MAX];
   int n, K, ktiles, ktiles_per_split, nsplit, total_tiles;
+  int overwrite;
   float* slab; float* cs_slab;
 };
 
 __device__ __forceinline__ void fp8_dw_tile(char* smem, const Dw8Desc& d, const int K, const int tm, const int tn, const int split, const int kt_begin, const int kt_end,
-                                            float* slab, const int nsplit, const int slot, const int nslots) {
+                                            float* slab, const int nsplit, const int slot, const int nslots, const int overwrite) {
   constexpr int WM = 128, WN = 64, NWN = 4, NW = 8, FM = 8, FN = 4, UNIT = 128 * 256, NUNIT = 5, PP = UNIT / 1024 / NW;
   const int lane = threadIdx.x & 63, w = __builtin_amdgcn_readfirstlane(threadIdx.x >> 6);
   const int t = lane & 15, g = lane >> 4;
@@ -126,6 +127,14 @@
     epilogue_rows<float, EPI_NONE, FM, FN, WM, EROWS, ESTR, LPR, RPP>(q, mine, acc, ew, wm, wn, lane, t, g);
     return;
   }
+  if (overwrite) {
+#pragma unroll
+    for (int i = 0; i < FM; ++i)
+#pragma unroll
+      for (int jj = 0; jj < FN; ++jj) acc[i][jj] = f4_t{0.f, 0.f, 0.f, 0.f} + acc[i][jj];
+    epilogue_rows<float, EPI_NONE, FM, FN, WM, EROWS, ESTR, LPR, RPP>(p, d.dW, acc, ew, m0 + wm, n0 + wn, lane, t, g);
+    return;
+  }
   epilogue_rows<float, EPI_RESID, FM, FN, WM, EROWS, ESTR, LPR, RPP>(p, d.dW, acc, ew, m0 + wm, n0 + wn, lane, t, g);
 }
 
@@ -140,7 +149,7 @@
   const int kt_begin = split * ga.ktiles_per_split;
   const int kt_end = min(kt_begin + ga.ktiles_per_split, ga.ktiles);
   __shared__ __attribute__((aligned(16))) char smem[5 * 128 * 256];
-fp8_dw_tile(smem, d, ga.K, tm, tn, split, kt_begin, kt_end, ga.slab, ga.nsplit, tile_id, ga.total_tiles);
+fp8_dw_tile(smem, d, ga.K, tm, tn, split, kt_begin, kt_end, ga.slab, ga.nsplit, tile_id, ga.total_tiles, ga.overwrite);
 }
 __global__ __launch_bounds__(256) void fp8_dw_group_reduce_kernel(Dw8GroupArgs ga) {
   const int tile_id = blockIdx.x / DWR_PARTS, quarter = blockIdx.x % DWR_PARTS;
@@ -154,16 +163,16 @@
   const long long sstride = (long long)ga.total_tiles * 256 * 256;
   const float* base = ga.slab + (long long)tile_id * 256 * 256;
   const int n = n0 + c4 * 4;
-  constexpr int RPB = 256 / DWR_PARTS;
-#pragma unroll 1
-  for (int r = quarter * RPB + r0; r < quarter * RPB + RPB; r += 4) {
-    const int m = m0 + r;
-    if (m >= d.M || n >= d.N) continue;
-    float* dst = d.dW + (long long)m * d.N + n;
-    f4_t a = *reinterpret_cast<f4_t*>(dst);
-    for (int sl = 0; sl < ga.nsplit; ++sl) a += *reinterpret_cast<const f4_t*>(base + sl * sstride + r * 256 + c4 * 4);
-    *reinterpret_cast<f4_t*>(dst) = a;
-  }
+  constexpr int RPB = 256 / DWR_PARTS, NR = RPB / 4;
+  const int r = quarter * RPB + r0;
+  float* dst[NR]; bool ok[NR];
+#pragma unroll
+  for (int i = 0; i < NR; ++i) {
+    const int m = m0 + r + 4 * i;
+    ok[i] = m < d.M && n < d.N;
+    dst[i] = d.dW + (long long)(ok[i] ? m : 0) * d.N + (ok[i] ? n : 0);
+  }
+  dw_fold_rows<NR>(base + r * 256 + c4 * 4, sstride, 4 * 256, ga.nsplit, dst, ok, ga.overwrite != 0);
 }
 
 #define CS_RB 64
@@ -213,12 +222,12 @@
   for (int rb = 0; rb < CS_RB; rb += 4) {
     a0 += src[(long long)rb * pitch]; a1 += src[(long long)(rb + 1) * pitch]; a2 += src[(long long)(rb + 2) * pitch]; a3 += src[(long long)(rb + 3) * pitch];
   }
-  d.db[m] += ((a0 + a1) + (a2 + a3)) * (d.dq_y ? d.dq_y[0] : 1.f);
-}
-
-extern "C" int csmae_gemm_dw_group_fp8(int count, long long K, const void* const* dY, const long long* ldy, const float* const* dq_y, const void* const* X,
-                                       const long long* ldx, const float* const* dq_x, float* const* dW, float* const* db, const long long* M, const long long* N,
-                                       int slots, float* workspace, long long ws_elems, void* stream) {
+  d.db[m] = (ga.overwrite ? 0.0f : d.db[m]) + ((a0 + a1) + (a2 + a3)) * (d.dq_y ? d.dq_y[0] : 1.f);
+}
+
+static int gemm_dw_group_fp8_core(int count, long long K, const void* const* dY, const long long* ldy, const float* const* dq_y, const void* const* X,
+                                  const long long* ldx, const float* const* dq_x, float* const* dW, float* const* db, const long long* M, const long long* N,
+                                  int slots, float* workspace, long long ws_elems, int overwrite, void* stream) {
   CSMAE_REQUIRE(count > 0 && count <= DW_GROUP_MAX && K > 0 && dY && X && dW && M && N && ldy && ldx && dq_y && dq_x && workspace, "csmae_gemm_dw_group_fp8: bad arguments (1..%d products)", DW_GROUP_MAX);
   Dw8GroupArgs ga;
   int tiles = 0;
@@ -232,7 +241,7 @@
     tiles += cdiv(M[i], 256) * d.tiles_n;
   }
   for (int i = count; i < DW_GROUP_MAX; ++i) ga.d[i] = ga.d[0];
-  ga.n = count; ga.K = (int)K; ga.total_tiles = tiles;
+  ga.n = count; ga.K = (int)K; ga.total_tiles = tiles; ga.overwrite = overwrite ? 1 : 0;
   ga.ktiles = cdiv(K, 128);
   if (slots <= 0) slots = 128;
   long long S = slots / tiles;
@@ -244,18 +253,26 @@
   ga.nsplit = cdiv(ga.ktiles, ga.ktiles_per_split);
   ga.slab = workspace; ga.cs_slab = nullptr;
   CSMAE_REQUIRE(ga.nsplit == 1 || ws_elems >= ga.nsplit * per_slice, "csmae_gemm_dw_group_fp8: workspace too small");
+  int maxM = 0; bool any = false;
+  if (db) for (int i = 0; i < count; ++i) if (db[i]) { any = true; if (M[i] > maxM) maxM = (int)M[i]; }
+  const int pitch = cdiv(maxM, 256) * 256;
+  CSMAE_REQUIRE(!any || ws_elems >= (long long)ga.nsplit * per_slice + (long long)count * CS_RB * pitch, "csmae_gemm_dw_group_fp8: workspace too small for the bias-gradient partial sums");
   hipLaunchKernelGGL(gemm_fp8_dw_group_kernel, dim3(tiles * ga.nsplit), dim3(512), 0, (hipStream_t)stream, ga);
   if (ga.nsplit > 1) hipLaunchKernelGGL(fp8_dw_group_reduce_kernel, dim3(tiles * DWR_PARTS), dim3(256), 0, (hipStream_t)stream, ga);
-  if (db) {
-    int maxM = 0; bool any = false;
-    for (int i = 0; i < count; ++i) if (db[i]) { any = true; if (M[i] > maxM) maxM = (int)M[i]; }
-    if (any) {
-      const int pitch = cdiv(maxM, 256) * 256;
-      float* part = workspace + (long long)ga.nsplit * per_slice;
-      CSMAE_REQUIRE(ws_elems >= (long long)ga.nsplit * per_slice + (long long)count * CS_RB * pitch, "csmae_gemm_dw_group_fp8: workspace too small for the bias-gradient partial sums");
-      hipLaunchKernelGGL(fp8_colsum_partial_kernel, dim3(pitch / 256, CS_RB, count), dim3(256), 0, (hipStream_t)stream, ga, part, pitch);
-      hipLaunchKernelGGL(fp8_colsum_fold_kernel, dim3(pitch / 256, 1, count), dim3(256), 0, (hipStream_t)stream, ga, part, pitch);
-    }
+  if (any) {
+    float* part = workspace + (long long)ga.nsplit * per_slice;
+    hipLaunchKernelGGL(fp8_colsum_partial_kernel, dim3(pitch / 256, CS_RB, count), dim3(256), 0, (hipStream_t)stream, ga, part, pitch);
+    hipLaunchKernelGGL(fp8_colsum_fold_kernel, dim3(pitch / 256, 1, count), dim3(256), 0, (hipStream_t)stream, ga, part, pitch);
   }
   return csmae_check_launch("csmae_gemm_dw_group_fp8");
 }
+extern "C" int csmae_gemm_dw_group_fp8(int count, long long K, const void* const* dY, const long long* ldy, const float* const* dq_y, const void* const* X,
+                                       const long long* ldx, const float* const* dq_x, float* const* dW, float* const* db, const long long* M, const long long* N,
+                                       int slots, float* workspace, long long ws_elems, void* stream) {
+  return gemm_dw_group_fp8_core(count, K, dY, ldy, dq_y, X, ldx, dq_x, dW, db, M, N, slots, workspace, ws_elems, 0, stream);
+}
+extern "C" int csmae_gemm_dw_group_fp8_ow(int count, long long K, const void* const* dY, const long long* ldy, const float* const* dq_y, const void* const* X,
+                                          const long long* ldx, const float* const* dq_x, float* const* dW, float* const* db, const long long* M, const long long* N,
+                                          int slots, float* workspace, long long ws_elems, int overwrite, void* stream) {
+  return gemm_dw_group_fp8_core(count, K, dY, ldy, dq_y, X, ldx, dq_x, dW, db, M, N, slots, workspace, ws_elems, overwrite, stream);
+}
diff --git a/cross-scale-mae_amd/csrc/gemm_k2.hip b/cross-scale-mae_amd/csrc/gemm_k2.hip
--- a/cross-scale-mae_amd/csrc/gemm_k2.hip
+++ b/cross-scale-mae_amd/csrc/gemm_k2.hip
@@ -278,7 +278,7 @@
 
 
 #ifdef CSMAE_K2_DW
-struct DwFold2 { float* slab; float* cs_slab; int nsplit; int slot; int nslots; };
+struct DwFold2 { float* slab; float* cs_slab; int nsplit; int slot; int nslots; int overwrite; };
 #define K2_LDS_BYTES (2 * 64 * 128 * 2 + 4 * 3 * 32 * 64 * 2)
 template <bool CS>
 __device__ __forceinline__ void k2_tile_tn(char* smem, const GemmArgs& p, const int tm, const int tn, const int split, const int kt_begin, const int kt_end, const DwFold2 fold) {
@@ -449,9 +449,16 @@
 #pragma unroll
     for (int e = 0; e < 2; ++e) {
       const int m = m0 + (2 * w + e) * 16 + t;
-      if (m < p.M) p.colsum[m] += cs[e];
-    }
-  }
+      if (m < p.M) p.colsum[m] = (fold.overwrite ? 0.0f : p.colsum[m]) + cs[e];
+    }
+  }
+  if (fold.overwrite) {
+#pragma unroll
+    for (int i = 0; i < FM; ++i)
+#pragma unroll
+      for (int jj = 0; jj < FN; ++jj) acc[i][jj] = f4_t{0.f, 0.f, 0.f, 0.f} + acc[i][jj];
+    epilogue_rows<float, EPI_NONE, FM, FN, WM, EROWS, ESTR, LPR, RPP>(p, p.C, acc, ew, m0, n0 + wn, lane, t, g);
+  } else
   epilogue_rows<float, EPI_RESID, FM, FN, WM, EROWS, ESTR, LPR, RPP>(p, p.C, acc, ew, m0, n0 + wn, lane, t, g);
   GTS(3);
 }
@@ -473,7 +480,7 @@
   p.a_bytes = (unsigned)((long long)ga.K * d.ldy * 2); p.b_bytes = (unsigned)((long long)ga.K * d.ldx * 2);
   p.force_cfg = 0; p.split_stride = 0; p.colsum = d.db; p.dq_a = p.dq_b = nullptr; p.a_fmt = 0; p.aux_q8 = 0; p.q_out = nullptr;
   __shared__ __attribute__((aligned(16))) char smem[K2_LDS_BYTES];
-  const DwFold2 fold{ga.slab, ga.cs_slab, ga.nsplit, tile_id, ga.total_tiles};
+  const DwFold2 fold{ga.slab, ga.cs_slab, ga.nsplit, tile_id, ga.total_tiles, ga.overwrite};
   if (d.db != nullptr && tn == 0) k2_tile_tn<true>(smem, p, tm, tn, split, kt_begin, kt_end, fold);
   else k2_tile_tn<false>(smem, p, tm, tn, split, kt_begin, kt_end, fold);
 }
@@ -489,20 +496,20 @@
   const long long sstride = (long long)ga.total_tiles * 128 * 256;
   const float* base = ga.slab + (long long)tile_id * 128 * 256;
   const int n = n0 + c4 * 4;
-  constexpr int RPB = 128 / DWR_PARTS;
-#pragma unroll
-  for (int r = part * RPB + r0; r < part * RPB + RPB; r += 4) {
-    const int m = m0 + r;
-    if (m >= d.M || n >= d.N) continue;
-    float* dst = d.dW + (long long)m * d.N + n;
-    f4_t a = *reinterpret_cast<f4_t*>(dst);
-    for (int sl = 0; sl < ga.nsplit; ++sl) a += *reinterpret_cast<const f4_t*>(base + sl * sstride + r * 256 + c4 * 4);
-    *reinterpret_cast<f4_t*>(dst) = a;
-  }
+  constexpr int RPB = 128 / DWR_PARTS, NR = RPB / 4;
+  const int r = part * RPB + r0;
+  float* dst[NR]; bool ok[NR];
+#pragma unroll
+  for (int i = 0; i < NR; ++i) {
+    const int m = m0 + r + 4 * i;
+    ok[i] = m < d.M && n < d.N;
+    dst[i] = d.dW + (long long)(ok[i] ? m : 0) * d.N + (ok[i] ? n : 0);
+  }
+  dw_fold_rows<NR>(base + r * 256 + c4 * 4, sstride, 4 * 256, ga.nsplit, dst, ok, ga.overwrite != 0);
   if (part == 0 && tn == 0 && d.db != nullptr && threadIdx.x < 128) {
     const int m = m0 + threadIdx.x;
     if (m < d.M) {
-      float a = d.db[m];
+      float a = ga.overwrite ? 0.0f : d.db[m];
       for (int sl = 0; sl < ga.nsplit; ++sl) a += ga.cs_slab[((long long)sl * ga.total_tiles + tile_id) * 128 + threadIdx.x];
       d.db[m] = a;
     }
diff --git a/cross-scale-mae_amd/csrc/optim.hip b/cross-scale-mae_amd/csrc/optim.hip
--- a/cross-scale-mae_amd/csrc/optim.hip
+++ b/cross-scale-mae_amd/csrc/optim.hip
@@ -65,6 +65,27 @@
   return csmae_check_launch("csmae_adamw");
 }
 
+__global__ __launch_bounds__(256) void zero_ranges_kernel(const long long* __restrict__ ranges, float* __restrict__ buf) {
+  const long long off = ranges[2 * blockIdx.y], cnt = ranges[2 * blockIdx.y + 1];
+  if (cnt <= 0) return;
+  float* p = buf + off;
+  long long head = (4 - (long long)((reinterpret_cast<uintptr_t>(p) >> 2) & 3)) & 3;
+  if (head > cnt) head = cnt;
+  const long long n4 = (cnt - head) >> 2, tail0 = head + n4 * 4;
+  const long long tid = (long long)blockIdx.x * blockDim.x + threadIdx.x, nthr = (long long)gridDim.x * blockDim.x;
+  if (tid < head) p[tid] = 0.f;
+  f4_t* p4 = reinterpret_cast<f4_t*>(p + head);
+  for (long long i = tid; i < n4; i += nthr) p4[i] = f4_t{0.f, 0.f, 0.f, 0.f};
+  if (tid < cnt - tail0) p[tail0 + tid] = 0.f;
+}
+extern "C" int csmae_zero_ranges(int nranges, const long long* ranges, long long max_count, float* buf, void* stream) {
+  CSMAE_REQUIRE(nranges >= 0 && nranges <= 65535 && (nranges == 0 || (ranges && buf)) && max_count >= 0 && (((uintptr_t)buf & 3) == 0), "csmae_zero_ranges: bad arguments (0..65535 ranges)");
+  if (nranges == 0) return CSMAE_OK;
+  const unsigned gx = (unsigned)fmax(1.0, fmin((double)cdiv(max_count, 4 * 256 * 4), 256.0));
+  hipLaunchKernelGGL(zero_ranges_kernel, dim3(gx, (unsigned)nranges), dim3(256), 0, (hipStream_t)stream, ranges, buf);
+  return csmae_check_launch("csmae_zero_ranges");
+}
+
 __global__ __launch_bounds__(256) void adamw_f8_kernel(const long long* __restrict__ tile8, float wd, float* __restrict__ p, const float* __restrict__ g, float* __restrict__ m,
                                                        float* __restrict__ v, float lr, float b1, float b2, float eps, float bc1, float bc2, bf16_t* __restrict__ p_lp,
                                                        const float* __restrict__ gate, unsigned char* __restrict__ w8, unsigned char* __restrict__ w8t,
diff --git a/include/csmae.h b/include/csmae.h
--- a/include/csmae.h
+++ b/include/csmae.h
@@ -43,9 +43,15 @@
 int csmae_gemm_dw_group(int dtype, int count, long long K, const void* const* dY, const long long* ldy, const void* const* X,
                         const long long* ldx, float* const* dW, float* const* db, const long long* M, const long long* N, int slots,
                         float* workspace, long long ws_elems, void* stream);
+int csmae_gemm_dw_group_ow(int dtype, int count, long long K, const void* const* dY, const long long* ldy, const void* const* X,
+                           const long long* ldx, float* const* dW, float* const* db, const long long* M, const long long* N, int slots,
+                           float* workspace, long long ws_elems, int overwrite, void* stream);
 int csmae_gemm_dw_group_fp8(int count, long long K, const void* const* dY, const long long* ldy, const float* const* dq_y, const void* const* X,
                             const long long* ldx, const float* const* dq_x, float* const* dW, float* const* db, const long long* M, const long long* N,
                             int slots, float* workspace, long long ws_elems, void* stream);
+int csmae_gemm_dw_group_fp8_ow(int count, long long K, const void* const* dY, const long long* ldy, const float* const* dq_y, const void* const* X,
+                               const long long* ldx, const float* const* dq_x, float* const* dW, float* const* db, const long long* M, const long long* N,
+                               int slots, float* workspace, long long ws_elems, int overwrite, void* stream);
 int csmae_fp8_amax(int in_dtype, long long rows, int cols, const void* src, long long ld, float* amax, void* stream);
 int csmae_fp8_quantize(int in_dtype, int fmt, int transpose, long long rows, int cols, const void* src, long long ld, void* dst,
                        long long ldd, const float* amax, float* dq, float* amax_next , void* stream);
@@ -159,6 +165,7 @@
 int csmae_adamw(long long ntiles, const long long* tile_off, const int* tile_cnt, const float* tile_wd, float* p, const float* g,
                 float* m, float* v, float lr, float beta1, float beta2, float eps, float bias_correction1, float bias_correction2,
                 void* p_lp, const float* gate, const long long* tile_ks, void* p_ks, void* stream);
+int csmae_zero_ranges(int nranges, const long long* ranges, long long max_count, float* buf, void* stream);
 int csmae_adamw_fp8(long long ntiles, const long long* tile8, float weight_decay, float* p, const float* g, float* m, float* v, float lr, float beta1,
                     float beta2, float eps, float bias_correction1, float bias_correction2, void* p_lp, const float* gate, void* w8, void* w8t,
                     const float* amax_prev, float* amax_next, float* dq, void* stream);
```

New measurement: 6053 images/s, median of 2. About the same (+0.2%).
